# Owen-Liuyuxuan/FSNet

Hardware: AMD Instinct MI355X
Metric: training samples/sec (3-frame triplets) at 192x640, ResNet-18 depth+pose (higher is better)
Workload: dtype bf16; 1 GPU; KITTI Eigen-Zhou-shaped synthetic triplets, ResNet-18 depth+pose, 192x640, bf16, batch 12/GPU, full step (fwd+loss+bwd+clip35+Adam); inputs HBM-resident, no H2D in the timed region; global_batch=12, parallelism=dp1, encoder_pass=two chains (depth and pose encoder on two streams), autotune_steps=0, hipgraph_replays=570

## Files before the change

### fsnet_amd/csrc/bn.hip

```cpp
#include "common.h"
#include "fsnet_hip_internal.h"
#include <algorithm>
#include <cstdlib>

namespace {

__device__ __forceinline__ int pow2_shift(int v) { return (v & (v - 1)) == 0 ? __ffs(v) - 1 : -1; }
__device__ __forceinline__ void split_vec(long i, int CG, int sh, int& cg, long& m) {
  if (sh >= 0) { cg = (int)(i & (CG - 1)); m = i >> sh; }
  else if (i < (1L << 31)) { const unsigned u = (unsigned)i, q = u / (unsigned)CG; cg = (int)(u - q * CG); m = q; }
  else { cg = (int)(i % CG); m = i / CG; }
}
__device__ __forceinline__ void split_row(long m, int H, int W, long& n, int& h, int& w) {
  if (m < (1L << 31)) {
    const unsigned u = (unsigned)m, q = u / (unsigned)W, nn = q / (unsigned)H;
    w = (int)(u - q * W); h = (int)(q - nn * H); n = nn;
  } else {
    w = (int)(m % W); const long q = m / W; h = (int)(q % H); n = q / H;
  }
}


constexpr int MAXC = 2048;

// ... 281 lines not shown
        for (int j = 0; j < V; ++j) {
          v[j] = v[j] * sc[j] + sh[j];
          if (p.relu) v[j] = fmaxf(v[j], 0.f);
        }
        const uint4 u = Unit<T>::pack(v);
        Unit<T>::unpack(u, v);
        if (y && r >= 1 && s >= 1) *reinterpret_cast<uint4*>(y + off) = u;
#pragma unroll
        for (int j = 0; j < V; ++j)
          if (fst || v[j] > best[j]) { best[j] = v[j]; bi[j] = r * 3 + s; }
        fst = false;
      }
    }
    const long mg = ((n * Ho + ho) * Wo + wo) * C + c;
    storev<T>(py + mg, best);
#pragma unroll
    for (int k = 0; k < V / 4; ++k) {
      const uint32_t packed = (uint32_t)bi[4 * k] | ((uint32_t)bi[4 * k + 1] << 8) | ((uint32_t)bi[4 * k + 2] << 16) |
                              ((uint32_t)bi[4 * k + 3] << 24);
      reinterpret_cast<uint32_t*>(p.pool_idx + mg)[k] = packed;
    }
  }
}

template <typename T>
__device__ inline void load_dout(const FsBnBwdArgs& p, const T* dout, long n, int h, int w, int c, float* g) {
  constexpr int V = VecN<T>::N;
  if (!p.fold) {
    loadv<T>(dout + n * p.gN + (long)h * p.gH + (long)w * p.gW + c, g);
    return;
  }
#pragma unroll
  for (int j = 0; j < V; ++j) g[j] = 0.f;
  int hs[2] = {h + 1, 0}, ws[2] = {w + 1, 0};
  int nh = 1, nw = 1;
  if (h == 0) { hs[1] = 0; nh = 2; } else if (h == p.H - 1) { hs[1] = p.H + 1; nh = 2; }
  if (w == 0) { ws[1] = 0; nw = 2; } else if (w == p.W - 1) { ws[1] = p.W + 1; nw = 2; }
  for (int a = 0; a < nh; ++a)
    for (int b = 0; b < nw; ++b) {
      float t[V];
      loadv<T>(dout + n * p.gN + (long)hs[a] * p.gH + (long)ws[b] * p.gW + c, t);
#pragma unroll
      for (int j = 0; j < V; ++j) g[j] += t[j];
    }
}

template <typename T>
__device__ inline void masked_grad(const FsBnBwdArgs& p, const T* dout, const T* yv, long m, int c, float* g) {
  constexpr int V = VecN<T>::N;
  const long hw = (long)p.H * p.W;
  if (!p.fold && p.gW == p.C && p.gH == (long)p.W * p.C && p.gN == hw * p.C &&
      (!p.relu || (p.yW == p.C && p.yH == (long)p.W * p.C && p.yN == hw * p.C))) {
    loadv<T>(dout + m * p.C + c, g);
    if (p.relu) {
      float yy[V];
      loadv<T>(yv + m * p.C + c, yy);
#pragma unroll
      for (int j = 0; j < V; ++j) g[j] = yy[j] > 0.f ? g[j] : 0.f;
    }
    return;
  }
  int w, h; long n;
  split_row(m, p.H, p.W, n, h, w);
  load_dout<T>(p, dout, n, h, w, c, g);
  if (p.relu) {
    float yy[V];
    loadv<T>(yv + n * p.yN + (long)h * p.yH + (long)w * p.yW + c, yy);
#pragma unroll
    for (int j = 0; j < V; ++j) g[j] = yy[j] > 0.f ? g[j] : 0.f;
  }
}


template <typename T>
__device__ inline void pool_grad(const FsBnBwdArgs& p, long m, int c, float* g) {
  constexpr int V = VecN<T>::N;
  const int C = p.C, H = p.H, W = p.W, Ho = H >> 1, Wo = W >> 1;
  const unsigned u = (unsigned)m, q = u / (unsigned)W, nn = q / (unsigned)H;
  const int w = (int)(u - q * W), h = (int)(q - nn * H);
  const int h2 = h >> 1, w2 = w >> 1;
  const int r0 = (h & 1) ? 2 : 1, s0 = (w & 1) ? 2 : 1;
  const bool vh = (h & 1) && h2 + 1 < Ho, vw = (w & 1) && w2 + 1 < Wo;
  const long base = (((long)nn * Ho + h2) * Wo + w2) * C + c;
  const long dh = vh ? (long)Wo * C : 0, dw = vw ? C : 0;
  const long off[4] = {base, base + dw, base + dh, base + dh + dw};
  const int code[4] = {r0 * 3 + s0, r0 * 3, s0, 0};
  const bool ok[4] = {true, vw, vh, vh && vw};
  const T* __restrict__ dy = reinterpret_cast<const T*>(p.pool_dy);
  uint32_t packed[4][V / 4];
  float t[4][V];
#pragma unroll
  for (int k = 0; k < 4; ++k) {
#pragma unroll
    for (int e = 0; e < V / 4; ++e) packed[k][e] = reinterpret_cast<const uint32_t*>(p.pool_idx + off[k])[e];
    loadv<T>(dy + off[k], t[k]);
  }
  if (p.dout) loadv<T>(reinterpret_cast<const T*>(p.dout) + m * C + c, g);
  else {
#pragma unroll
    for (int j = 0; j < V; ++j) g[j] = 0.f;
  }
#pragma unroll
  for (int k = 0; k < 4; ++k)
#pragma unroll
    for (int j = 0; j < V; ++j)
      if (ok[k] && (int)((packed[k][j >> 2] >> (8 * (j & 3))) & 0xff) == code[k]) g[j] += t[k][j];
}
template <typename T>
__device__ inline void pool_mask(const FsBnBwdArgs& p, const T* yv, long m, int c, const float* xr, const float* sc,
                                 const float* sh, float* g) {
  constexpr int V = VecN<T>::N;
  if (!p.relu) return;
  if (yv) {
    float yy[V];
    loadv<T>(yv + m * p.C + c, yy);
#pragma unroll
    for (int j = 0; j < V; ++j) g[j] = yy[j] > 0.f ? g[j] : 0.f;
  } else {
// ... 244 lines not shown
          if (left > 2) req(off + 2 * step, d2, x2, y2);
#pragma unroll
          for (int j = 0; j < V; ++j) { s1[j] += g[j]; s2[j] += g[j] * (xr[j] - mean[j]) * istd[j]; }
        }
        m = m_end;
      }
    }
    for (; m + stride < m_end; m += 2 * stride) {
      float g0[V], g1[V], x0[V], x1[V];
      masked_grad<T>(p, dout, yv, m, c, g0);
      masked_grad<T>(p, dout, yv, m + stride, c, g1);
      loadv<T>(xv + m * C + c, x0);
      loadv<T>(xv + (m + stride) * C + c, x1);
#pragma unroll
      for (int j = 0; j < V; ++j) {
        s1[j] += g0[j] + g1[j];
        s2[j] += g0[j] * (x0[j] - mean[j]) * istd[j] + g1[j] * (x1[j] - mean[j]) * istd[j];
      }
    }
    for (; m < m_end; m += stride) {
      float g0[V], x0[V];
      masked_grad<T>(p, dout, yv, m, c, g0);
      loadv<T>(xv + m * C + c, x0);
#pragma unroll
      for (int j = 0; j < V; ++j) { s1[j] += g0[j]; s2[j] += g0[j] * (x0[j] - mean[j]) * istd[j]; }
    }
  }
#pragma unroll
  for (int j = 0; j < V; ++j) { red[0][j][threadIdx.x] = s1[j]; red[1][j][threadIdx.x] = s2[j]; }
  __syncthreads();
  if (act && pl < 2 * V && pl < PL) {
    for (int kj = pl; kj < 2 * V; kj += PL) {
      int kind = kj / V, j = kj % V;
      float a = 0.f;
      for (int k = 0; k < PL; ++k) a += red[kind][j][k * CGB + cgl];
      double* sl = p.sums + ((long)z * FS_STAT_SLOTS + blockIdx.x % FS_STAT_SLOTS) * 2 * C;
      atomicAdd(sl + kind * C + c + j, (double)a);
    }
  }
}

template <typename T, bool POOL = false>
__global__ __launch_bounds__(256) void bn_bwd_apply_kernel(const FsDual<FsBnBwdArgs, FsNoGeom> d, const int fast) {
  extern __shared__ float bn_smem[];
  const int prob = (int)blockIdx.z >= d.nb0 ? 1 : 0;
  const FsBnBwdArgs& p = d.a[prob];
  const int C = p.C;
  constexpr int V = VecN<T>::N;
  const int CG = C / V, cg_sh = pow2_shift(CG);
  const int SCG = gridDim.y > 1 ? 32 : CG, scg_sh = gridDim.y > 1 ? 5 : cg_sh;
  const int SC = SCG * V, c0 = (int)blockIdx.y * SC;
  float* s_a = bn_smem; float* s_b = bn_smem + SC; float* s_k = bn_smem + 2 * SC;
  float* s_mean = bn_smem + 3 * SC; float* s_istd = bn_smem + 4 * SC;
  const int G = p.groups > 1 ? p.groups : 1;
  const int z = (int)blockIdx.z - (prob ? d.nb0 : 0);
  const int Mg = p.M / G;
  const double* sums = p.sums + (long)z * FS_STAT_SLOTS * 2 * C;
  const double* sums_local = p.sums_local ? p.sums_local + (long)z * FS_STAT_SLOTS * 2 * C : nullptr;
  const T* __restrict__ dout = reinterpret_cast<const T*>(p.dout);
  const T* __restrict__ yv = reinterpret_cast<const T*>(p.y);
  const T* __restrict__ xv = reinterpret_cast<const T*>(p.x);
  const long total = (long)Mg * SCG;
  const long i0 = (long)blockIdx.x * 256 + threadIdx.x;
  float pg[V], px[V];
  if (i0 < total) {
    int cg; long m;
    split_vec(i0, SCG, scg_sh, cg, m);
    m += (long)z * Mg;
    if constexpr (POOL) pool_grad<T>(p, m, c0 + cg * V, pg);
    else masked_grad<T>(p, dout, yv, m, c0 + cg * V, pg);
    loadv<T>(xv + m * C + c0 + cg * V, px);
  }
  for (int cl = threadIdx.x; cl < SC; cl += 256) {
    const int c = c0 + cl;
    double sg = 0.0, sgx = 0.0, lg = 0.0, lgx = 0.0;
#pragma unroll
    for (int k = 0; k < FS_STAT_SLOTS; ++k) {
      sg += sums[(long)k * 2 * C + c]; sgx += sums[(long)k * 2 * C + C + c];
      if (sums_local) { lg += sums_local[(long)k * 2 * C + c]; lgx += sums_local[(long)k * 2 * C + C + c]; }
    }
    float istd = p.save_invstd[z * C + c];
    s_mean[cl] = p.save_mean[z * C + c]; s_istd[cl] = istd;
    s_k[cl] = p.gamma[c] * istd;
    if constexpr (POOL) bn_smem[5 * SC + cl] = (p.beta ? p.beta[c] : 0.f) - s_mean[cl] * s_k[cl];
    s_a[cl] = (float)(sg / p.count);
    s_b[cl] = (float)(sgx / p.count);
    if (blockIdx.x == 0) {
      if (G > 1) {
        if (p.dgamma) atomicAdd(p.dgamma + c, (float)(sums_local ? lgx : sgx));
        if (p.dbeta) atomicAdd(p.dbeta + c, (float)(sums_local ? lg : sg));
      } else {
        if (p.dgamma) p.dgamma[c] += (float)(sums_local ? lgx : sgx);
        if (p.dbeta) p.dbeta[c] += (float)(sums_local ? lg : sg);
      }
    }
  }
  __syncthreads();
  T* __restrict__ dx = reinterpret_cast<T*>(p.dx);
  T* __restrict__ gout = reinterpret_cast<T*>(p.g_out);
  const long stride = (long)gridDim.x * 256;
  if constexpr (!POOL) {
    const long hw = (long)p.H * p.W;
    const bool plain = fast && !p.fold && scg_sh >= 0 && p.gW == C && p.gH == (long)p.W * C && p.gN == hw * C &&
                       (!p.relu || (p.yW == C && p.yH == (long)p.W * C && p.yN == hw * C));
    if (plain) {
      if (i0 >= total) return;
      const int cl = (int)(i0 & (SCG - 1)) * V;
      const long rows = stride >> scg_sh, step = rows * C;
      long off = ((long)z * Mg + (i0 >> scg_sh)) * C + c0 + cl;
      long left = (total - i0 + stride - 1) / stride;
      const bool relu = p.relu != 0;
      float ka[V], kb[V], kk[V], km[V], ki[V];
#pragma unroll
      for (int j = 0; j < V; ++j) { ka[j] = s_a[cl + j]; kb[j] = s_b[cl + j]; kk[j] = s_k[cl + j]; km[j] = s_mean[cl + j]; ki[j] = s_istd[cl + j]; }
      uint4 d1, x1, y1, d2, x2, y2;
      d1 = x1 = y1 = d2 = x2 = y2 = make_uint4(0, 0, 0, 0);
      if (left > 1) {
        d1 = *reinterpret_cast<const uint4*>(dout + off + step); x1 = *reinterpret_cast<const uint4*>(xv + off + step);
        if (relu) y1 = *reinterpret_cast<const uint4*>(yv + off + step);
      }
      if (left > 2) {
        d2 = *reinterpret_cast<const uint4*>(dout + off + 2 * step); x2 = *reinterpret_cast<const uint4*>(xv + off + 2 * step);
        if (relu) y2 = *reinterpret_cast<const uint4*>(yv + off + 2 * step);
      }
      float g[V], xr[V], o[V];
#pragma unroll
      for (int j = 0; j < V; ++j) { g[j] = pg[j]; xr[j] = px[j]; }
      for (;;) {
#pragma unroll
        for (int j = 0; j < V; ++j) {
          float xh = (xr[j] - km[j]) * ki[j];
          o[j] = kk[j] * (g[j] - ka[j] - xh * kb[j]);
        }
        storev<T>(dx + off, o);
        if (gout) storev<T>(gout + off, g);
        if (--left == 0) break;
        off += step;
        Unit<T>::unpack(d1, g); Unit<T>::unpack(x1, xr);
        if (relu) {
          float yy[V];
          Unit<T>::unpack(y1, yy);
#pragma unroll
          for (int j = 0; j < V; ++j) g[j] = yy[j] > 0.f ? g[j] : 0.f;
        }
        d1 = d2; x1 = x2; y1 = y2;
        if (left > 2) {
          d2 = *reinterpret_cast<const uint4*>(dout + off + 2 * step); x2 = *reinterpret_cast<const uint4*>(xv + off + 2 * step);
          if (relu) y2 = *reinterpret_cast<const uint4*>(yv + off + 2 * step);
        }
      }
      return;
    }
  }
  for (long i = i0; i < total; i += stride) {
    int cg; long m;
    split_vec(i, SCG, scg_sh, cg, m);
    m += (long)z * Mg;
    const int cl = cg * V, c = c0 + cl;
    float g[V], xr[V], o[V];
#pragma unroll
    for (int j = 0; j < V; ++j) { g[j] = pg[j]; xr[j] = px[j]; }
    if (i + stride < total) {
      int cg2; long m2;
      split_vec(i + stride, SCG, scg_sh, cg2, m2);
      m2 += (long)z * Mg;
      if constexpr (POOL) pool_grad<T>(p, m2, c0 + cg2 * V, pg);
      else masked_grad<T>(p, dout, yv, m2, c0 + cg2 * V, pg);
      loadv<T>(xv + m2 * C + c0 + cg2 * V, px);
    }
    if constexpr (POOL) pool_mask<T>(p, yv, m, c, xr, s_k + cl, bn_smem + 5 * SC + cl, g);
#pragma unroll
    for (int j = 0; j < V; ++j) {
      float xh = (xr[j] - s_mean[cl + j]) * s_istd[cl + j];
      o[j] = s_k[cl + j] * (g[j] - s_a[cl + j] - xh * s_b[cl + j]);
    }
    storev<T>(dx + m * C + c, o);
    if (gout) storev<T>(gout + m * C + c, g);
  }
}

int bn_slabs(int CG) { return (CG > 32 && (CG & (CG - 1)) == 0) ? CG / 32 : 1; }

bool bn_pool_quads(int CG) { return CG >= 1 && CG <= 32 && (CG & (CG - 1)) == 0; }

int grid_for(long items) {
  long b = (items + 255) / 256;
  const long cap = 512;
  if (b > cap) b = cap;
  if (b < 1) b = 1;
  return (int)b;
}

}

extern "C" int fs_bn_finalize(const FsBnApplyArgs* a, float* scale, float* shift, void* stream) {
  if (!a || !a->gamma || !a->beta || !a->save_mean || !a->save_invstd || !scale || !shift) return FS_EINVAL;
  if (!a->stats && (!a->running_mean || !a->running_var)) return FS_EINVAL;
  if (a->C <= 0 || a->C > MAXC || a->gamma2) return FS_EINVAL;
  const int G = a->groups > 1 ? a->groups : 1;
  if (G > 1 && !a->stats) return FS_EINVAL;
  hipLaunchKernelGGL(bn_finalize_kernel, dim3((a->C + 255) / 256, G), dim3(256), 0, reinterpret_cast<hipStream_t>(stream),
                     *a, scale, shift);
  return fs_launch_status();
}

namespace {
int bn_apply_check(const FsBnApplyArgs* a) {
  if (!a || !a->x || (!a->y && !a->pool_y) || !a->gamma || !a->beta || !a->save_mean || !a->save_invstd) return FS_EINVAL;
  if (a->pool_y) {
    if (!a->pool_idx || !a->stats || a->res || a->gamma2 || a->pad_out || a->H <= 0 || a->W <= 0 || (a->H & 1) || (a->W & 1))
      return FS_EINVAL;
    if (a->M % (a->H * a->W) != 0 || (long)a->M * (a->C / 4) >= 0x7fffffffL) return FS_EINVAL;
    if (a->y && !(a->yW == a->C && a->yH == (long)a->W * a->C && a->yN == (long)a->H * a->W * a->C)) return FS_EINVAL;
  }
  if (!a->stats && (!a->running_mean || !a->running_var)) return FS_EINVAL;
  if (a->C % 8 != 0 || a->C > MAXC || a->M <= 0) return FS_EINVAL;
  if (a->gamma2 && (!a->res || !a->beta2 || !a->save_mean2 || !a->save_invstd2)) return FS_EINVAL;
  if (a->gamma2 && !a->stats2 && (!a->running_mean2 || !a->running_var2)) return FS_EINVAL;
  const int G = a->groups > 1 ? a->groups : 1;
  if (a->M % G != 0 || (G > 1 && !a->stats)) return FS_EINVAL;
  return FS_OK;
}
int bn_bwd_check(const FsBnBwdArgs* a, bool apply) {
  if (!a || (!a->dout && !a->pool_dy) || !a->x || !a->sums || !a->save_mean || !a->save_invstd) return FS_EINVAL;
  if (apply && (!a->dx || !a->gamma)) return FS_EINVAL;
  if (a->C % 8 != 0 || a->C > MAXC || a->M <= 0) return FS_EINVAL;
  const int G = a->groups > 1 ? a->groups : 1;
  if (a->M % G != 0) return FS_EINVAL;
  if (a->pool_dy) {
    if (!a->pool_idx || !a->gamma || a->fold || a->g_out || a->H <= 0 || a->W <= 0 || (a->H & 1) || (a->W & 1)) return FS_EINVAL;
    if (a->relu && !a->y && !a->beta) return FS_EINVAL;
    const long hw = (long)a->H * a->W;
    if (a->M % hw != 0 || (a->M / G) % hw != 0 || (long)a->M >= 0x7fffffffL) return FS_EINVAL;
    if (a->dout && !(a->gW == a->C && a->gH == (long)a->W * a->C && a->gN == hw * a->C)) return FS_EINVAL;
    if (a->y && !(a->yW == a->C && a->yH == (long)a->W * a->C && a->yN == hw * a->C)) return FS_EINVAL;
    return FS_OK;
  }
  if (a->relu && !a->y) return FS_EINVAL;
  return FS_OK;
}
template <typename A>
FsDual<A, FsNoGeom> bn_dual(const A* a, const A* b) {
  FsDual<A, FsNoGeom> d;
  d.a[0] = *a; d.a[1] = b ? *b : *a;
  d.g[0].unused = d.g[1].unused = 0;
  d.nb0 = a->groups > 1 ? a->groups : 1;
  d.nprob = b ? 2 : 1;
  return d;
}
}

extern "C" int fs_bn_apply2(const FsBnApplyArgs* a, const FsBnApplyArgs* b, int dtype, void* stream) {
  int r = bn_apply_check(a);
  if (r != FS_OK) return r;
  if (b) {
    r = bn_apply_check(b);
    if (r != FS_OK) return r;
    if (b->C != a->C || (a->pool_y != nullptr) != (b->pool_y != nullptr) || (a->pool_y && (a->H != b->H || a->W != b->W))) {
      r = fs_bn_apply2(a, nullptr, dtype, stream);
      return r != FS_OK ? r : fs_bn_apply2(b, nullptr, dtype, stream);
    }
  }
  hipStream_t st = reinterpret_cast<hipStream_t>(stream);
  const int vec = dtype == FS_DTYPE_BF16 ? 8 : 4;
  const int G = a->groups > 1 ? a->groups : 1, G1 = b ? (b->groups > 1 ? b->groups : 1) : 0;
  long items = (long)(a->M / G) * (a->C / vec);
  if (b) items = std::max(items, (long)(b->M / G1) * (b->C / vec));
  const FsDual<FsBnApplyArgs, FsNoGeom> d = bn_dual(a, b);
  if (a->pool_y) {
    dim3 pgrid(std::min(2 * grid_for(items / 4), (int)((items / 4 + 255) / 256)), 1, G + G1);
    if (pgrid.x < 1) pgrid.x = 1;
    const unsigned plds = 2u * a->C * sizeof(float);
    if (dtype == FS_DTYPE_BF16) hipLaunchKernelGGL(bn_apply_pool_kernel<bf16>, pgrid, dim3(256), plds, st, d);
    else if (dtype == FS_DTYPE_F32) hipLaunchKernelGGL(bn_apply_pool_kernel<float>, pgrid, dim3(256), plds, st, d);
    else return FS_EINVAL;
    return fs_launch_status();
  }
  const int nslab = bn_slabs(a->C / vec);
  dim3 grid(std::min(grid_for(items / nslab), std::max(32, grid_for(1L << 40) / nslab)), nslab, G + G1);
  const unsigned lds = ((a->gamma2 || (b && b->gamma2)) ? 4u : 2u) * (a->C / nslab) * sizeof(float);
  const int fast = 1;
  if (dtype == FS_DTYPE_BF16) hipLaunchKernelGGL(bn_apply_kernel<bf16>, grid, dim3(256), lds, st, d, fast);
  else if (dtype == FS_DTYPE_F32) hipLaunchKernelGGL(bn_apply_kernel<float>, grid, dim3(256), lds, st, d, fast);
  else return FS_EINVAL;
  return fs_launch_status();
}

extern "C" int fs_bn_apply(const FsBnApplyArgs* a, int dtype, void* stream) { return fs_bn_apply2(a, nullptr, dtype, stream); }

extern "C" int fs_bn_bwd_reduce2(const FsBnBwdArgs* a, const FsBnBwdArgs* b, int dtype, void* stream) {
  int r = bn_bwd_check(a, false);
// ... 13 lines not shown
  if (b) Mg = std::max<long>(Mg, b->M / G1);
  const FsDual<FsBnBwdArgs, FsNoGeom> d = bn_dual(a, b);
  if (a->pool_dy && bn_pool_quads(CG)) {
    long Qg = (a->M / G) / 4;
    if (b) Qg = std::max<long>(Qg, (b->M / G1) / 4);
    dim3 grid((unsigned)std::min<long>((Qg + 256 / CG - 1) / (256 / CG), 1024), 1, G + G1);
    if (dtype == FS_DTYPE_BF16) hipLaunchKernelGGL(bn_bwd_reduce_pool_kernel<bf16>, grid, dim3(256), 0, st, d);
    else if (dtype == FS_DTYPE_F32) hipLaunchKernelGGL(bn_bwd_reduce_pool_kernel<float>, grid, dim3(256), 0, st, d);
    else return FS_EINVAL;
    return fs_launch_status();
  }
#define LAUNCH_REDUCE(CGB, ROWS_PER_BLOCK, MAXB)                                                               \
  {                                                                                                             \
    dim3 grid((unsigned)std::min<long>((Mg + (ROWS_PER_BLOCK) - 1) / (ROWS_PER_BLOCK), MAXB), (CG + CGB - 1) / CGB, G + G1); \
    if (a->pool_dy) {                                                                                           \
      if (dtype == FS_DTYPE_BF16) hipLaunchKernelGGL((bn_bwd_reduce_kernel<bf16, CGB, true>), grid, dim3(256), 0, st, d, 0);  \
      else if (dtype == FS_DTYPE_F32) hipLaunchKernelGGL((bn_bwd_reduce_kernel<float, CGB, true>), grid, dim3(256), 0, st, d, 0); \
      else return FS_EINVAL;                                                                                    \
    } else                                                                                                      \
    if (dtype == FS_DTYPE_BF16) hipLaunchKernelGGL((bn_bwd_reduce_kernel<bf16, CGB>), grid, dim3(256), 0, st, d, rfast);  \
    else if (dtype == FS_DTYPE_F32) hipLaunchKernelGGL((bn_bwd_reduce_kernel<float, CGB>), grid, dim3(256), 0, st, d, rfast); \
    else return FS_EINVAL;                                                                                      \
  }
  const int rfast = 1;
  const long wide_cap = std::max<long>(32, std::min<long>(512, 1024 / ((long)((CG + 31) / 32) * (G + G1))));
  if (CG >= 32) LAUNCH_REDUCE(32, 16, wide_cap)
  else if (CG >= 8) LAUNCH_REDUCE(8, 64, 1024)
  else if (CG >= 4) LAUNCH_REDUCE(4, 128, 1024)
  else LAUNCH_REDUCE(2, 256, 1024)
#undef LAUNCH_REDUCE
  return fs_launch_status();
}

extern "C" int fs_bn_bwd_reduce(const FsBnBwdArgs* a, int dtype, void* stream) { return fs_bn_bwd_reduce2(a, nullptr, dtype, stream); }

extern "C" int fs_bn_bwd_apply2(const FsBnBwdArgs* a, const FsBnBwdArgs* b, int dtype, void* stream) {
  int r = bn_bwd_check(a, true);
  if (r != FS_OK) return r;
  if (b) {
    r = bn_bwd_check(b, true);
    if (r != FS_OK) return r;
    if (b->C != a->C || (a->pool_dy != nullptr) != (b->pool_dy != nullptr) || (a->pool_dy && (a->H != b->H || a->W != b->W))) {
      r = fs_bn_bwd_apply2(a, nullptr, dtype, stream);
      return r != FS_OK ? r : fs_bn_bwd_apply2(b, nullptr, dtype, stream);
    }
  }
  hipStream_t st = reinterpret_cast<hipStream_t>(stream);
  const int vec = dtype == FS_DTYPE_BF16 ? 8 : 4;
  const int G = a->groups > 1 ? a->groups : 1, G1 = b ? (b->groups > 1 ? b->groups : 1) : 0;
  long items = (long)(a->M / G) * (a->C / vec);
  if (b) items = std::max(items, (long)(b->M / G1) * (b->C / vec));
  const int nslab = a->pool_dy ? 1 : bn_slabs(a->C / vec);
  dim3 grid(std::min(grid_for(items / nslab), std::max(32, grid_for(1L << 40) / nslab)), nslab, G + G1);
  const unsigned lds = (a->pool_dy ? 6u : 5u) * (a->C / nslab) * sizeof(float);
  const FsDual<FsBnBwdArgs, FsNoGeom> d = bn_dual(a, b);
  const int fast = 1;
  if (a->pool_dy && bn_pool_quads(a->C / vec)) {
    const int CG = a->C / vec;
    long Qg = (a->M / G) / 4;
    if (b) Qg = std::max<long>(Qg, (b->M / G1) / 4);
    dim3 qgrid((unsigned)std::min<long>((Qg + 256 / CG - 1) / (256 / CG), 2048), 1, G + G1);
    if (dtype == FS_DTYPE_BF16) hipLaunchKernelGGL(bn_bwd_apply_pool_kernel<bf16>, qgrid, dim3(256), lds, st, d);
    else if (dtype == FS_DTYPE_F32) hipLaunchKernelGGL(bn_bwd_apply_pool_kernel<float>, qgrid, dim3(256), lds, st, d);
    else return FS_EINVAL;
    return fs_launch_status();
  }
  if (a->pool_dy) {
    if (dtype == FS_DTYPE_BF16) hipLaunchKernelGGL((bn_bwd_apply_kernel<bf16, true>), grid, dim3(256), lds, st, d, 0);
    else if (dtype == FS_DTYPE_F32) hipLaunchKernelGGL((bn_bwd_apply_kernel<float, true>), grid, dim3(256), lds, st, d, 0);
    else return FS_EINVAL;
    return fs_launch_status();
  }
  if (dtype == FS_DTYPE_BF16) hipLaunchKernelGGL(bn_bwd_apply_kernel<bf16>, grid, dim3(256), lds, st, d, fast);
  else if (dtype == FS_DTYPE_F32) hipLaunchKernelGGL(bn_bwd_apply_kernel<float>, grid, dim3(256), lds, st, d, fast);
  else return FS_EINVAL;
  return fs_launch_status();
}

extern "C" int fs_bn_bwd_apply(const FsBnBwdArgs* a, int dtype, void* stream) { return fs_bn_bwd_apply2(a, nullptr, dtype, stream); }
```

### fsnet_amd/csrc/common.h

```cpp
#pragma once
#include <hip/hip_runtime.h>
#include <stdint.h>

typedef __bf16 bf16;
typedef __attribute__((ext_vector_type(8))) __bf16 bf16x8;
typedef __attribute__((ext_vector_type(4))) __bf16 bf16x4;
typedef __attribute__((ext_vector_type(4))) short s16x4;
typedef __attribute__((ext_vector_type(4))) float f32x4;

#define FS_WAVE 64

#define FS_OK 0
#define FS_EINVAL 1
#define FS_ELAUNCH 2

static inline int fs_launch_status() {
  hipError_t e = hipGetLastError();
  return e == hipSuccess ? FS_OK : FS_ELAUNCH;
}

template <typename T> struct ElemTraits;
template <> struct ElemTraits<float> {
  static constexpr int EG = 4;
  __device__ static inline float to_f(float v) { return v; }
  __device__ static inline float from_f(float v) { return v; }
};
template <> struct ElemTraits<bf16> {
  static constexpr int EG = 8;
  __device__ static inline float to_f(bf16 v) { return (float)v; }
  __device__ static inline bf16 from_f(float v) { return (bf16)v; }
};

__device__ static inline float bf16_bits_to_f(uint32_t b16) { return __uint_as_float(b16 << 16); }
__device__ static inline uint32_t f_to_bf16_bits(float f) {
  uint32_t u = __float_as_uint(f);
  u += 0x7fffu + ((u >> 16) & 1u);
  return u >> 16;
}
typedef __attribute__((ext_vector_type(2))) __bf16 bf16x2_t;
typedef __attribute__((ext_vector_type(2))) float f32x2_t;
__device__ static inline uint32_t pack_bf16x2(float lo, float hi) {
  f32x2_t v = {lo, hi};
  return __builtin_bit_cast(uint32_t, __builtin_convertvector(v, bf16x2_t));
}

template <typename T> __device__ inline void load4(const T* p, float v[4]);
template <> __device__ inline void load4<float>(const float* p, float v[4]) {
  float4 t = *reinterpret_cast<const float4*>(p);
  v[0] = t.x; v[1] = t.y; v[2] = t.z; v[3] = t.w;
}
template <> __device__ inline void load4<bf16>(const bf16* p, float v[4]) {
  uint2 t = *reinterpret_cast<const uint2*>(p);
  v[0] = bf16_bits_to_f(t.x & 0xffffu); v[1] = bf16_bits_to_f(t.x >> 16);
  v[2] = bf16_bits_to_f(t.y & 0xffffu); v[3] = bf16_bits_to_f(t.y >> 16);
}
template <typename T> __device__ inline void store4(T* p, const float v[4]);
template <> __device__ inline void store4<float>(float* p, const float v[4]) {
  *reinterpret_cast<float4*>(p) = make_float4(v[0], v[1], v[2], v[3]);
}
template <> __device__ inline void store4<bf16>(bf16* p, const float v[4]) {
  uint2 t; t.x = pack_bf16x2(v[0], v[1]); t.y = pack_bf16x2(v[2], v[3]);
  *reinterpret_cast<uint2*>(p) = t;
}

__host__ __device__ static inline unsigned fs_div_magic(int d) { return (1u << 20) / (unsigned)d + 1u; }
__device__ static inline int fs_fastdiv(int x, unsigned magic) { return (int)(((unsigned)x * magic) >> 20); }

struct FsDiv { unsigned m; unsigned sh; };
__host__ static inline FsDiv fs_make_div(int d) {
  int l = 0;
  while ((1LL << l) < (long long)d) ++l;
  FsDiv r;
  r.m = (unsigned)(((1ULL << (31 + l)) / (unsigned long long)d) + 1ULL);
  r.sh = (unsigned)(31 + l);
  return r;
}
__device__ static inline int fs_div(int x, FsDiv d) {
  return (int)(((unsigned long long)(unsigned)x * d.m) >> d.sh);
}

template <int CTRL>
__device__ static inline float dpp_mov(float v) {
  return __builtin_bit_cast(float, __builtin_amdgcn_update_dpp(0, __builtin_bit_cast(int, v), CTRL, 0xf, 0xf, true));
}
template <int CTRL>
__device__ static inline double dpp_mov(double v) {
  const long long b = __builtin_bit_cast(long long, v);
  const int lo = __builtin_amdgcn_update_dpp(0, (int)b, CTRL, 0xf, 0xf, true);
  const int hi = __builtin_amdgcn_update_dpp(0, (int)(b >> 32), CTRL, 0xf, 0xf, true);
  return __builtin_bit_cast(double, ((long long)hi << 32) | (unsigned int)lo);
}
__device__ static inline float read_lane(float v, int lane) {
  return __builtin_bit_cast(float, __builtin_amdgcn_readlane(__builtin_bit_cast(int, v), lane));
}
__device__ static inline double read_lane(double v, int lane) {
  const long long b = __builtin_bit_cast(long long, v);
  const int lo = __builtin_amdgcn_readlane((int)b, lane), hi = __builtin_amdgcn_readlane((int)(b >> 32), lane);
  return __builtin_bit_cast(double, ((long long)hi << 32) | (unsigned int)lo);
}
template <typename F>
__device__ static inline F row16_sum(F v) {
  v += dpp_mov<0xB1>(v);
  v += dpp_mov<0x4E>(v);
  v += dpp_mov<0x141>(v);
  v += dpp_mov<0x140>(v);
  return v;
}
__device__ static inline float wave_sum(float v) {
  v = row16_sum(v);
  return (read_lane(v, 0) + read_lane(v, 16)) + (read_lane(v, 32) + read_lane(v, 48));
}
__device__ static inline double wave_sum_d(double v) {
  v = row16_sum(v);
  return (read_lane(v, 0) + read_lane(v, 16)) + (read_lane(v, 32) + read_lane(v, 48));
}
// ... 56 lines not shown
```

### fsnet_amd/csrc/conv1x1.hip

```cpp
#include <cstdlib>
#include "common.h"
#include "fsnet_hip_internal.h"

namespace {

__device__ __forceinline__ uint4 buf_load16(__amdgpu_buffer_rsrc_t rsrc, int voff) {
  return __builtin_bit_cast(uint4, __builtin_amdgcn_raw_buffer_load_b128(rsrc, voff, 0, 0));
}

template <typename T, int CO, int KC>
__global__ __launch_bounds__(256) void conv1x1_kernel(const FsConvArgs p, const FsDiv dW, const FsDiv dH) {
  constexpr int PIX = 128, WP = 4, WC = 1;
  constexpr int WPIX = PIX / WP, WCO = CO / WC;
  constexpr int TP = WPIX / 16, TC = WCO / 16;
  constexpr int UR = KC / 8;
  constexpr int KS = KC / 32;
  constexpr int LCU = (CO * UR + 255) / 256;
  static_assert(sizeof(T) == 2, "bf16 only");
  __shared__ uint4 lds_c[CO * UR < 128 ? 128 : CO * UR];
  constexpr int OROW = CO * 2 + 16;
  __shared__ __attribute__((aligned(16))) unsigned char lds_o[4][WPIX * OROW];

  const int t = threadIdx.x;
  const int lane = t & 63, wave = t >> 6;
// ... 165 lines not shown
  if (p.stats) {
    __syncthreads();
    float* red = reinterpret_cast<float*>(&lds_c[0]);
#pragma unroll
    for (int a = 0; a < TC; ++a)
#pragma unroll
      for (int j = 0; j < 4; ++j) {
        float u = s1[a][j], w = s2[a][j];
        u = row16_sum(u); w = row16_sum(w);
        if (li == 0) {
          int cl = wc * WCO + a * 16 + lg * 4 + j;
          red[(wp * CO + cl) * 2] = u; red[(wp * CO + cl) * 2 + 1] = w;
        }
      }
    __syncthreads();
    if (t < CO) {
      float u = 0.f, w = 0.f;
#pragma unroll
      for (int k = 0; k < WP; ++k) { u += red[(k * CO + t) * 2]; w += red[(k * CO + t) * 2 + 1]; }
      int co = co0 + t;
      if (co < p.Co) {
        const long sg = p.grp_imgs > 0 ? (long)blockIdx.z : (p.stat_group_rows > 0 ? pix0 / p.stat_group_rows : 0);
        double* sl = p.stats + (sg * FS_STAT_SLOTS + px % FS_STAT_SLOTS) * 2 * p.Co;
        atomicAdd(sl + co, (double)u);
        atomicAdd(sl + p.Co + co, (double)w);
      }
    }
  }
}


template <typename T, int CO, int KC>
int launch_1x1(const FsConvArgs& a, hipStream_t st) {
  constexpr int PIX = 128;
  const int npix = (a.M + PIX - 1) / PIX, nco = a.Co_p / CO;
  int blocks = npix * nco;
  if (nco % 8 != 0 && 8 % nco == 0) { const int g = 8 / nco; blocks = 8 * ((npix + g - 1) / g); }
  hipLaunchKernelGGL((conv1x1_kernel<T, CO, KC>), dim3(blocks, 1, a.grp_imgs > 0 ? a.N / a.grp_imgs : 1), dim3(256), 0, st,
                     a, fs_make_div(a.Wd), fs_make_div(a.Hd));
  return fs_launch_status();
}

template <typename T, int CO>
int launch_co(const FsConvArgs& a, hipStream_t st) {
  if (a.Cs <= 64) return launch_1x1<T, CO, 64>(a, st);
  if (a.Cs <= 128) return launch_1x1<T, CO, 128>(a, st);
  return launch_1x1<T, CO, 256>(a, st);
}

}

extern "C" int fs_conv1x1(const FsConvArgs* args, int dtype, void* stream) {
  if (!args || !args->src || !args->wgt || !args->dst) return FS_EINVAL;
  if (dtype != FS_DTYPE_BF16 || args->dshift != 0 || args->ncls > 1 || args->hb_add != 0 || args->hb_mul < 1) return FS_EINVAL;
  if (args->Cs <= 0 || (args->Cs * 2) % 64 != 0 || args->Co % 4 != 0 || args->Co_p % 16 != 0 || args->M <= 0) return FS_EINVAL;
  if (args->src_bytes <= 0 || args->src_bytes > 0x7fffffffLL || args->wgt_bytes <= 0 || args->wgt_bytes > 0x7fffffffLL)
    return FS_EINVAL;
  if (args->stats && args->stat_group_rows > 0 && args->stat_group_rows % 128 != 0) return FS_EINVAL;
  hipStream_t st = reinterpret_cast<hipStream_t>(stream);
  {
    const int r = fs_conv1x1_gemm(*args, st);
    if (r != FS_EINVAL) return r;
  }
  const int cop = args->Co_p;
  if (cop % 64 == 0) return launch_co<bf16, 64>(*args, st);
  if (cop % 32 == 0) return launch_co<bf16, 32>(*args, st);
  return launch_co<bf16, 16>(*args, st);
}
```

### fsnet_amd/csrc/conv3x3_halo.hip

```cpp
#include "common.h"
#include "fsnet_hip_internal.h"
#include "conv_pro.h"
#include <algorithm>
#include <cstdlib>

namespace {

__device__ __forceinline__ int swz64(int row) { return ((row >> 3) & 1) << 1; }

__device__ __forceinline__ uint4 buf_load16(__amdgpu_buffer_rsrc_t rsrc, int voff) {
  return __builtin_bit_cast(uint4, __builtin_amdgcn_raw_buffer_load_b128(rsrc, voff, 0, 0));
}

__device__ __forceinline__ void lds_barrier() {
  asm volatile("s_waitcnt lgkmcnt(0)" ::: "memory");
  __builtin_amdgcn_s_barrier();
  asm volatile("" ::: "memory");
}

struct HaloGeom {
  int TH, TW;
  int tiles_x, tiles_y;
  unsigned mTW, mHW;
  FsDiv dTX, dTY;
// ... 141 lines not shown
    int pi = wp * WPIX + b * 16 + li;
    if (pi >= ntile) pi = 0;
    int ty = fs_fastdiv(pi, g.mTW), tx = pi - ty * g.TW;
    hbase[b] = (STR * ty * HWs + tx) * HS + lg;
  }

  f32x4 acc[TC][TP];
#pragma unroll
  for (int a = 0; a < TC; ++a)
#pragma unroll
    for (int b = 0; b < TP; ++b) acc[a][b] = f32x4{0.f, 0.f, 0.f, 0.f};
  const int s2_row = HWs * HS, s2_par = (g.TW + 1) * HS;

  const int nchunk = (p.Cs * (int)sizeof(T) + 63) / 64;
  load_regs(0);
  for (int cc = 0; cc < nchunk; ++cc) {
    lds_barrier();
    store_lds(cc);
    lds_barrier();
    if (cc + 1 < nchunk) load_regs(cc + 1);
#pragma unroll
    for (int tap = 0; tap < 9; ++tap) {
      const int r = tap / 3, s = tap - r * 3;
      const int hoff = STR == 2 ? r * s2_row + (s & 1) * s2_par + (s >> 1) * HS
                                : (fwd ? (r * HW + s) : ((2 - r) * HW + (2 - s))) * HS;
      uint4 fa[TC], fb[TP];
#pragma unroll
      for (int a = 0; a < TC; ++a) {
        int row = tap * CO + wc * WCO + a * 16 + li;
        fa[a] = lds_w[row * 4 + (lg ^ swz64(row))];
      }
#pragma unroll
      for (int b = 0; b < TP; ++b) fb[b] = lds_h[hbase[b] + hoff];
#pragma unroll
      for (int a = 0; a < TC; ++a)
#pragma unroll
        for (int b = 0; b < TP; ++b) {
          if constexpr (sizeof(T) == 2) {
            acc[a][b] = __builtin_amdgcn_mfma_f32_16x16x32_bf16(
                __builtin_bit_cast(bf16x8, fa[a]), __builtin_bit_cast(bf16x8, fb[b]), acc[a][b], 0, 0, 0);
          } else {
            f32x4 va = __builtin_bit_cast(f32x4, fa[a]);
            f32x4 vb = __builtin_bit_cast(f32x4, fb[b]);
#pragma unroll
            for (int j = 0; j < 4; ++j)
              acc[a][b] = __builtin_amdgcn_mfma_f32_16x16x4f32(va[j], vb[j], acc[a][b], 0, 0, 0);
          }
        }
    }
  }

  const bool has_add = STR == 1 && p.addend != nullptr, has_mask = STR == 1 && p.mask != nullptr;
  const bool has_bnb = STR == 1 && p.bnb_x != nullptr, has_mbn = has_bnb && p.bnb_scale != nullptr;
  float s1[TC][4], s2[TC][4];
#pragma unroll
  for (int a = 0; a < TC; ++a)
#pragma unroll
    for (int j = 0; j < 4; ++j) { s1[a][j] = 0.f; s2[a][j] = 0.f; }
  const int sgoff = p.stat_group_rows > 0 ? fs_div(n, g.dIPG) * p.Co : 0;
  int doff[TP], aoff[TP], moff[TP];
#pragma unroll
  for (int b = 0; b < TP; ++b) {
    int pi = wp * WPIX + b * 16 + li;
    int ty = fs_fastdiv(pi, g.mTW), tx = pi - ty * g.TW;
    int y = y0 + ty, x = x0 + tx;
    bool mok = pi < ntile && y < p.Hd && x < p.Wd;
    doff[b] = mok ? n * (int)p.dN + y * (int)p.dH + x * (int)p.dW : -1;
    aoff[b] = n * (int)p.aN + y * (int)p.aH + x * (int)p.aW;
    moff[b] = n * (int)p.mN + y * (int)p.mH + x * (int)p.mW;
  }
#pragma unroll
  for (int a = 0; a < TC; ++a) {
    const int co = co0 + wc * WCO + a * 16 + lg * 4;
    if (co >= p.Co) continue;
    float4 bv = make_float4(0.f, 0.f, 0.f, 0.f), mu = bv, is = bv, msc = bv, msh = bv;
    if (p.bias) bv = *reinterpret_cast<const float4*>(p.bias + co);
    if (has_bnb) {
      mu = *reinterpret_cast<const float4*>(p.bnb_mean + sgoff + co);
      is = *reinterpret_cast<const float4*>(p.bnb_invstd + sgoff + co);
      if (has_mbn) {
        msc = *reinterpret_cast<const float4*>(p.bnb_scale + sgoff + co);
        msh = *reinterpret_cast<const float4*>(p.bnb_shift + sgoff + co);
      }
    }
#pragma unroll
    for (int b = 0; b < TP; ++b) {
      if (doff[b] < 0) continue;
      float v[4] = {acc[a][b][0] + bv.x, acc[a][b][1] + bv.y, acc[a][b][2] + bv.z, acc[a][b][3] + bv.w};
      if (has_add) {
        float av[4];
        load4<T>(reinterpret_cast<const T*>(p.addend) + aoff[b] + co, av);
        v[0] += av[0]; v[1] += av[1]; v[2] += av[2]; v[3] += av[3];
      }
      if (p.relu) {
#pragma unroll
        for (int j = 0; j < 4; ++j) v[j] = fmaxf(v[j], 0.f);
      }
      if (has_mask) {
        float mv[4];
        load4<T>(reinterpret_cast<const T*>(p.mask) + moff[b] + co, mv);
#pragma unroll
        for (int j = 0; j < 4; ++j) v[j] = mv[j] > 0.f ? v[j] : 0.f;
      }
      if (has_bnb) {
        float cv[4];
        load4<T>(reinterpret_cast<const T*>(p.bnb_x) + doff[b] + co, cv);
        if (has_mbn) {
          v[0] = (cv[0] * msc.x + msh.x) > 0.f ? v[0] : 0.f; v[1] = (cv[1] * msc.y + msh.y) > 0.f ? v[1] : 0.f;
          v[2] = (cv[2] * msc.z + msh.z) > 0.f ? v[2] : 0.f; v[3] = (cv[3] * msc.w + msh.w) > 0.f ? v[3] : 0.f;
        }
        s1[a][0] += v[0]; s1[a][1] += v[1]; s1[a][2] += v[2]; s1[a][3] += v[3];
        s2[a][0] += v[0] * (cv[0] - mu.x) * is.x; s2[a][1] += v[1] * (cv[1] - mu.y) * is.y;
        s2[a][2] += v[2] * (cv[2] - mu.z) * is.z; s2[a][3] += v[3] * (cv[3] - mu.w) * is.w;
      } else if (p.stats) {
#pragma unroll
        for (int j = 0; j < 4; ++j) { s1[a][j] += v[j]; s2[a][j] += v[j] * v[j]; }
      }
      if (p.out_f32) store4<float>(reinterpret_cast<float*>(p.dst) + doff[b] + co, v);
      else store4<T>(reinterpret_cast<T*>(p.dst) + doff[b] + co, v);
    }
  }
  if (p.stats) {
    lds_barrier();
    float* red = reinterpret_cast<float*>(&lds_w[0]);
#pragma unroll
    for (int a = 0; a < TC; ++a)
#pragma unroll
      for (int j = 0; j < 4; ++j) {
        float u = s1[a][j], w = s2[a][j];
        u = row16_sum(u); w = row16_sum(w);
        if (li == 0) {
          int cl = wc * WCO + a * 16 + lg * 4 + j;
          red[(wp * CO + cl) * 2] = u; red[(wp * CO + cl) * 2 + 1] = w;
        }
      }
    lds_barrier();
    if (t < CO) {
      float u = 0.f, w = 0.f;
#pragma unroll
      for (int k = 0; k < WP; ++k) { u += red[(k * CO + t) * 2]; w += red[(k * CO + t) * 2 + 1]; }
      int co = co0 + t;
      if (co < p.Co) {
        const long sg = p.stat_group_rows > 0 ? fs_div(n, g.dIPG) : 0;
        double* sl = p.stats + (sg * FS_STAT_SLOTS + px % FS_STAT_SLOTS) * 2 * p.Co;
        atomicAdd(sl + co, (double)u);
        atomicAdd(sl + p.Co + co, (double)w);
      }
    }
  }
  if constexpr (PRO != 0) { if (bid == 0) pro_block0<PRO>(p, t, 256); }
}

HaloGeom pick_geom(int Hd, int Wd, int PIX, int hmax) {
  HaloGeom best{0, 0, 0, 0, 0u, 0u, FsDiv{0u, 0u}, FsDiv{0u, 0u}, FsDiv{0u, 0u}, FsDiv{0u, 0u}, 0};
  double best_cost = 1e30;
  for (int tw = std::min(4, Wd); tw <= std::min(Wd, 64); ++tw) {
    int th = std::min(PIX / tw, Hd);
    if (th < 1 || (th + 2) * (tw + 2) > hmax) continue;
    int tx = (Wd + tw - 1) / tw, ty = (Hd + th - 1) / th;
    double waste = (double)tx * ty * PIX / ((double)Hd * Wd);
    double halo = (double)(th + 2) * (tw + 2) / ((double)th * tw);
    double cost = waste * (1.0 + 0.15 * halo);
    if (cost < best_cost - 1e-9) { best_cost = cost; best.TH = th; best.TW = tw; best.tiles_x = tx; best.tiles_y = ty; }
  }
  if (best.TW > 0) {
    best.mTW = fs_div_magic(best.TW); best.mHW = fs_div_magic(best.TW + 2);
// ... 83 lines not shown
template <typename T>
int dispatch(const FsConvArgs& a, const FsConvArgs* b, hipStream_t st) {
  const int cop = a.Co_p;
  const int nimg = a.N + (b ? b->N : 0);
  auto blocks_for = [&](int PIX, int CO) {
    HaloGeom g = pick_geom(a.Hd, a.Wd, PIX, PIX == 256 ? 360 : (PIX == 128 ? 208 : 120));
    return g.TH == 0 ? 0L : (long)nimg * g.tiles_x * g.tiles_y * (cop / CO);
  };
  if (cop % 32 == 0) {
    if (blocks_for(128, 32) < 256) return launch_halo<T, 128, 16, 4>(a, b, st);
    return launch_halo<T, 128, 32, 4>(a, b, st);
  }
  if (cop % 16 == 0) {
    if (blocks_for(256, 16) >= 1024) return launch_halo<T, 256, 16, 4>(a, b, st);
    return launch_halo<T, 128, 16, 4>(a, b, st);
  }
  return FS_EINVAL;
}

}

int fs_conv3x3_t32(const FsConvArgs& a, const FsConvArgs* b, int dtype, hipStream_t st);
int fs_conv3x3_p1(const FsConvArgs& a, int dtype, hipStream_t st);

namespace {
int conv3x3_check(const FsConvArgs* args, int dtype) {
  if (!args || !args->src || !args->wgt || !args->dst) return FS_EINVAL;
  const int es = dtype == FS_DTYPE_BF16 ? 2 : 4;
  if (args->Cs <= 0 || (args->Cs * es) % 32 != 0 || ((args->Cs * es) % 64 != 0 && args->Cs * es != 32) || args->dshift != 0)
    return FS_EINVAL;
  const bool s2 = args->hb_mul == 2;
  if (args->hb_mul != 1 && !(s2 && args->sgn > 0 && args->hb_add == -1 && (args->Cs * es) % 64 == 0 && args->pro_mode == 0 &&
                             !args->bnb_x && !args->addend && !args->mask &&
                             args->Hd == (args->Hs - 1) / 2 + 1 && args->Wd == (args->Ws - 1) / 2 + 1))
    return FS_EINVAL;
  if (args->Co % 4 != 0 || args->Co_p % 16 != 0 || args->N <= 0) return FS_EINVAL;
  if (args->src_bytes <= 0 || args->src_bytes > 0x7fffffffLL || args->wgt_bytes <= 0 ||
      args->wgt_bytes > 0x7fffffffLL)
    return FS_EINVAL;
  if (!pro_args_ok(*args)) return FS_EINVAL;
  if (args->pro_mode != 0 && (args->Cs * es) % 64 != 0) return FS_EINVAL;
  {
    auto span_ok = [&](const void* ptr, int64_t sn, int64_t sh, int64_t sw) {
      if (!ptr) return true;
      if (sn < 0 || sh < 0 || sw < 0) return false;
      return (int64_t)(args->N - 1) * sn + (int64_t)(args->Hd - 1) * sh + (int64_t)(args->Wd - 1) * sw + args->Co_p < 0x7fffffffLL;
    };
    if (!span_ok(args->dst, args->dN, args->dH, args->dW) || !span_ok(args->addend, args->aN, args->aH, args->aW) ||
        !span_ok(args->mask, args->mN, args->mH, args->mW))
      return FS_EINVAL;
  }
  if (args->bnb_scale && (!args->bnb_x || !args->bnb_shift || args->mask)) return FS_EINVAL;
  if (args->bnb_x && (!args->stats || !args->bnb_mean || !args->bnb_invstd)) return FS_EINVAL;
  return FS_OK;
}

bool conv3x3_pairable(const FsConvArgs& a, const FsConvArgs& b) {
  auto nn = [](const void* x, const void* y) { return (x == nullptr) == (y == nullptr); };
  return a.Hs == b.Hs && a.Ws == b.Ws && a.Hd == b.Hd && a.Wd == b.Wd && a.Cs == b.Cs && a.Co == b.Co && a.Co_p == b.Co_p &&
         a.nchunks == b.nchunks && a.kg == b.kg && a.hb_mul == b.hb_mul && a.hb_add == b.hb_add && a.sgn == b.sgn &&
         a.relu == b.relu && a.out_f32 == b.out_f32 && a.pro_mode == b.pro_mode && a.pro_relu == b.pro_relu &&
         a.wgt_bytes == b.wgt_bytes && nn(a.bias, b.bias) && nn(a.addend, b.addend) && nn(a.mask, b.mask) &&
         nn(a.stats, b.stats) && nn(a.bnb_x, b.bnb_x) && nn(a.bnb_scale, b.bnb_scale) && nn(a.pro_stats, b.pro_stats);
}

int conv3x3_entry(const FsConvArgs* args, const FsConvArgs* b, int dtype, hipStream_t st) {
  int r = conv3x3_check(args, dtype);
  if (r != FS_OK) return r;
  if (b) {
    r = conv3x3_check(b, dtype);
    if (r != FS_OK) return r;
    if (!conv3x3_pairable(*args, *b)) {
      r = conv3x3_entry(args, nullptr, dtype, st);
      return r != FS_OK ? r : conv3x3_entry(b, nullptr, dtype, st);
    }
  }
  if (args->hb_mul == 2) {
    if (dtype == FS_DTYPE_BF16) return dispatch_s2<bf16>(*args, b, st);
    if (dtype == FS_DTYPE_F32) return dispatch_s2<float>(*args, b, st);
    return FS_EINVAL;
  }
  const int force = args->force_impl;
  if (force < 0 || force > 5 || (b && b->force_impl != force)) return FS_EINVAL;
  if (!b && (force == 0 || force == 5)) {
    r = fs_conv3x3_p1(*args, dtype, st);
    if (r != FS_EINVAL) return r;
  }
  if (force != 1) {
    r = fs_conv3x3_t32(*args, b, dtype, st);
    if (r != FS_EINVAL || (force >= 2 && force <= 4)) return r;
  }
  if (dtype == FS_DTYPE_BF16) return dispatch<bf16>(*args, b, st);
  if (dtype == FS_DTYPE_F32) return dispatch<float>(*args, b, st);
  return FS_EINVAL;
}
}

extern "C" int fs_conv3x3_halo(const FsConvArgs* args, int dtype, void* stream) {
  return conv3x3_entry(args, nullptr, dtype, reinterpret_cast<hipStream_t>(stream));
}

extern "C" int fs_conv3x3_halo2(const FsConvArgs* a0, const FsConvArgs* a1, int dtype, void* stream) {
  return conv3x3_entry(a0, a1, dtype, reinterpret_cast<hipStream_t>(stream));
}

extern "C" int fs_conv3x3_halo_plan(const FsConvArgs* args, int dtype, int32_t* plan) {
  if (!plan) return FS_EINVAL;
  plan[0] = -1; plan[1] = plan[2] = plan[3] = 0;
  fs_conv3x3_plan_slot = plan;
  const int r = conv3x3_entry(args, nullptr, dtype, nullptr);
  fs_conv3x3_plan_slot = nullptr;
  return r;
}

extern "C" int fs_conv3x3_halo2_plan(const FsConvArgs* a0, const FsConvArgs* a1, int dtype, int32_t* plan) {
  if (!plan || !a0) return FS_EINVAL;
// ... 9 lines not shown
```

### fsnet_amd/csrc/conv3x3_p1.hip

```cpp
#include "common.h"
#include "fsnet_hip_internal.h"
#include <algorithm>
#include <cstdlib>

namespace {

__device__ __forceinline__ int p1_swz64(int row) { return ((row >> 3) & 1) << 1; }
__device__ __forceinline__ uint4 p1_load16(__amdgpu_buffer_rsrc_t rsrc, int voff) {
  return __builtin_bit_cast(uint4, __builtin_amdgcn_raw_buffer_load_b128(rsrc, voff, 0, 0));
}
__device__ __forceinline__ void p1_barrier() {
  asm volatile("s_waitcnt lgkmcnt(0)" ::: "memory");
  __builtin_amdgcn_s_barrier();
  asm volatile("" ::: "memory");
}

struct P1Geom {
  int TH, TW, tiles_x, tiles_y, ntiles;
  unsigned mTW, mHW;
  FsDiv dTX, dTY, dIPG;
};

template <typename T, int CO, int UQ>
__global__ __launch_bounds__(256, CO == 16 ? 3 : 2) void conv3x3_p1_kernel(const FsConvArgs p, const P1Geom g) {
// ... 26 lines not shown
      const int tap = rt / CO, row = rt - tap * CO;
      const int off = (tap < 9 && q * 16 < row_bytes) ? row * wrow_bytes + tap * row_bytes + q * 16 : OOB;
      const uint4 w = p1_load16(rs_wgt, off);
      if (rt < 9 * CO) lds_w[rt * 4 + (q ^ p1_swz64(rt))] = w;
    }
  }

  int hrel[LH], hyx[LH];
#pragma unroll
  for (int i = 0; i < LH; ++i) {
    const int idx = t + i * 256, hp = idx / UQ, q = idx % UQ;
    const int hy = fs_fastdiv(min(hp, 4095), g.mHW), hx = hp - hy * HW;
    const bool ok = hp < nhalo && q * 16 < row_bytes;
    hyx[i] = ok ? ((hy << 16) | hx) : -1;
    hrel[i] = (int)(((long)hy * p.sH + (long)hx * p.sW) * es) + q * 16;
  }
  int hbase[TP];
#pragma unroll
  for (int b = 0; b < TP; ++b) {
    int pi = wp * WPIX + b * 16 + li;
    if (pi >= ntile) pi = 0;
    const int ty = fs_fastdiv(pi, g.mTW), tx = pi - ty * g.TW;
    hbase[b] = (ty * HW + tx) * HS + lg;
  }
  int prow[TP];
#pragma unroll
  for (int b = 0; b < TP; ++b) {
    const int pi = wp * WPIX + b * 16 + li;
    const int ty = fs_fastdiv(pi, g.mTW), tx = pi - ty * g.TW;
    prow[b] = pi < ntile ? ((ty << 16) | tx) : -1;
  }

  uint4 rh[LH];
  auto tile_origin = [&](int tile, int& n, int& y0, int& x0) {
    const int tq = fs_div(tile, g.dTX); const int tx_i = tile - tq * g.tiles_x;
    n = fs_div(tq, g.dTY); const int ty_i = tq - n * g.tiles_y;
    y0 = ty_i * g.TH; x0 = tx_i * g.TW;
  };
  auto load_tile = [&](int tile) {
    int n, y0, x0;
    tile_origin(tile, n, y0, x0);
    const int oy = y0 + p.hb_add + (fwd ? 0 : -2), ox = x0 + p.hb_add + (fwd ? 0 : -2);
    const long base = ((long)n * p.sN + (long)oy * p.sH + (long)ox * p.sW) * es;
#pragma unroll
    for (int i = 0; i < LH; ++i) {
      const int hy = hyx[i] >> 16, hx = hyx[i] & 0xffff;
      const bool ok = hyx[i] >= 0 && (unsigned)(oy + hy) < (unsigned)p.Hs && (unsigned)(ox + hx) < (unsigned)p.Ws;
      rh[i] = p1_load16(rs_src, ok ? (int)(base + hrel[i]) : OOB);
    }
  };

  const bool has_add = p.addend != nullptr, has_mask = p.mask != nullptr;
  const bool has_bnb = p.bnb_x != nullptr, has_mbn = has_bnb && p.bnb_scale != nullptr;

  auto store_halo = [&]() {
#pragma unroll
    for (int i = 0; i < LH; ++i) {
      const int idx = t + i * 256, hp = idx / UQ, q = idx % UQ;
      if (hp < HMAX) lds_h[hp * HS + q] = rh[i];
    }
  };
  if constexpr (UQ < 4) {
    for (int idx = t; idx < HMAX * (4 - UQ); idx += 256) lds_h[(idx / (4 - UQ)) * HS + UQ + idx % (4 - UQ)] = make_uint4(0u, 0u, 0u, 0u);
  }
  const int gstep = (int)gridDim.x;
  load_tile(blockIdx.x);
  store_halo();
  if ((int)blockIdx.x + gstep < g.ntiles) load_tile(blockIdx.x + gstep);
  p1_barrier();
  for (int tile = blockIdx.x; tile < g.ntiles; tile += gstep) {
    f32x4 acc[TC][TP];
#pragma unroll
    for (int a = 0; a < TC; ++a)
#pragma unroll
      for (int b = 0; b < TP; ++b) acc[a][b] = f32x4{0.f, 0.f, 0.f, 0.f};
#pragma unroll 1
    for (int r = 0; r < 3; ++r)
#pragma unroll
    for (int s = 0; s < 3; ++s) {
      const int tap = r * 3 + s;
      const int hoff = (fwd ? (r * HW + s) : ((2 - r) * HW + (2 - s))) * HS;
      uint4 fa[TC], fb[TP];
#pragma unroll
      for (int a = 0; a < TC; ++a) {
        const int row = tap * CO + a * 16 + li;
        fa[a] = lds_w[row * 4 + (lg ^ p1_swz64(row))];
      }
#pragma unroll
      for (int b = 0; b < TP; ++b) fb[b] = lds_h[hbase[b] + hoff];
#pragma unroll
      for (int a = 0; a < TC; ++a)
#pragma unroll
        for (int b = 0; b < TP; ++b) {
          if constexpr (sizeof(T) == 2) {
            acc[a][b] = __builtin_amdgcn_mfma_f32_16x16x32_bf16(
                __builtin_bit_cast(bf16x8, fa[a]), __builtin_bit_cast(bf16x8, fb[b]), acc[a][b], 0, 0, 0);
          } else {
            const f32x4 va = __builtin_bit_cast(f32x4, fa[a]), vb = __builtin_bit_cast(f32x4, fb[b]);
#pragma unroll
            for (int j = 0; j < 4; ++j)
              acc[a][b] = __builtin_amdgcn_mfma_f32_16x16x4f32(va[j], vb[j], acc[a][b], 0, 0, 0);
          }
        }
    }

    p1_barrier();
    if (tile + gstep < g.ntiles) {
      store_halo();
      if (tile + 2 * gstep < g.ntiles) load_tile(tile + 2 * gstep);
    }

    int n, y0, x0;
    tile_origin(tile, n, y0, x0);
    const int sgoff = p.stat_group_rows > 0 ? fs_div(n, g.dIPG) * p.Co : 0;
    float s1[TC][4], s2[TC][4];
#pragma unroll
    for (int a = 0; a < TC; ++a)
#pragma unroll
      for (int j = 0; j < 4; ++j) { s1[a][j] = 0.f; s2[a][j] = 0.f; }
    int doff[TP], aoff[TP], moff[TP];
#pragma unroll
    for (int b = 0; b < TP; ++b) {
      const int y = y0 + (prow[b] >> 16), x = x0 + (prow[b] & 0xffff);
      const bool mok = prow[b] >= 0 && y < p.Hd && x < p.Wd;
      doff[b] = mok ? n * (int)p.dN + y * (int)p.dH + x * (int)p.dW : -1;
      aoff[b] = n * (int)p.aN + y * (int)p.aH + x * (int)p.aW;
      moff[b] = n * (int)p.mN + y * (int)p.mH + x * (int)p.mW;
    }
#pragma unroll
    for (int a = 0; a < TC; ++a) {
      const int co = a * 16 + lg * 4;
      if (co >= p.Co) continue;
      float4 bv = make_float4(0.f, 0.f, 0.f, 0.f), mu = bv, is = bv, msc = bv, msh = bv;
      if (p.bias) bv = *reinterpret_cast<const float4*>(p.bias + co);
      if (has_bnb) {
        mu = *reinterpret_cast<const float4*>(p.bnb_mean + sgoff + co);
        is = *reinterpret_cast<const float4*>(p.bnb_invstd + sgoff + co);
        if (has_mbn) {
          msc = *reinterpret_cast<const float4*>(p.bnb_scale + sgoff + co);
          msh = *reinterpret_cast<const float4*>(p.bnb_shift + sgoff + co);
        }
      }
#pragma unroll
      for (int b = 0; b < TP; ++b) {
        if (doff[b] < 0) continue;
        float v[4] = {acc[a][b][0] + bv.x, acc[a][b][1] + bv.y, acc[a][b][2] + bv.z, acc[a][b][3] + bv.w};
        if (has_add) {
          float av[4];
          load4<T>(reinterpret_cast<const T*>(p.addend) + aoff[b] + co, av);
          v[0] += av[0]; v[1] += av[1]; v[2] += av[2]; v[3] += av[3];
        }
        if (p.relu) {
#pragma unroll
          for (int j = 0; j < 4; ++j) v[j] = fmaxf(v[j], 0.f);
        }
        if (has_mask) {
          float mv[4];
          load4<T>(reinterpret_cast<const T*>(p.mask) + moff[b] + co, mv);
#pragma unroll
          for (int j = 0; j < 4; ++j) v[j] = mv[j] > 0.f ? v[j] : 0.f;
        }
        if (has_bnb) {
          float cv[4];
          load4<T>(reinterpret_cast<const T*>(p.bnb_x) + doff[b] + co, cv);
          if (has_mbn) {
            v[0] = (cv[0] * msc.x + msh.x) > 0.f ? v[0] : 0.f; v[1] = (cv[1] * msc.y + msh.y) > 0.f ? v[1] : 0.f;
            v[2] = (cv[2] * msc.z + msh.z) > 0.f ? v[2] : 0.f; v[3] = (cv[3] * msc.w + msh.w) > 0.f ? v[3] : 0.f;
          }
          s1[a][0] += v[0]; s1[a][1] += v[1]; s1[a][2] += v[2]; s1[a][3] += v[3];
          s2[a][0] += v[0] * (cv[0] - mu.x) * is.x; s2[a][1] += v[1] * (cv[1] - mu.y) * is.y;
          s2[a][2] += v[2] * (cv[2] - mu.z) * is.z; s2[a][3] += v[3] * (cv[3] - mu.w) * is.w;
        } else if (p.stats) {
#pragma unroll
          for (int j = 0; j < 4; ++j) { s1[a][j] += v[j]; s2[a][j] += v[j] * v[j]; }
        }
        if (p.out_f32) store4<float>(reinterpret_cast<float*>(p.dst) + doff[b] + co, v);
        else store4<T>(reinterpret_cast<T*>(p.dst) + doff[b] + co, v);
      }
    }
    if (p.stats) {
#pragma unroll
      for (int a = 0; a < TC; ++a)
#pragma unroll
        for (int j = 0; j < 4; ++j) {
          float u = row16_sum(s1[a][j]), w = row16_sum(s2[a][j]);
          if (li == 0) {
            const int cl = a * 16 + lg * 4 + j;
            red[(wp * CO + cl) * 2] = u; red[(wp * CO + cl) * 2 + 1] = w;
          }
        }
      p1_barrier();
      if (t < CO) {
        float u = 0.f, w = 0.f;
#pragma unroll
        for (int k = 0; k < 4; ++k) { u += red[(k * CO + t) * 2]; w += red[(k * CO + t) * 2 + 1]; }
        if (t < p.Co) {
          const long sg = p.stat_group_rows > 0 ? fs_div(n, g.dIPG) : 0;
          double* sl = p.stats + (sg * FS_STAT_SLOTS + tile % FS_STAT_SLOTS) * 2 * p.Co;
          atomicAdd(sl + t, (double)u);
          atomicAdd(sl + p.Co + t, (double)w);
        }
      }
    }
    p1_barrier();
  }
}

P1Geom p1_pick_geom(int Hd, int Wd) {
  P1Geom best{};
  double best_cost = 1e30;
  for (int tw = std::min(4, Wd); tw <= std::min(Wd, 64); ++tw) {
    const int th = std::min(256 / tw, Hd);
    if (th < 1 || (th + 2) * (tw + 2) > 360) continue;
    const int tx = (Wd + tw - 1) / tw, ty = (Hd + th - 1) / th;
    const double waste = (double)tx * ty * 256 / ((double)Hd * Wd);
    const double halo = (double)(th + 2) * (tw + 2) / ((double)th * tw);
    const double cost = waste * (1.0 + 0.15 * halo);
    if (cost < best_cost - 1e-9) { best_cost = cost; best.TH = th; best.TW = tw; best.tiles_x = tx; best.tiles_y = ty; }
  }
  if (best.TW > 0) {
    best.mTW = fs_div_magic(best.TW); best.mHW = fs_div_magic(best.TW + 2);
    best.dTX = fs_make_div(best.tiles_x); best.dTY = fs_make_div(best.tiles_y);
  }
  return best;
// ... 55 lines not shown
```

### fsnet_amd/csrc/conv3x3_s2d.hip

```cpp
#include "t32_common.h"

namespace {

struct S2dGeom {
  int TH, TW;
  int tiles_x, tiles_y;
  unsigned mTW, mHW;
  FsDiv dTX, dTY;
  FsDiv dIPG;
  int pix_major;
};

constexpr int S2D_PIX = 128;
constexpr int S2D_CO = 32;
constexpr int S2D_HMAX = 192;

constexpr int s2d_cls(int pos) { return pos == 0 ? 0 : (pos <= 2 ? 1 : (pos <= 4 ? 2 : 3)); }
constexpr int s2d_off(int pos) { return pos == 1 ? 1 : (pos == 3 ? 2 : (pos == 5 ? 3 : (pos == 6 ? 2 : (pos == 7 ? 1 : 0)))); }

template <typename T, int EP, bool DS>
__global__ __launch_bounds__(256, 3) void conv3x3_s2d_kernel(const FsDual<FsConvArgs, S2dGeom> d) {
  const int prob = (int)blockIdx.x >= d.nb0 ? 1 : 0;
  const FsConvArgs& p = d.a[prob];
  const S2dGeom& g = d.g[prob];
// ... 268 lines not shown
  return blocks;
}

template <typename T, int EP, bool DS>
int s2d_launch(const FsConvArgs& a, const FsConvArgs* b, hipStream_t st) {
  FsDual<FsConvArgs, S2dGeom> d;
  d.a[0] = a; d.a[1] = b ? *b : a;
  d.nprob = b ? 2 : 1;
  int blocks = s2d_problem(a, d.g[0]);
  if (blocks == 0) return FS_EINVAL;
  d.g[1] = d.g[0];
  d.nb0 = blocks;
  if (b) {
    const int b1 = s2d_problem(*b, d.g[1]);
    if (b1 == 0) return FS_EINVAL;
    d.nb0 = fs_xcd_round(blocks);
    blocks = d.nb0 + b1;
  }
  hipLaunchKernelGGL((conv3x3_s2d_kernel<T, EP, DS>), dim3(blocks), dim3(256), 0, st, d);
  return fs_launch_status();
}

inline int s2d_ep_mask(const FsConvArgs& a) {
  return (a.addend ? EP_ADDEND : 0) | (a.mask ? EP_MASK : 0) | (a.bnb_x ? EP_BNB : 0);
}

template <typename T, bool DS>
int s2d_dispatch_ep(const FsConvArgs& a, const FsConvArgs* b, int ep, hipStream_t st) {
  if constexpr (sizeof(T) == 2) {
    switch (ep) {
      case EP_ADDEND: return s2d_launch<T, EP_ADDEND, DS>(a, b, st);
      case EP_ADDEND | EP_MASK | EP_BNB: return s2d_launch<T, EP_ADDEND | EP_MASK | EP_BNB, DS>(a, b, st);
      case EP_MASK | EP_BNB: return s2d_launch<T, EP_MASK | EP_BNB, DS>(a, b, st);
      default: break;
    }
  }
  return s2d_launch<T, -1, DS>(a, b, st);
}

template <typename T>
int s2d_dispatch(const FsConvArgs& a, const FsConvArgs* b, hipStream_t st) {
  const int ep = (b && s2d_ep_mask(*b) != s2d_ep_mask(a)) ? -1 : s2d_ep_mask(a);
  return a.ds_src ? s2d_dispatch_ep<T, true>(a, b, ep, st) : s2d_dispatch_ep<T, false>(a, b, ep, st);
}

bool s2d_takes(const FsConvArgs& a, int dtype) {
  const int es = dtype == FS_DTYPE_BF16 ? 2 : 4;
  if (!a.src || !a.wgt || !a.dst) return false;
  if (a.ncls != 4 || a.hb_mul != 1 || a.hb_add != 0 || a.sgn != 1 || a.dshift != 0) return false;
  if (a.Hs != a.Hd || a.Ws != a.Wd || a.N <= 0) return false;
  if ((a.Cs * es) % 64 != 0 || a.Co_p % S2D_CO != 0 || a.Co % 8 != 0) return false;
  if (a.bias || a.relu || a.out_f32 || a.pro_mode || a.bnb_scale || a.grp_imgs) return false;
  if (a.stats && !a.bnb_x) return false;
  if ((a.ds_src != nullptr) != (a.ds_wgt != nullptr)) return false;
  if (a.ds_src && (a.ds_wgt_row_bytes < (int64_t)a.Cs * es || a.ds_wgt_row_bytes * a.Co_p >= 0x7ffff000LL ||
                   ((uintptr_t)a.ds_src & 15u) || ((uintptr_t)a.ds_wgt & 15u)))
    return false;
  if (a.bnb_x && (!a.stats || !a.bnb_mean || !a.bnb_invstd)) return false;
  if (a.src_bytes <= 0 || a.src_bytes >= 0x7ffff000LL) return false;
  const int64_t wrow = a.wgt_row_bytes ? a.wgt_row_bytes : (int64_t)a.nchunks * a.kg * 16;
  if (wrow < (int64_t)9 * a.Cs * es || (int64_t)a.Co_p * wrow >= 0x7ffff000LL) return false;
  auto al16 = [&](const void* ptr, int64_t sn, int64_t sh, int64_t sw) {
    return ptr == nullptr || (((uintptr_t)ptr & 15u) == 0 && (sn * es) % 16 == 0 && (sh % 2) == 0 && (sw % 2) == 0 &&
                              ((sh / 2) * es) % 16 == 0 && ((sw / 2) * es) % 16 == 0);
  };
  if (!al16(a.dst, a.dN, a.dH, a.dW) || !al16(a.addend, a.aN, a.aH, a.aW) || !al16(a.mask, a.mN, a.mH, a.mW)) return false;
  auto span_ok = [&](const void* ptr, int64_t sn, int64_t sh, int64_t sw) {
    if (!ptr) return true;
    if (sn < 0 || sh < 0 || sw < 0) return false;
    return (int64_t)(a.N - 1) * sn + (int64_t)a.Hd * sh + (int64_t)a.Wd * sw + a.Co < 0x7fffffffLL;
  };
  if (!span_ok(a.dst, a.dN, a.dH, a.dW) || !span_ok(a.addend, a.aN, a.aH, a.aW) || !span_ok(a.mask, a.mN, a.mH, a.mW)) return false;
  if (a.Hd >= 0x7fff || a.Wd >= 0xffff) return false;
  S2dGeom g;
  return s2d_problem(a, g) > 0;
}

bool s2d_pairable(const FsConvArgs& a, const FsConvArgs& b) {
  return a.Co_p == b.Co_p && a.Cs == b.Cs && (a.ds_src != nullptr) == (b.ds_src != nullptr);
}

int s2d_entry(const FsConvArgs* a, const FsConvArgs* b, int dtype, hipStream_t st) {
  if (!a || !s2d_takes(*a, dtype) || (b && !s2d_takes(*b, dtype))) return FS_EINVAL;
  if (b && !s2d_pairable(*a, *b)) {
    const int r = s2d_entry(a, nullptr, dtype, st);
    return r != FS_OK ? r : s2d_entry(b, nullptr, dtype, st);
  }
  if (dtype == FS_DTYPE_BF16) return s2d_dispatch<bf16>(*a, b, st);
  if (dtype == FS_DTYPE_F32) return s2d_dispatch<float>(*a, b, st);
  return FS_EINVAL;
}

}

extern "C" int fs_conv3x3_s2d(const FsConvArgs* args, int dtype, void* stream) {
  return s2d_entry(args, nullptr, dtype, reinterpret_cast<hipStream_t>(stream));
}

extern "C" int fs_conv3x3_s2d2(const FsConvArgs* a0, const FsConvArgs* a1, int dtype, void* stream) {
  return s2d_entry(a0, a1, dtype, reinterpret_cast<hipStream_t>(stream));
}
```

### fsnet_amd/csrc/conv3x3_t32.hip

```cpp
#include "t32_common.h"
#include "conv_pro.h"

namespace {

constexpr int t32_minwaves(int PIX, int CO, int EP, int PRO) {
  return EP < 0 ? 1 : (t32_occupancy(PIX, CO) - (PRO != 0 ? 1 : 0) < 1 ? 1 : t32_occupancy(PIX, CO) - (PRO != 0 ? 1 : 0));
}

template <typename T, int PIX, int CO, int EP, int PRO>
__global__ __launch_bounds__(256, t32_minwaves(PIX, CO, EP, PRO)) void conv3x3_t32_kernel(const FsDual<FsConvArgs, T32Geom> d) {
  const int prob = (int)blockIdx.x >= d.nb0 ? 1 : 0;
  const FsConvArgs& p = d.a[prob];
  const T32Geom& g = d.g[prob];
  const int bid = (int)blockIdx.x - (prob ? d.nb0 : 0);
  constexpr int WPIX = PIX / 4;
  constexpr int TP = WPIX / 32, TC = CO / 32;
  constexpr int HMAX = t32_hmax(PIX);
  constexpr int HS = 5;
  constexpr int LH = (HMAX * 4 + 255) / 256;
  constexpr int WU = 9 * CO * 4;
  constexpr int LW = (WU + 255) / 256;
  constexpr int BUFU = HMAX * HS + WU;
  constexpr int EPS = 9;
  constexpr int OOB = 0x7ffff000;
// ... 103 lines not shown
#pragma unroll
  for (int b = 0; b < TP; ++b) {
    int pi = wave * WPIX + b * 32 + l31;
    if (pi >= ntile) pi = 0;
    const int ty = fs_fastdiv(pi, g.mTW), tx = pi - ty * g.TW;
    hbase[b] = (ty * HW + tx) * HS + hk;
  }
  const int we = hk ^ ((l31 >> 2) & 3);
  const int wa0 = l31 * 4 + we, wa1 = l31 * 4 + (we ^ 2);

  f32x16 acc[TC][TP];
#pragma unroll
  for (int a = 0; a < TC; ++a)
#pragma unroll
    for (int b = 0; b < TP; ++b)
#pragma unroll
      for (int j = 0; j < 16; ++j) acc[a][b][j] = 0.f;

  const int nchunk = (row_bytes + 63) / 64;
  load_regs(0);
  if constexpr (PRO != 0) {
    pro_build_table<PRO>(p, t32_pro_tab, pgrp, t, 256);
  }
  for (int cc = 0; cc < nchunk; ++cc) {
    t32_barrier();
    store_lds(cc);
    t32_barrier();
    if (cc + 1 < nchunk) load_regs(cc + 1);
#pragma unroll
    for (int tap = 0; tap < 9; ++tap) {
      const int r = tap / 3, s = tap - r * 3;
      const int hoff = (fwd ? (r * HW + s) : ((2 - r) * HW + (2 - s))) * HS;
#pragma unroll
      for (int ks = 0; ks < 2; ++ks) {
        uint4 fa[TC], fb[TP];
#pragma unroll
        for (int a = 0; a < TC; ++a) fa[a] = lds_w[(ks ? wa1 : wa0) + (tap * CO + a * 32) * 4];
#pragma unroll
        for (int b = 0; b < TP; ++b) fb[b] = lds[hbase[b] + hoff + 2 * ks];
#pragma unroll
        for (int a = 0; a < TC; ++a)
#pragma unroll
          for (int b = 0; b < TP; ++b) Mma32<T>::run(acc[a][b], fa[a], fb[b]);
      }
    }
  }

  const bool has_bias = T32_FLAG(EP_BIAS, p.bias != nullptr);
  const bool has_add = T32_FLAG(EP_ADDEND, p.addend != nullptr);
  const bool has_relu = T32_FLAG(EP_RELU, p.relu != 0);
  const bool has_mask = T32_FLAG(EP_MASK, p.mask != nullptr);
  const bool has_bnb = T32_FLAG(EP_BNB, p.bnb_x != nullptr);
  const bool has_stats = T32_FLAG(EP_STATS | EP_BNB, p.stats != nullptr);
  const bool has_mbn = T32_FLAG(EP_MASKBN, p.bnb_scale != nullptr);
  const bool f32out = T32_FLAG(EP_F32, p.out_f32 != 0);

  t32_barrier();
  float* ep = reinterpret_cast<float*>(lds + wave * (WPIX * EPS));
  const int l15 = lane & 15, cs = lane >> 4;
  const int sgoff = p.stat_group_rows > 0 ? fs_div(n, g.dIPG) * p.Co : 0;
  constexpr int NI = WPIX / 16;
  int doff[NI];
#pragma unroll
  for (int i = 0; i < NI; ++i) {
    const int pi = wave * WPIX + i * 16 + l15;
    const int ty = fs_fastdiv(pi, g.mTW), tx = pi - ty * g.TW;
    const int y = y0 + ty, x = x0 + tx;
    const bool mok = pi < ntile && y < p.Hd && x < p.Wd;
    doff[i] = mok ? ((y << 16) | x) : -1;
  }
  float* red = reinterpret_cast<float*>(lds + PIX * EPS);

#pragma unroll
  for (int a = 0; a < TC; ++a) {
#pragma unroll
    for (int b = 0; b < TP; ++b)
#pragma unroll
      for (int gq = 0; gq < 4; ++gq) {
        const float4 v = make_float4(acc[a][b][4 * gq], acc[a][b][4 * gq + 1], acc[a][b][4 * gq + 2], acc[a][b][4 * gq + 3]);
        *reinterpret_cast<float4*>(ep + ((b * 32 + l31) * EPS + 2 * gq + hk) * 4) = v;
      }
    t32_wave_sync();
    const int co = co0 + a * 32 + cs * 8;
    const bool cok = co < p.Co;
    const int cof = cok ? co : 0;
    float bv[8], msc[8], msh[8], s1[8], s2[8];
#pragma unroll
    for (int j = 0; j < 8; ++j) { bv[j] = 0.f; msc[j] = 0.f; msh[j] = 0.f; s1[j] = 0.f; s2[j] = 0.f; }
    if (has_bias) load8<float>(p.bias + cof, bv);
    if (has_mbn) { load8<float>(p.bnb_scale + sgoff + cof, msc); load8<float>(p.bnb_shift + sgoff + cof, msh); }
#pragma unroll
    for (int i = 0; i < NI; ++i) {
      const float* rp = ep + ((i * 16 + l15) * EPS + 2 * cs) * 4;
      const float4 v0 = reinterpret_cast<const float4*>(rp)[0], v1 = reinterpret_cast<const float4*>(rp)[1];
      if (doff[i] < 0 || !cok) continue;
      const int y = doff[i] >> 16, x = doff[i] & 0xffff;
      const int dof = n * (int)p.dN + y * (int)p.dH + x * (int)p.dW;
      float v[8] = {v0.x + bv[0], v0.y + bv[1], v0.z + bv[2], v0.w + bv[3], v1.x + bv[4], v1.y + bv[5], v1.z + bv[6], v1.w + bv[7]};
      if (has_add) {
        float av[8];
        load8<T>(reinterpret_cast<const T*>(p.addend) + n * (int)p.aN + y * (int)p.aH + x * (int)p.aW + co, av);
#pragma unroll
        for (int j = 0; j < 8; ++j) v[j] += av[j];
      }
      if (has_relu) {
#pragma unroll
        for (int j = 0; j < 8; ++j) v[j] = fmaxf(v[j], 0.f);
      }
      if (has_mask) {
        float mv[8];
        load8<T>(reinterpret_cast<const T*>(p.mask) + n * (int)p.mN + y * (int)p.mH + x * (int)p.mW + co, mv);
#pragma unroll
        for (int j = 0; j < 8; ++j) v[j] = mv[j] > 0.f ? v[j] : 0.f;
      }
      if (has_bnb) {
        float cv[8];
        load8<T>(reinterpret_cast<const T*>(p.bnb_x) + dof + co, cv);
        if (has_mbn) {
#pragma unroll
          for (int j = 0; j < 8; ++j) v[j] = (cv[j] * msc[j] + msh[j]) > 0.f ? v[j] : 0.f;
        }
#pragma unroll
        for (int j = 0; j < 8; ++j) { s1[j] += v[j]; s2[j] += v[j] * cv[j]; }
      } else if (has_stats) {
#pragma unroll
        for (int j = 0; j < 8; ++j) { s1[j] += v[j]; s2[j] += v[j] * v[j]; }
      }
      if (f32out) store8<float>(reinterpret_cast<float*>(p.dst) + dof + co, v);
      else store8<T>(reinterpret_cast<T*>(p.dst) + dof + co, v);
    }
    if (has_stats) {
      float sv[16];
#pragma unroll
      for (int j = 0; j < 8; ++j) { sv[j] = s1[j]; sv[8 + j] = s2[j]; }
      const float tot = t32_reduce16_row(sv, lane);
      const int j = ((lane >> 1) & 1) * 4 + ((lane >> 2) & 1) * 2 + ((lane >> 3) & 1);
      red[(wave * CO + a * 32 + cs * 8 + j) * 2 + (lane & 1)] = tot;
    }
    t32_wave_sync();
  }
  if (has_stats) {
    t32_barrier();
    if (t < CO) {
      float u = 0.f, w = 0.f;
#pragma unroll
      for (int k = 0; k < 4; ++k) { u += red[(k * CO + t) * 2]; w += red[(k * CO + t) * 2 + 1]; }
      const int co = co0 + t;
      if (co < p.Co) {
        const long sg = p.stat_group_rows > 0 ? fs_div(n, g.dIPG) : 0;
        double* sl = p.stats + (sg * FS_STAT_SLOTS + px % FS_STAT_SLOTS) * 2 * p.Co;
        double wd = (double)w;
        if (has_bnb) wd = (wd - (double)p.bnb_mean[sg * p.Co + co] * (double)u) * (double)p.bnb_invstd[sg * p.Co + co];
        atomicAdd(sl + co, (double)u);
        atomicAdd(sl + p.Co + co, wd);
      }
    }
  }
  if constexpr (PRO != 0) { if (bid == 0) pro_block0<PRO>(p, t, 256); }
}

template <int PIX, int CO>
int t32_problem(const FsConvArgs& a, T32Geom& g) {
  g = t32_pick_geom(a.Hd, a.Wd, PIX, t32_hmax(PIX));
  if (g.TH == 0) return 0;
  g.dIPG = FsDiv{0u, 0u}; g.dPRG = FsDiv{0u, 0u};
  if (a.stat_group_rows > 0) {
    const long hw = (long)a.Hd * a.Wd;
    if (a.stat_group_rows % hw != 0) return 0;
    g.dIPG = fs_make_div((int)(a.stat_group_rows / hw));
  }
  if (a.pro_group_imgs > 0) g.dPRG = fs_make_div(a.pro_group_imgs);
  const int npix = a.N * g.tiles_x * g.tiles_y, nco = a.Co_p / CO;
  int blocks = npix * nco;
  g.pix_major = (nco > 1 && a.src_bytes > 2 * a.wgt_bytes) ? 1 : 0;
  if (g.pix_major) blocks = 8 * ((npix + 7) / 8) * nco;
  else if (nco % 8 != 0 && 8 % nco == 0) { const int q = 8 / nco; blocks = 8 * ((npix + q - 1) / q); }
// ... 16 lines not shown
    blocks = d.nb0 + b1;
  }
  if (fs_conv3x3_plan_slot) {
    fs_conv3x3_plan_slot[0] = 1; fs_conv3x3_plan_slot[1] = blocks; fs_conv3x3_plan_slot[2] = PIX; fs_conv3x3_plan_slot[3] = CO;
    return FS_OK;
  }
  hipLaunchKernelGGL((conv3x3_t32_kernel<T, PIX, CO, EP, PRO>), dim3(blocks), dim3(256), pro_lds_bytes<PRO>(a), st, d);
  return fs_launch_status();
}

template <typename T, int EP, int PRO>
int t32_dispatch_cfg(const FsConvArgs& a, const FsConvArgs* b, int cfg, hipStream_t st) {
  switch (cfg) {
    case 1: return t32_launch<T, 128, 64, EP, PRO>(a, b, st);
    case 2: return t32_launch<T, 128, 32, EP, PRO>(a, b, st);
    default: return t32_launch<T, 256, 32, EP, PRO>(a, b, st);
  }
}

long t32_blocks(const FsConvArgs& a, int nimg, int PIX, int CO) {
  T32Geom g = t32_pick_geom(a.Hd, a.Wd, PIX, t32_hmax(PIX));
  if (g.TH == 0) return 0;
  return (long)nimg * g.tiles_x * g.tiles_y * (a.Co_p / CO);
}
double t32_waste(const FsConvArgs& a, int PIX) {
  T32Geom g = t32_pick_geom(a.Hd, a.Wd, PIX, t32_hmax(PIX));
  if (g.TH == 0) return 1e9;
  return (double)g.tiles_x * g.tiles_y * PIX / ((double)a.Hd * a.Wd);
}

int t32_pick_cfg(const FsConvArgs& a, int nimg) {
  if (a.force_impl >= 2 && a.force_impl <= 4) {
    const int c = a.force_impl - 1;
    return (a.Co_p % 64 != 0 && c == 1) ? 2 : c;
  }
  const bool big = t32_waste(a, 256) <= 1.15 * t32_waste(a, 128);
  if (big && t32_blocks(a, nimg, 256, 32) >= 512) return 3;
  return -1;
}

template <typename T, int PRO>
int t32_dispatch_ep(const FsConvArgs& a, const FsConvArgs* b, int cfg, hipStream_t st) {
  if constexpr (sizeof(T) == 2) {
    switch (t32_ep_mask(a)) {
      case EP_STATS: return t32_dispatch_cfg<T, EP_STATS, PRO>(a, b, cfg, st);
      case EP_BIAS | EP_STATS: return t32_dispatch_cfg<T, EP_BIAS | EP_STATS, PRO>(a, b, cfg, st);
      case EP_BIAS | EP_RELU: return t32_dispatch_cfg<T, EP_BIAS | EP_RELU, PRO>(a, b, cfg, st);
      case 0: return t32_dispatch_cfg<T, 0, PRO>(a, b, cfg, st);
      case EP_ADDEND: return t32_dispatch_cfg<T, EP_ADDEND, PRO>(a, b, cfg, st);
      case EP_MASK: return t32_dispatch_cfg<T, EP_MASK, PRO>(a, b, cfg, st);
      case EP_MASK | EP_BNB: return t32_dispatch_cfg<T, EP_MASK | EP_BNB, PRO>(a, b, cfg, st);
      case EP_ADDEND | EP_MASK | EP_BNB: return t32_dispatch_cfg<T, EP_ADDEND | EP_MASK | EP_BNB, PRO>(a, b, cfg, st);
      case EP_BNB | EP_MASKBN: return t32_dispatch_cfg<T, EP_BNB | EP_MASKBN, PRO>(a, b, cfg, st);
      default: break;
    }
  }
  return t32_dispatch_cfg<T, -1, PRO>(a, b, cfg, st);
}

template <typename T>
int t32_dispatch(const FsConvArgs& a, const FsConvArgs* b, hipStream_t st) {
  const int cfg = t32_pick_cfg(a, a.N + (b ? b->N : 0));
  if (cfg < 0) return FS_EINVAL;
  switch (a.pro_mode) {
    case 0: return t32_dispatch_ep<T, 0>(a, b, cfg, st);
    case 1: return t32_dispatch_ep<T, 1>(a, b, cfg, st);
    default: return FS_EINVAL;
  }
}

}

namespace {
bool t32_takes(const FsConvArgs& a, int dtype) {
  const int es = dtype == FS_DTYPE_BF16 ? 2 : 4;
  if ((a.Cs * es) % 64 != 0 || a.Co_p % 32 != 0 || a.Co % 8 != 0 || a.hb_mul != 1) return false;
  if (a.src_bytes >= 0x7ffff000LL) return false;
  if (a.bnb_scale && (!a.bnb_x || !a.bnb_shift || a.mask)) return false;
  if (a.bnb_x && !a.stats) return false;
  auto al16 = [&](const void* ptr, int64_t sn, int64_t sh, int64_t sw, int esz) {
    return ptr == nullptr || (((uintptr_t)ptr & 15u) == 0 && (sn * esz) % 16 == 0 && (sh * esz) % 16 == 0 && (sw * esz) % 16 == 0);
  };
  const int dsz = a.out_f32 ? 4 : es;
  if (!al16(a.dst, a.dN, a.dH, a.dW, dsz) || !al16(a.addend, a.aN, a.aH, a.aW, es) || !al16(a.mask, a.mN, a.mH, a.mW, es) ||
      !al16(a.bnb_x, a.dN, a.dH, a.dW, es))
    return false;
  const int64_t span = (int64_t)(a.N - 1) * a.dN + (int64_t)(a.Hd - 1) * a.dH + (int64_t)(a.Wd - 1) * a.dW + a.Co;
  if (a.dN < 0 || a.dH < 0 || a.dW < 0 || span >= 0x7fffffffLL) return false;
  return true;
}
}

int fs_conv3x3_t32(const FsConvArgs& a, const FsConvArgs* b, int dtype, hipStream_t st) {
  if (!t32_takes(a, dtype) || (b && !t32_takes(*b, dtype))) return FS_EINVAL;
  if (dtype == FS_DTYPE_BF16) return t32_dispatch<bf16>(a, b, st);
  if (dtype == FS_DTYPE_F32) return t32_dispatch<float>(a, b, st);
  return FS_EINVAL;
}
```

### fsnet_amd/csrc/conv_igemm.hip

```cpp
#include "common.h"
#include "fsnet_hip_internal.h"
#include <algorithm>

namespace {

template <int KG> __device__ __forceinline__ int lds_swz(int row) {
  return KG == 4 ? (((row >> 3) & 1) << 1) : ((row >> 1) & 7);
}

__device__ __forceinline__ uint4 buf_load16(__amdgpu_buffer_rsrc_t rsrc, int voff) {
  return __builtin_bit_cast(uint4, __builtin_amdgcn_raw_buffer_load_b128(rsrc, voff, 0, 0));
}

struct IgGeom { FsDiv dW, dH; };

template <typename T, int PIX, int CO, int WP, int KG>
__global__ __launch_bounds__(256) void conv_igemm_kernel(const FsDual<FsConvArgs, IgGeom> d) {
  const int prob = (int)blockIdx.x >= d.nb0 ? 1 : 0;
  const FsConvArgs& p = d.a[prob];
  const FsDiv dW = d.g[prob].dW, dH = d.g[prob].dH;
  const int bid = (int)blockIdx.x - (prob ? d.nb0 : 0);
  if ((int)blockIdx.z >= (p.grp_imgs > 0 ? p.N / p.grp_imgs : 1)) return;
  using TR = ElemTraits<T>;
  constexpr int WC = 4 / WP;
// ... 267 lines not shown
  const int npix = (a.M + PIX - 1) / PIX, nco = a.Co_p / CO;
  int blocks = npix * nco;
  if (nco % 8 != 0 && 8 % nco == 0) { const int g = 8 / nco; blocks = 8 * ((npix + g - 1) / g); }
  return blocks;
}

template <typename T, int PIX, int CO, int WP, int KG>
int launch_tile(const FsConvArgs& a, const FsConvArgs* b, hipStream_t st) {
  FsDual<FsConvArgs, IgGeom> d;
  d.a[0] = a; d.a[1] = b ? *b : a;
  d.g[0] = IgGeom{fs_make_div(a.Wd), fs_make_div(a.Hd)};
  d.g[1] = b ? IgGeom{fs_make_div(b->Wd), fs_make_div(b->Hd)} : d.g[0];
  d.nprob = b ? 2 : 1;
  int blocks = igemm_blocks<PIX, CO>(a);
  d.nb0 = blocks;
  int nz = a.grp_imgs > 0 ? a.N / a.grp_imgs : 1;
  if (b) {
    d.nb0 = fs_xcd_round(blocks);
    blocks = d.nb0 + igemm_blocks<PIX, CO>(*b);
    nz = std::max(nz, b->grp_imgs > 0 ? b->N / b->grp_imgs : 1);
  }
  hipLaunchKernelGGL((conv_igemm_kernel<T, PIX, CO, WP, KG>), dim3(blocks, a.ncls > 1 ? a.ncls : 1, nz), dim3(256), 0, st, d);
  return fs_launch_status();
}

template <typename T>
int launch_conv(const FsConvArgs& a, const FsConvArgs* b, hipStream_t st) {
  const int cop = a.Co_p;
  const bool k8 = a.kg == 8;
  auto rows = [](const FsConvArgs& q) { return (long)q.M * (q.grp_imgs > 0 ? q.N / q.grp_imgs : 1); };
  const long mtot = rows(a) + (b ? rows(*b) : 0);
  const long m128 = b ? (mtot + 127) / 128 : (long)((a.M + 127) / 128);
  if (cop % 128 == 0 && !k8) {
    long blocks = m128 * (cop / 128);
    if (blocks >= 512) return launch_tile<T, 128, 128, 2, 4>(a, b, st);
    return launch_tile<T, 64, 64, 2, 4>(a, b, st);
  }
  if (cop % 64 == 0) {
    long blocks = m128 * (cop / 64);
    if (blocks >= 512) return k8 ? launch_tile<T, 128, 64, 2, 8>(a, b, st) : launch_tile<T, 128, 64, 2, 4>(a, b, st);
    return k8 ? launch_tile<T, 64, 64, 2, 8>(a, b, st) : launch_tile<T, 64, 64, 2, 4>(a, b, st);
  }
  if (cop % 32 == 0) return k8 ? launch_tile<T, 128, 32, 4, 8>(a, b, st) : launch_tile<T, 128, 32, 4, 4>(a, b, st);
  if (cop % 16 == 0 && !k8) return launch_tile<T, 256, 16, 4, 4>(a, b, st);
  return FS_EINVAL;
}

}

namespace {
int igemm_check(const FsConvArgs* args) {
  if (!args || !args->src || !args->wgt || !args->dst || !args->ktab) return FS_EINVAL;
  if (args->kg != 4 && args->kg != 8) return FS_EINVAL;
  const int units = args->nchunks * (args->kg == 8 ? 2 : 4);
  if (args->nchunks <= 0 || units > 1024) return FS_EINVAL;
  if (args->Co % 4 != 0 || args->Co_p % 16 != 0) return FS_EINVAL;
  if (args->src_bytes <= 0 || args->src_bytes > 0x7fffffffLL || args->wgt_bytes <= 0 ||
      args->wgt_bytes > 0x7fffffffLL)
    return FS_EINVAL;
  if (args->dshift && ((args->sH | args->sW) & 1)) return FS_EINVAL;
  if (args->stats && args->stat_group_rows > 0 && args->stat_group_rows % 256 != 0) return FS_EINVAL;
  if (args->grp_imgs > 0 && (args->N <= 0 || args->N % args->grp_imgs != 0)) return FS_EINVAL;
  return FS_OK;
}
bool igemm_pairable(const FsConvArgs& a, const FsConvArgs& b) {
  return a.Co_p == b.Co_p && a.kg == b.kg && (a.ncls > 1 ? a.ncls : 1) == (b.ncls > 1 ? b.ncls : 1);
}
}

extern "C" int fs_conv_igemm2(const FsConvArgs* args, const FsConvArgs* a1, int dtype, void* stream) {
  int r = igemm_check(args);
  if (r != FS_OK) return r;
  if (a1) {
    r = igemm_check(a1);
    if (r != FS_OK) return r;
    if (!igemm_pairable(*args, *a1)) {
      r = fs_conv_igemm2(args, nullptr, dtype, stream);
      return r != FS_OK ? r : fs_conv_igemm2(a1, nullptr, dtype, stream);
    }
  }
  hipStream_t st = reinterpret_cast<hipStream_t>(stream);
  if (dtype == FS_DTYPE_BF16) return launch_conv<bf16>(*args, a1, st);
  if (dtype == FS_DTYPE_F32) return launch_conv<float>(*args, a1, st);
  return FS_EINVAL;
}

extern "C" int fs_conv_igemm(const FsConvArgs* args, int dtype, void* stream) {
  return fs_conv_igemm2(args, nullptr, dtype, stream);
}
```

### fsnet_amd/csrc/conv_stem.hip

```cpp
#include "common.h"
#include "fsnet_hip_internal.h"
#include <algorithm>

namespace {

constexpr int TY = 8, TX = 16;
constexpr int PH = 2 * TY + 5, PW = 2 * TX + 6;
constexpr int CO = 64, TAPS = 49;

__device__ __forceinline__ uint4 stem_load16(__amdgpu_buffer_rsrc_t rsrc, int voff) {
  return __builtin_bit_cast(uint4, __builtin_amdgcn_raw_buffer_load_b128(rsrc, voff, 0, 0));
}

struct StemFwdGeom { int tiles_x, tiles_y, ntiles, tiles_per_block; FsDiv dTX, dTY, dIPG; };

__global__ __launch_bounds__(256) void conv_stem_kernel(const FsDual<FsConvArgs, StemFwdGeom> d) {
  const int prob = (int)blockIdx.x >= d.nb0 ? 1 : 0;
  const FsConvArgs& p = d.a[prob];
  const int bid = (int)blockIdx.x - (prob ? d.nb0 : 0);
  const int tiles_x = d.g[prob].tiles_x, tiles_y = d.g[prob].tiles_y, ntiles = d.g[prob].ntiles;
  const int tiles_per_block = d.g[prob].tiles_per_block;
  const FsDiv dTX = d.g[prob].dTX, dTY = d.g[prob].dTY, dIPG = d.g[prob].dIPG;
  typedef bf16 T;
  __shared__ uint4 lds_w[CO * TAPS];
// ... 70 lines not shown
    f32x4 acc[4][2];
#pragma unroll
    for (int c = 0; c < 4; ++c)
#pragma unroll
      for (int b = 0; b < 2; ++b) acc[c][b] = f32x4{0.f, 0.f, 0.f, 0.f};
#pragma unroll
    for (int r = 0; r < 7; ++r)
#pragma unroll
      for (int j = 0; j < 2; ++j) {
        const int s = 4 * j + lg;
        uint4 fa[4], fb[2];
#pragma unroll
        for (int c = 0; c < 4; ++c) {
          const uint4 w = lds_w[(c * 16 + li) * TAPS + r * 7 + min(s, 6)];
          fa[c] = s < 7 ? w : make_uint4(0u, 0u, 0u, 0u);
        }
#pragma unroll
        for (int b = 0; b < 2; ++b) fb[b] = lds_x[(2 * (2 * wave + b) + r) * PW + 2 * li + s];
#pragma unroll
        for (int c = 0; c < 4; ++c)
#pragma unroll
          for (int b = 0; b < 2; ++b)
            acc[c][b] = __builtin_amdgcn_mfma_f32_16x16x32_bf16(__builtin_bit_cast(bf16x8, fa[c]),
                                                                __builtin_bit_cast(bf16x8, fb[b]), acc[c][b], 0, 0, 0);
      }

#pragma unroll
    for (int b = 0; b < 2; ++b) {
      const int y = y0 + 2 * wave + b, x = x0 + li;
      if (y < p.Hd && x < p.Wd) {
        T* d = reinterpret_cast<T*>(p.dst) + (long)n * p.dN + (long)y * p.dH + (long)x * p.dW;
#pragma unroll
        for (int c = 0; c < 4; ++c) {
          const int co = c * 16 + lg * 4;
          if (co < p.Co) {
            float v[4] = {acc[c][b][0], acc[c][b][1], acc[c][b][2], acc[c][b][3]};
            store4<T>(d + co, v);
#pragma unroll
            for (int j = 0; j < 4; ++j) { s1[c][j] += v[j]; s2[c][j] += v[j] * v[j]; }
          }
        }
      }
    }
  }
  if (p.stats && cur_group >= 0) flush_stats(cur_group);
}

}

namespace {
int stem_check(const FsConvArgs* a, int dtype) {
  if (!a || !a->src || !a->wgt || !a->dst) return FS_EINVAL;
  if (dtype != FS_DTYPE_BF16 || a->Cs != 8 || a->Co != 64 || a->Co_p != 64) return FS_EINVAL;
  if (a->bias || a->addend || a->mask || a->bnb_x || a->relu || a->out_f32 || a->grp_imgs || a->ncls > 1) return FS_EINVAL;
  if (a->Hd != (a->Hs + 6 - 7) / 2 + 1 || a->Wd != (a->Ws + 6 - 7) / 2 + 1 || a->N <= 0) return FS_EINVAL;
  if (a->nchunks * a->kg * 8 < TAPS * 8) return FS_EINVAL;
  if (a->src_bytes <= 0 || a->src_bytes > 0x7fffffffLL || a->wgt_bytes <= 0 || a->wgt_bytes > 0x7fffffffLL)
    return FS_EINVAL;
  if ((long)a->N * ((a->Wd + TX - 1) / TX) * ((a->Hd + TY - 1) / TY) > 0x7fffffffL) return FS_EINVAL;
  if (a->stat_group_rows > 0 && a->stat_group_rows % ((long)a->Hd * a->Wd) != 0) return FS_EINVAL;
  return FS_OK;
}
int stem_geom(const FsConvArgs& a, long total, StemFwdGeom& g) {
  g.tiles_x = (a.Wd + TX - 1) / TX; g.tiles_y = (a.Hd + TY - 1) / TY;
  g.ntiles = (int)((long)a.N * g.tiles_x * g.tiles_y);
  g.tiles_per_block = (int)std::max<long>(1, (total + 511) / 512);
  g.dTX = fs_make_div(g.tiles_x); g.dTY = fs_make_div(g.tiles_y);
  g.dIPG = a.stat_group_rows > 0 ? fs_make_div((int)(a.stat_group_rows / ((long)a.Hd * a.Wd))) : fs_make_div(1);
  return (g.ntiles + g.tiles_per_block - 1) / g.tiles_per_block;
}
}

extern "C" int fs_conv_stem2(const FsConvArgs* a, const FsConvArgs* a1, int dtype, void* stream) {
  int r = stem_check(a, dtype);
  if (r != FS_OK) return r;
  if (a1 && (r = stem_check(a1, dtype)) != FS_OK) return r;
  FsDual<FsConvArgs, StemFwdGeom> d;
  d.a[0] = *a; d.a[1] = a1 ? *a1 : *a;
  d.nprob = a1 ? 2 : 1;
  auto tiles = [](const FsConvArgs& q) { return (long)q.N * ((q.Wd + TX - 1) / TX) * ((q.Hd + TY - 1) / TY); };
  const long total = tiles(*a) + (a1 ? tiles(*a1) : 0);
  int blocks = stem_geom(*a, total, d.g[0]);
  d.g[1] = d.g[0];
  d.nb0 = blocks;
  if (a1) blocks += stem_geom(*a1, total, d.g[1]);
  hipLaunchKernelGGL(conv_stem_kernel, dim3(blocks), dim3(256), 0, reinterpret_cast<hipStream_t>(stream), d);
  return fs_launch_status();
}

extern "C" int fs_conv_stem(const FsConvArgs* a, int dtype, void* stream) { return fs_conv_stem2(a, nullptr, dtype, stream); }
```

### fsnet_amd/csrc/fsnet_hip_internal.h

```cpp
#pragma once
#include "../../include/fsnet_hip.h"
inline thread_local int32_t* fs_conv3x3_plan_slot = nullptr;

template <typename A, typename G>
struct FsDual {
  A a[2];
  G g[2];
  int nb0;
  int nprob;
};
struct FsNoGeom { int unused; };
inline int fs_xcd_round(long blocks) { return (int)((blocks + 7) / 8 * 8); }

int fs_conv1x1_gemm(const FsConvArgs& a, hipStream_t st);
```

### fsnet_amd/csrc/t32_common.h

```cpp
#pragma once
#include "common.h"
#include "fsnet_hip_internal.h"
#include <algorithm>
#include <cstdlib>

namespace {

typedef __attribute__((ext_vector_type(16))) float f32x16;

__device__ __forceinline__ uint4 t32_load16(__amdgpu_buffer_rsrc_t rsrc, int voff) {
  return __builtin_bit_cast(uint4, __builtin_amdgcn_raw_buffer_load_b128(rsrc, voff, 0, 0));
}

__device__ __forceinline__ void t32_barrier() {
  asm volatile("s_waitcnt lgkmcnt(0)" ::: "memory");
  __builtin_amdgcn_s_barrier();
  asm volatile("" ::: "memory");
}
__device__ __forceinline__ void t32_wave_sync() { asm volatile("s_waitcnt lgkmcnt(0)" ::: "memory"); }

struct T32Geom {
  int TH, TW;
  int tiles_x, tiles_y;
  unsigned mTW, mHW;
// ... 81 lines not shown
struct T32Item { int n, y0, x0, co0, px; };

template <int NR, int NM, int K = 0>
__device__ __forceinline__ void t32_sched_step() {
  if constexpr (K < NR) {
    __builtin_amdgcn_sched_group_barrier(0x100, 1, 0);
    constexpr int m = (NM * (K + 1)) / NR - (NM * K) / NR;
    if constexpr (m > 0) __builtin_amdgcn_sched_group_barrier(0x008, m, 0);
    t32_sched_step<NR, NM, K + 1>();
  }
}

inline T32Geom t32_pick_geom(int Hd, int Wd, int PIX, int hmax) {
  T32Geom best{};
  double best_cost = 1e30;
  for (int tw = std::min(4, Wd); tw <= std::min(Wd, 64); ++tw) {
    const int th = std::min(PIX / tw, Hd);
    if (th < 1 || (th + 2) * (tw + 2) > hmax) continue;
    const int tx = (Wd + tw - 1) / tw, ty = (Hd + th - 1) / th;
    const double waste = (double)tx * ty * PIX / ((double)Hd * Wd);
    const double halo = (double)(th + 2) * (tw + 2) / ((double)th * tw);
    double cost = waste * (1.0 + 0.15 * halo);
    if (tw % 32 != 0 && tw != Wd) cost *= 1.02;
    if (cost < best_cost - 1e-9) { best_cost = cost; best.TH = th; best.TW = tw; best.tiles_x = tx; best.tiles_y = ty; }
  }
  if (best.TW > 0) {
    best.mTW = fs_div_magic(best.TW); best.mHW = fs_div_magic(best.TW + 2);
    best.dTX = fs_make_div(best.tiles_x); best.dTY = fs_make_div(best.tiles_y);
  }
  return best;
}

inline int t32_cu_count() {
  static const int n = [] {
    int dev = 0, cus = 256;
    if (hipGetDevice(&dev) == hipSuccess) {
      hipDeviceProp_t pr;
      if (hipGetDeviceProperties(&pr, dev) == hipSuccess && pr.multiProcessorCount > 0) cus = pr.multiProcessorCount;
    }
    return cus;
  }();
  return n;
}

inline int t32_ep_mask(const FsConvArgs& a) {
  int m = 0;
  if (a.bias) m |= EP_BIAS;
  if (a.addend) m |= EP_ADDEND;
  if (a.relu) m |= EP_RELU;
  if (a.mask) m |= EP_MASK;
  if (a.bnb_x) m |= EP_BNB;
  else if (a.stats) m |= EP_STATS;
  if (a.out_f32) m |= EP_F32;
  if (a.bnb_x && a.bnb_scale) m |= EP_MASKBN;
  return m;
}

}
```

### fsnet_amd/csrc/version.hip

```cpp
#include "common.h"
#include "fsnet_hip_internal.h"
extern "C" int fs_abi_version(void) { return FS_ABI_VERSION; }
extern "C" const char* fs_target_arch(void) { return "gfx950"; }

namespace {
__global__ void timestamp_kernel(unsigned long long* slot) { *slot = wall_clock64(); }
}
extern "C" int fs_debug_timestamp(void* slot, void* stream) {
  if (!slot) return FS_EINVAL;
  hipLaunchKernelGGL(timestamp_kernel, dim3(1), dim3(1), 0, (hipStream_t)stream, (unsigned long long*)slot);
  return fs_launch_status();
}

extern "C" int fs_capture_position(void* stream, unsigned long long* token) {
  if (!token) return FS_EINVAL;
  *token = 0;
  hipStreamCaptureStatus status = hipStreamCaptureStatusNone;
  unsigned long long id = 0;
  hipGraph_t graph = nullptr;
  const hipGraphNode_t* deps = nullptr;
  size_t n = 0;
  hipError_t e = hipStreamGetCaptureInfo_v2((hipStream_t)stream, &status, &id, &graph, &deps, &n);
  if (e != hipSuccess) { (void)hipGetLastError(); return FS_ELAUNCH; }
  if (status != hipStreamCaptureStatusActive) return FS_OK;
  unsigned long long h = 0x9e3779b97f4a7c15ull ^ (unsigned long long)n;
  for (size_t i = 0; i < n; ++i) {
    unsigned long long x = (unsigned long long)(uintptr_t)deps[i];
    x ^= x >> 33; x *= 0xff51afd7ed558ccdull; x ^= x >> 33; x *= 0xc4ceb9fe1a85ec53ull; x ^= x >> 33;
    h += x;
  }
  *token = h ? h : 1;
  return FS_OK;
}
```

### fsnet_amd/engine/nets.py

```python
import os
import weakref

import torch

from ..hip import ops
from ..hip.binding import raw_stream
from ..hip.conv import ConvOp, run_specs
from .runtime import RT, grad_of

STAT_SLOTS = ops.STAT_SLOTS
FOLD_BN = os.environ.get("FSNET_AMD_BN_FOLD", "1").strip().lower() not in ("0", "off", "false", "no")


class StatsPool:

    def __init__(self, device, capacity=1 << 21):
        self.buf = torch.zeros(capacity, dtype=torch.float64, device=device)
        self.off = 0
        self.high = 0
        self.dirty = False
        self.epoch = -1
        ops.register_prezero(self, StatsPool._prezero, device)

    def _prezero(self):
# ... 488 lines not shown
    def accumulate_param_grads(self, op, dc, x, pro=None):
        gw = grad_of(self.m.weight)
        gb = grad_of(self.m.bias) if self.m.bias is not None else None
        if gw is None:
            if gb is not None:
                ops.channel_sum(dc, gb, self.m.bias.numel())
            return
        item = (op, dc, x, gw, gb, self.m.bias.numel() if gb is not None else 0, pro)
        if _TAIL_SINK[0] is not None:
            _TAIL_SINK[0].append(item)
            return
        mode = RT.wgrad_streams if (dc.is_cuda and RT.overlap and (RT.dp is None or RT.dp.wgrad_companions)) else 0
        if mode:
            _defer_param_grads(_current_stream(dc.device), item)
            return
        _run_param_grads(*item, bias_later=_inline_bias_list(dc.device))


def bn_tensors(bn):
    c = bn.__dict__.get("_fs_tensors")
    w = bn.weight
    if c is None or c[0] != w.data_ptr() or c[1] != bn.running_mean.data_ptr():
        d = {"weight": w.data, "bias": bn.bias.data, "running_mean": bn.running_mean,
             "running_var": bn.running_var, "num_batches_tracked": bn.num_batches_tracked}
        c = (w.data_ptr(), bn.running_mean.data_ptr(), d)
        bn.__dict__["_fs_tensors"] = c
    return c[2]


def _dp_stats(stats):
    if RT.dp is not None:
        RT.dp.allreduce_small(stats)
        return RT.dp.world
    return 1


_BWD_POOLS = {}


def bwd_pool_reset(device):
    key = (device, raw_stream(device.index))
    p = _BWD_POOLS.get(key)
    if p is None:
        p = _BWD_POOLS[key] = StatsPool(device)
    if p.epoch != ops.PREZERO_EPOCH[0]:
        p.reset()
    return p


def _bwd_sums(c, st):
    return _BWD_POOLS[(c.device, raw_stream(c.device.index))].take(c.shape[-1], st.groups)


def _bn_bwd(dout, y, c, bn, st, H, W, relu=True, fold=False, g_out=None, sums=None):
    dc = torch.empty_like(c)
    reduced = sums is not None
    if sums is None:
        sums = _bwd_sums(c, st)
    sync = RT.dp is not None and st.count != float("inf")
    ops.bn_backward(dout, y, c, bn.weight.data, st, dc, grad_of(bn.weight), grad_of(bn.bias), H, W, relu=relu,
                    fold=fold, g_out=g_out, sums=sums, sums_zeroed=True, reduced=reduced,
                    allreduce=(RT.dp.allreduce_small if sync else None))
    return dc


def _check_train_bn(bn, what):
    if not bn.training:
        raise NotImplementedError(
            "%s: BatchNorm in eval mode inside a training step is only implemented for the ResNet encoders "
            "(norm_eval / frozen_stages); the reference has no such switch for this module" % what)


def _exchange(pool, tensors, out_of_place=False):
    if RT.dp is None:
        return 1, list(tensors)
    base = pool.buf.untyped_storage().data_ptr() if pool is not None else None
    idx = [i for i, t in enumerate(tensors) if t is not None]
    inside = [i for i in idx if base is not None and tensors[i].untyped_storage().data_ptr() == base]
    res = list(tensors)
    runs, cur = [], []
    for i in sorted(inside, key=lambda i: tensors[i].storage_offset()):
        if cur and tensors[cur[-1]].storage_offset() + tensors[cur[-1]].numel() == tensors[i].storage_offset():
            cur.append(i)
        else:
            if cur:
                runs.append(cur)
            cur = [i]
    if cur:
        runs.append(cur)
    for run in runs:
        lo = tensors[run[0]].storage_offset()
        hi = tensors[run[-1]].storage_offset() + tensors[run[-1]].numel()
        view = pool.buf[lo:hi]
        if out_of_place:
            out = torch.empty_like(view)
            RT.dp.allreduce_small(view, out=out)
            for i in run:
                o = tensors[i].storage_offset() - lo
                res[i] = out[o:o + tensors[i].numel()].view(tensors[i].shape)
        else:
            RT.dp.allreduce_small(view)
    for i in idx:
        if i in inside:
            continue
        if out_of_place:
            res[i] = torch.empty_like(tensors[i])
            RT.dp.allreduce_small(tensors[i], out=res[i])
        else:
            RT.dp.allreduce_small(tensors[i])
    return RT.dp.world, res


class ResNetRunner:

    def __init__(self, module):
# ... 511 lines not shown
                depth = inv if scale is None else inv * scale
                lv["sig"] = (u, depth)
                outs[i] = (lv["logits"], depth, u)
            return outs, ctx
        if sc:
            heads = ops.depth_head_fwd_multi([ctx["lv"][i]["logits"] for i in sc], m.depth_bins, K, m.min_depth,
                                             m.max_depth, P2=P2, base_fx=base_fx)
            for i, (depth, disp) in zip(sc, heads):
                lv = ctx["lv"][i]
                outs[i] = (lv["logits"], depth, disp) + ((lv["unc"],) if "unc" in lv else ())
        return outs, ctx

    def backward(self, ctx, g_depth, g_disp, g_unc=None):
        g_unc = g_unc or {}
        m = self.m
        feats = ctx["feats"]
        dev, dt = feats[-1].device, feats[-1].dtype
        K = int(m.num_output_channels)
        gfeats = [None] * 5
        bwd_pool_reset(dev)
        chain_begins(dev)
        RT.mark("ddec.bwd.start")
        tail = RT.dp is not None and RT.dp.decoder_tail and RT.overlap and dev.type == "cuda" and \
            torch._C._current_graph_task_id() >= 0
        if tail:
            _TAIL_SINK[0] = []
        try:
            return self._backward(ctx, g_depth, g_disp, g_unc, gfeats, dev, dt, K)
        finally:
            items, _TAIL_SINK[0] = _TAIL_SINK[0], None
            if items:
                defer_to_tail(items, self, dev)

    def _backward(self, ctx, g_depth, g_disp, g_unc, gfeats, dev, dt, K):
        m = self.m
        feats = ctx["feats"]

        sc = [i for i in range(5) if i in m.scales and (g_depth.get(i) is not None or g_disp.get(i) is not None)]
        dls = {}
        if sc and getattr(m, "sigmoid_head", False):
            a, bq = 1.0 / float(m.max_depth), 1.0 / float(m.min_depth) - 1.0 / float(m.max_depth)
            for i in sc:
                u, depth = ctx["lv"][i]["sig"]
                du = g_disp[i] if g_disp.get(i) is not None else torch.zeros_like(u)
                if g_depth.get(i) is not None:
                    du = du - g_depth[i] * depth * (bq / (a + bq * u))
                dls[i] = ops.sigmoid_head_bwd(u, du, self.disp[i].ready(dt, dev).Co_p, dt)
        elif sc:
            res = ops.depth_head_bwd_multi([ctx["lv"][i]["logits"] for i in sc], m.depth_bins,
                                           [g_depth.get(i) for i in sc], [g_disp.get(i) for i in sc], K, m.min_depth,
                                           m.max_depth, dt, P2=ctx["P2"], base_fx=ctx["base_fx"])
            dls = dict(zip(sc, res))

        def disp_grad(i):
            lv = ctx["lv"][i]
            y1p = lv["y1p"]
            G = None
            if i in dls:
                cld = self.disp[i]
                opd = cld.ready(dt, dev)
                dl = dls[i]
                cld.accumulate_param_grads(opd, dl, y1p)
                G = opd.dgrad(dl, y1p.shape[1], y1p.shape[2])
            if i in self.unc and g_unc.get(i) is not None:
                clu = self.unc[i]
                opu = clu.ready(dt, dev)
                dlu = ops.sigmoid_head_bwd(lv["unc"], g_unc[i], opu.Co_p, dt)
                clu.accumulate_param_grads(opu, dlu, y1p)
                G = opu.dgrad(dlu, y1p.shape[1], y1p.shape[2], addend=G)
            if G is not None:
                return G, False
            key = (tuple(y1p.shape), y1p.dtype, y1p.device)
            if self._border0 is None or self._border0[0] != key:
                self._border0 = (key, torch.zeros_like(y1p))
            return self._border0[1], True

        Gp, _ = disp_grad(0)
        for i in range(0, 5):
            issue_advanced(dev)
            lv = ctx["lv"][i]
            h, w = lv["h"], lv["w"]
            H2, W2 = 2 * h, 2 * w
            cl1, bn1 = self.up1[i]
            op1 = cl1.ready(dt, dev)
            y1_int = lv["y1p"][:, 1:-1, 1:-1]
            dc1 = _bn_bwd(Gp, y1_int, lv["c1"], bn1, lv["s1"], H2, W2, relu=True, fold=True)
            cl1.accumulate_param_grads(op1, dc1, lv["xcat"])
            dxcat = op1.dgrad(dc1, H2 + 2, W2 + 2)
            cl0, bn0 = self.up0[i]
            op0 = cl0.ready(dt, dev)
            sums0 = _bwd_sums(lv["c0"], lv["s0"])
            d_y0, d_skip = ops.upcat_pad_bwd(dxcat, h, w, op0.Co_p, lv["Cs"], bn=(lv["y0"], lv["c0"], lv["s0"], sums0))
            if i > 0 and lv["Cs"]:
                gfeats[i - 1] = d_skip
            dc0 = _bn_bwd(d_y0, None, lv["c0"], bn0, lv["s0"], h, w, sums=sums0)
            cl0.accumulate_param_grads(op0, dc0, lv["x"])
            if i < 4:
                Gp, fresh = disp_grad(i + 1)
                interior = Gp[:, 1:-1, 1:-1]
                op0.dgrad(dc0, h, w, out=interior, addend=None if fresh else interior)
            else:
                gfeats[4] = op0.dgrad(dc0, h, w)
        RT.mark("ddec.bwd.end")
        flush_deferred(_current_stream())
        return gfeats


class PoseDecoderRunner:
    def __init__(self, module):
        self.m = module
        self.cl = [ConvLayer(module.convs["squeeze"]), ConvLayer(module.convs[("pose", 0)]),
                   ConvLayer(module.convs[("pose", 1)]), ConvLayer(module.convs[("pose", 2)])]

    def forward(self, feat, invert):
        dt, dev = feat.dtype, feat.device
        acts = [feat]
        x = feat
        for j in range(3):
            op = self.cl[j].ready(dt, dev)
            x = op.forward(x, bias=self.cl[j].bias, relu=True)
            acts.append(x)
        op = self.cl[3].ready(dt, dev)
        x3 = op.forward(x, bias=self.cl[3].bias, out_f32=True)
        nf = int(self.m.num_frames_to_predict_for)
        if isinstance(invert, tuple):
            G = len(invert)
            B = x3.shape[0] // G
            outs = [ops.pose_tail_fwd(x3[g * B:(g + 1) * B], nf, invert[g]) for g in range(G)]
            aa, tr, T = (tuple(o[i] for o in outs) for i in range(3))
        else:
            aa, tr, T = ops.pose_tail_fwd(x3, nf, invert)
        return aa, tr, T, {"acts": acts, "x3": x3, "invert": invert, "nf": nf}

    def backward(self, ctx, dT):
        acts, x3 = ctx["acts"], ctx["x3"]
        dt, dev = acts[0].dtype, acts[0].device
        chain_begins(dev)
        RT.mark("pdec.bwd.start")
        if isinstance(ctx["invert"], tuple):
            G = len(ctx["invert"])
            B = x3.shape[0] // G
            d = torch.empty(x3.shape, dtype=dt, device=dev)
            for g in range(G):
                ops.pose_tail_bwd(x3[g * B:(g + 1) * B], dT[g], ctx["nf"], ctx["invert"][g], dt, out=d[g * B:(g + 1) * B])
        else:
            d = ops.pose_tail_bwd(x3, dT, ctx["nf"], ctx["invert"], dt)
        for j in range(3, -1, -1):
            op = self.cl[j].ready(dt, dev)
            xin = acts[j]
            self.cl[j].accumulate_param_grads(op, d, xin)
            d = op.dgrad(d, xin.shape[1], xin.shape[2], mask=(xin if j > 0 else None))
        if RT.lanes:
            flush_deferred(_current_stream())
# ... 2 lines not shown
```

### fsnet_amd/engine/runtime.py

```python
import os

import torch


class _Runtime:
    def __init__(self):
        name = os.environ.get("FSNET_AMD_DTYPE", "bf16").lower()
        self.compute_dtype = {"bf16": torch.bfloat16, "bfloat16": torch.bfloat16, "fp32": torch.float32,
                              "float32": torch.float32}[name]
        self.weights_epoch = 0
        self.dp = None
        self.noise_step = 0
        self.tie_noise = os.environ.get("FSNET_AMD_TIE_NOISE", "1") != "0"
        self.overlap = True
        self.wgrad_streams = 2
        self.wgrad_flush = 8
        self.even_chains = False
        self.wgrad_flush_even = 4
        self.wgrad_balance = 1
        self.wgrad_late = True
        self._nop = {}
        self.stem_flush = False
        self.batch_pose_pairs = True
        self._lanes_env = os.environ.get("FSNET_AMD_LANES", "auto").lower()
        self._lanes = self._lanes_env not in ("0", "auto")
        self._lanes_override = None
        self.stem_flush = self._lanes
        self.pack_overlap = True
        self._side = {}
        self._held = {}
        self._marks = {} if os.environ.get("FSNET_AMD_MARKS", "0") != "0" else None
        self._mark_buf = None

    @property
    def lanes(self):
        return self._lanes

    @lanes.setter
    def lanes(self, v):
        self._lanes_override = None
        if isinstance(v, str) and v.lower() == "auto":
            self._lanes_env, self._lanes = "auto", False
        else:
            self._lanes_env, self._lanes = ("1" if v else "0"), bool(v)
        self.stem_flush = self._lanes

    @property
    def lanes_auto(self):
        return self._lanes_env == "auto"

    @property
    def encoder_pass_ms(self):
        return getattr(self.dp, "encoder_pass_ms", None)

    @encoder_pass_ms.setter
    def encoder_pass_ms(self, v):
        self.dp.encoder_pass_ms = v

    def override_lanes(self, v):
        self._lanes_override = None if v is None else bool(v)
        self.resolve_lanes()

    def resolve_lanes(self):
        if self._lanes_env == "auto":
            if self._lanes_override is not None and self.dp is not None:
                self._lanes = self._lanes_override
            else:
                import torch.distributed as dist
                multi = self.dp is not None or (dist.is_available() and dist.is_initialized() and dist.get_world_size() > 1)
                self._lanes = bool(multi)
            self.stem_flush = self._lanes
        return self._lanes

    def mark(self, name):
        if self._marks is None or not torch.cuda.is_available():
            return
        from ..hip.binding import check, lib, stream_ptr
        if self._mark_buf is None:
            self._mark_buf = torch.zeros(512, dtype=torch.int64, device="cuda")
        idx = self._marks.get(name)
        if idx is None:
# ... 173 lines not shown
```

### fsnet_amd/hip/binding.py

```python
import ctypes as C
import os

_HERE = os.path.dirname(os.path.abspath(__file__))
LIB_PATH = os.path.join(os.path.dirname(_HERE), "lib", "libfsnet_hip.so")

FS_DTYPE_F32 = 0
FS_DTYPE_BF16 = 1


class FsError(RuntimeError):
    pass


class FsConvArgs(C.Structure):
    _fields_ = [
        ("src", C.c_void_p), ("wgt", C.c_void_p), ("dst", C.c_void_p), ("bias", C.c_void_p),
        ("addend", C.c_void_p), ("mask", C.c_void_p), ("stats", C.c_void_p), ("ktab", C.c_void_p),
        ("sN", C.c_int64), ("sH", C.c_int64), ("sW", C.c_int64),
        ("dN", C.c_int64), ("dH", C.c_int64), ("dW", C.c_int64),
        ("aN", C.c_int64), ("aH", C.c_int64), ("aW", C.c_int64),
        ("mN", C.c_int64), ("mH", C.c_int64), ("mW", C.c_int64),
        ("src_bytes", C.c_int64), ("wgt_bytes", C.c_int64),
        ("Hs", C.c_int32), ("Ws", C.c_int32), ("Hd", C.c_int32), ("Wd", C.c_int32),
        ("M", C.c_int32), ("Co", C.c_int32), ("Co_p", C.c_int32), ("nchunks", C.c_int32), ("kg", C.c_int32),
        ("hb_mul", C.c_int32), ("hb_add", C.c_int32), ("sgn", C.c_int32), ("dshift", C.c_int32),
        ("relu", C.c_int32), ("out_f32", C.c_int32), ("N", C.c_int32), ("Cs", C.c_int32),
        ("wgt_row_bytes", C.c_int64),
        ("grp_imgs", C.c_int32), ("ncls", C.c_int32), ("cls_nch", C.c_int32 * 4), ("cls_ktab_off", C.c_int32 * 4), ("cls_wgt_off", C.c_int64 * 4),
        ("bnb_x", C.c_void_p), ("bnb_mean", C.c_void_p), ("bnb_invstd", C.c_void_p),
        ("stat_group_rows", C.c_int32),
        ("pro_a", C.c_void_p), ("pro_b", C.c_void_p), ("pro_c", C.c_void_p), ("pro_m", C.c_void_p), ("pro_src2", C.c_void_p),
        ("pro_mode", C.c_int32), ("pro_relu", C.c_int32), ("pro_group_imgs", C.c_int32), ("force_impl", C.c_int32),
        ("bnb_scale", C.c_void_p), ("bnb_shift", C.c_void_p),
        ("pro_stats", C.c_void_p), ("pro_stats_local", C.c_void_p),
        ("pro_gamma", C.c_void_p), ("pro_beta", C.c_void_p),
        ("pro_mean", C.c_void_p), ("pro_invstd", C.c_void_p),
        ("pro_save_a", C.c_void_p), ("pro_save_b", C.c_void_p),
        ("pro_running_mean", C.c_void_p), ("pro_running_var", C.c_void_p),
        ("pro_nbt", C.c_void_p),
        ("pro_dgamma", C.c_void_p), ("pro_dbeta", C.c_void_p),
        ("pro_dst", C.c_void_p),
        ("pro_count", C.c_double), ("pro_eps", C.c_float), ("pro_momentum", C.c_float),
        ("ds_src", C.c_void_p), ("ds_wgt", C.c_void_p), ("ds_wgt_row_bytes", C.c_int64),
    ]


class FsWgradArgs(C.Structure):
    _fields_ = [
        ("dy", C.c_void_p), ("x", C.c_void_p), ("dw", C.c_void_p), ("ktab", C.c_void_p),
        ("sN", C.c_int64), ("sH", C.c_int64), ("sW", C.c_int64),
        ("Hs", C.c_int32), ("Ws", C.c_int32), ("Hd", C.c_int32), ("Wd", C.c_int32),
        ("M", C.c_int32), ("Cd", C.c_int32),
        ("Co", C.c_int32), ("Ci", C.c_int32), ("R", C.c_int32), ("S", C.c_int32),
        ("stride", C.c_int32), ("pad", C.c_int32), ("ncolgroups", C.c_int32),
        ("workspace", C.c_void_p), ("workspace_elems", C.c_int64), ("x_bytes", C.c_int64), ("use_halo", C.c_int32),
        ("pix_per_split", C.c_int32), ("nsplit", C.c_int32), ("ws_rows", C.c_int32), ("ws_cols", C.c_int32),
        ("pro_a", C.c_void_p), ("pro_b", C.c_void_p), ("pro_relu", C.c_int32), ("pro_group_imgs", C.c_int32),
    ]


class FsPackDesc(C.Structure):
    _fields_ = [
        ("w", C.c_void_p), ("dst_f", C.c_void_p), ("dst_d", C.c_void_p),
        ("k_f", C.c_int64), ("k_d", C.c_int64), ("block_start", C.c_int64),
        ("Co", C.c_int32), ("Ci", C.c_int32), ("R", C.c_int32), ("S", C.c_int32),
        ("rows_f", C.c_int32), ("cs_f", C.c_int32), ("rows_d", C.c_int32), ("cs_d", C.c_int32),
        ("tap_order_d", C.c_int32),
    ]


class FsAugArgs(C.Structure):
    _fields_ = [
        ("src", C.c_void_p), ("minv", C.c_void_p), ("iplan", C.c_void_p), ("fplan", C.c_void_p),
        ("image", C.c_void_p), ("original", C.c_void_p), ("mask", C.c_void_p),
        ("mean", C.c_float * 3), ("std", C.c_float * 3),
        ("B", C.c_int32), ("F", C.c_int32), ("Hs", C.c_int32), ("Ws", C.c_int32), ("H", C.c_int32), ("W", C.c_int32),
    ]


class FsHeadBatch(C.Structure):
    _fields_ = [
        ("logits", C.c_void_p * 4), ("depth", C.c_void_p * 4), ("disp", C.c_void_p * 4),
        ("d_depth", C.c_void_p * 4), ("d_disp", C.c_void_p * 4), ("dlogits", C.c_void_p * 4),
        ("M", C.c_int64 * 4), ("n", C.c_int32), ("nimg", C.c_int32), ("P2", C.c_void_p), ("base_fx", C.c_float),
        ("reserved", C.c_int32),
    ]


class FsResizeArgs(C.Structure):
    _fields_ = [
        ("src", C.c_void_p), ("dims", C.c_void_p), ("image", C.c_void_p),
        ("mean", C.c_float * 3), ("std", C.c_float * 3),
        ("B", C.c_int32), ("F", C.c_int32), ("Hs", C.c_int32), ("Ws", C.c_int32), ("H", C.c_int32), ("W", C.c_int32),
        ("iplan", C.c_void_p), ("fplan", C.c_void_p), ("original", C.c_void_p), ("mask", C.c_void_p),
    ]

# ... 57 lines not shown

class FsPostOptArgs(C.Structure):
    _fields_ = [
        ("image", C.c_void_p), ("depth", C.c_void_p), ("vo", C.c_void_p), ("centres", C.c_void_p),
        ("out", C.c_void_p), ("labels", C.c_void_p), ("nseg", C.c_void_p),
        ("workspace", C.c_void_p), ("workspace_bytes", C.c_int64),
        ("rgb_mean", C.c_double * 3), ("rgb_std", C.c_double * 3),
        ("lab_dist_weight", C.c_float), ("depth_dist_weight", C.c_float), ("image_dist_weight", C.c_float),
        ("lambda0", C.c_double), ("lambda1", C.c_double), ("lambda2", C.c_double),
        ("B", C.c_int32), ("H", C.c_int32), ("W", C.c_int32), ("K", C.c_int32), ("iter_num", C.c_int32),
        ("max_points", C.c_int32),
    ]


class FsFlowArgs(C.Structure):
    _fields_ = [
        ("img0", C.c_void_p), ("img1", C.c_void_p), ("flow", C.c_void_p),
        ("workspace", C.c_void_p), ("workspace_bytes", C.c_int64),
        ("pyr_scale", C.c_double), ("poly_sigma", C.c_double),
        ("B", C.c_int32), ("H", C.c_int32), ("W", C.c_int32), ("levels", C.c_int32), ("winsize", C.c_int32),
        ("iterations", C.c_int32), ("poly_n", C.c_int32), ("flags", C.c_int32),
    ]


class FsMotionMaskArgs(C.Structure):
    _fields_ = [
        ("flow", C.c_void_p), ("P2", C.c_void_p), ("pose", C.c_void_p), ("mask", C.c_void_p),
        ("threshold", C.c_float), ("mode", C.c_int32),
        ("B", C.c_int32), ("H", C.c_int32), ("W", C.c_int32),
    ]


ABI_VERSION = 15
_lib = None


def load_library(path=None):
    global _lib
    if _lib is not None:
        return _lib
    path = path or os.environ.get("FSNET_HIP_LIB", LIB_PATH)
    import torch
    if not os.path.exists(path):
        raise FsError(
            "libfsnet_hip.so not found at %s — the HIP kernel library is required (no CPU fallback). "
            "Build it with `python fsnet_amd/csrc/build.py` or __graft_entry__.build()." % path)
    handle = C.CDLL(path)
    from . import signatures
    signatures.declare(handle)
    got = int(handle.fs_abi_version())
    if got != ABI_VERSION:
        raise FsError("libfsnet_hip.so at %s reports ABI %d, this binding is written against ABI %d (FS_ABI_VERSION "
                      "in include/fsnet_hip.h): rebuild it with `python fsnet_amd/csrc/build.py`" % (path, got, ABI_VERSION))
    _lib = handle
    return _lib


class _LazyLib:
    def __getattr__(self, name):
        return getattr(load_library(), name)


lib = _LazyLib()


def check(status, what=""):
    if status != 0:
        raise FsError("libfsnet_hip call %s failed with status %d" % (what, status))


def raw_stream(device_index=None):
    import torch
    if device_index is None:
        device_index = torch._C._cuda_getDevice()
    return torch._C._cuda_getCurrentRawStream(device_index)


def stream_ptr():
    return C.c_void_p(raw_stream())
```

### fsnet_amd/hip/conv.py

```python
import ctypes as C

import numpy as np
import torch

from .binding import lib, check, stream_ptr, raw_stream, FsConvArgs, FsWgradArgs, FS_DTYPE_BF16, FS_DTYPE_F32


class LaunchProfile:
    active = False
    records = []

    @classmethod
    def begin(cls):
        cls.active, cls.records = True, []

    @classmethod
    def end(cls):
        cls.active = False
        torch.cuda.synchronize()
        out = [(k, f, s.elapsed_time(e) * 1e-3) for (k, f, s, e, _) in cls.records]
        cls.tagged = [(k, f, s.elapsed_time(e) * 1e-3, t) for (k, f, s, e, t) in cls.records]
        cls.records = []
        return out

# ... 384 lines not shown
        eb = dy.element_size()
        tab, offs, nchs = self._class_tables(*_nhwc_strides(dy)[1:])
        o = out[:, 0::2, 0::2]
        a = FsConvArgs()
        a.src, a.dst, a.wgt = dy.data_ptr(), o.data_ptr(), self.w_d.data_ptr()
        a.wgt_row_bytes = self.kd_p * eb
        a.wgt_bytes = (self.rows_d - 1) * self.kd_p * eb + (4 if self.R == 3 else 1) * self.Co_p * eb
        a.sN, a.sH, a.sW = _nhwc_strides(dy)
        a.ktab = tab.data_ptr()
        a.src_bytes = _span_bytes(dy)
        a.dN, a.dH, a.dW = _nhwc_strides(o)
        if addend is not None:
            ad = addend[:, 0::2, 0::2]
            a.addend = ad.data_ptr()
            a.aN, a.aH, a.aW = _nhwc_strides(ad)
        if mask is not None:
            mk = mask[:, 0::2, 0::2]
            a.mask = mk.data_ptr()
            a.mN, a.mH, a.mW = _nhwc_strides(mk)
        a.Hs, a.Ws, a.Hd, a.Wd = Ho, Wo, H // 2, W // 2
        a.M = N * (H // 2) * (W // 2)
        a.Co, a.Co_p, a.nchunks, a.kg = out.shape[3], self.rows_d, max(nchs), self.kg_d
        a.hb_mul, a.hb_add, a.sgn, a.dshift = 1, 0, 1, 0
        a.N, a.Cs = N, self.Co_p
        a.ncls = 4
        for k, ((py, px), taps) in enumerate(self._classes()):
            assert k == 2 * py + px
            a.cls_nch[k], a.cls_ktab_off[k] = nchs[k], min(offs[k], 0 if not taps else offs[k])
            a.cls_wgt_off[k] = taps[0][0] * self.Co_p * eb if taps else 0
        if bn_fuse is not None:
            c, st, sums = bn_fuse
            a.bnb_x = c.data_ptr()
            a.bnb_mean, a.bnb_invstd = st.mean.data_ptr(), st.invstd.data_ptr()
            a.stats = sums.data_ptr()
            a.stat_group_rows = (N // st.groups) * (H // 2) * (W // 2) if st.groups > 1 else 0
        flops = 2.0 * N * Ho * Wo * self.Co * self.R * self.S * self.Ci
        if ds is not None:
            ds_op, dc_ds = ds
            assert self.can_fold_ds_dgrad(ds_op, dy, dc_ds) and out.is_contiguous()
            assert (addend is None or addend.is_contiguous()) and (mask is None or mask.is_contiguous())
            a.ds_src, a.ds_wgt, a.ds_wgt_row_bytes = dc_ds.data_ptr(), ds_op.w_d.data_ptr(), ds_op.kd_p * eb
            flops += 2.0 * N * Ho * Wo * self.Co * self.Ci
            return Spec(["conv3x3_s2d"], a, self.code, "conv3x3_s2d", flops,
                        lambda: "dgrd %s + 1x1/s2 dy[%d,%d,%d,%d]" % (self.describe(), N, Ho, Wo, Cd), out, "conv_dgrad_s2")
        return Spec(["conv3x3_s2d", "conv_igemm"] if self.s2d else ["conv_igemm"], a, self.code,
                    "conv3x3_s2d" if self.s2d else "conv_igemm", flops,
                    lambda: "dgrd %s dy[%d,%d,%d,%d]" % (self.describe(), N, Ho, Wo, Cd), out, "conv_dgrad_s2")

    def dgrad(self, dy, H, W, **kw):
        sp = self.dgrad_spec(dy, H, W, **kw)
        run_specs([sp])
        return sp.out

    def dgrad_spec(self, dy, H, W, out=None, addend=None, mask=None, bn_fuse=None, mask_bn=False, ds=None):
        N, Ho, Wo, Cd = dy.shape
        assert Cd == self.Co_p and dy.dtype == self.dtype and self.need_dgrad
        if out is None:
            out = torch.empty(N, H, W, self.Ci_p, dtype=self.dtype, device=dy.device)
        if bn_fuse is not None:
            c, st, _ = bn_fuse
            assert c.is_contiguous() and out.is_contiguous() and c.shape == out.shape and c.dtype == self.dtype
            assert self.can_fuse_bn_bwd(N, H, W, st.groups)
        if self.s2_classes:
            if H % 2 or W % 2 or H != 2 * Ho or W != 2 * Wo:
                raise NotImplementedError("stride-2 3x3 data gradient expects an even input size (%dx%d)" % (H, W))
            return self._dgrad_s2_classes(dy, H, W, out, addend, mask, bn_fuse, ds)
        if self.s2_classes_1x1 and ds is None and H % 2 == 0 and W % 2 == 0 and H == 2 * Ho and W == 2 * Wo and not mask_bn:
            return self._dgrad_s2_classes(dy, H, W, out, addend, mask, bn_fuse, None)
        assert ds is None
        a = FsConvArgs()
        a.src, a.wgt, a.dst = dy.data_ptr(), self.w_d.data_ptr(), out.data_ptr()
        a.bias, a.stats = None, None
        a.addend = addend.data_ptr() if addend is not None else None
        a.sN, a.sH, a.sW = _nhwc_strides(dy)
        a.ktab = self._table("d", a.sH, a.sW).data_ptr()
        a.src_bytes, a.wgt_bytes = _span_bytes(dy), self.w_d.numel() * self.w_d.element_size()
        a.dN, a.dH, a.dW = _nhwc_strides(out)
        if addend is not None:
            a.aN, a.aH, a.aW = _nhwc_strides(addend)
        if mask is not None:
            a.mask = mask.data_ptr()
            a.mN, a.mH, a.mW = _nhwc_strides(mask)
        a.Hs, a.Ws, a.Hd, a.Wd = Ho, Wo, H, W
        a.M = N * H * W
        a.Co, a.Co_p, a.nchunks, a.kg = out.shape[3], self.rows_d, self.nch_d, self.kg_d
        a.hb_mul, a.hb_add, a.sgn, a.dshift = 1, self.pad, -1, (1 if self.stride == 2 else 0)
        a.relu, a.out_f32 = 0, 0
        a.N, a.Cs = N, self.Co_p
        if bn_fuse is not None:
            c, st, sums = bn_fuse
            a.bnb_x, a.bnb_mean, a.bnb_invstd = c.data_ptr(), st.mean.data_ptr(), st.invstd.data_ptr()
            a.stats = sums.data_ptr()
            a.stat_group_rows = (N // st.groups) * H * W if st.groups > 1 else 0
            if mask_bn:
                assert mask is None and st.scale is not None and self.halo_d
                a.bnb_scale, a.bnb_shift = st.scale.data_ptr(), st.shift.data_ptr()
        else:
            assert not mask_bn
        flops = 2.0 * N * Ho * Wo * self.Co * self.R * self.S * self.Ci
        halo = self.halo_d
        tag = lambda: "dgrd %s dy[%d,%d,%d,%d]" % (self.describe(), N, Ho, Wo, Cd)
        if self._wants_1x1(a):
            return Spec(["conv1x1", "conv_igemm"], a, self.code, "conv1x1", flops, tag, out, "conv_dgrad")
        if halo:
            a.force_impl = FORCE_3X3
            return Spec(["conv3x3_halo"], a, self.code, lambda other: self._kind3x3(a, other), flops, tag, out, "conv_dgrad")
        return Spec(["conv_igemm"], a, self.code, "conv_igemm", flops, tag, out, "conv_dgrad")

    def describe(self):
        return "%dx%d/s%d p%d %d->%d" % (self.R, self.S, self.stride, self.pad, self.Ci, self.Co)

    def wgrad(self, dy, x, dw, pro=None):
        run_specs([self.wgrad_spec(dy, x, dw, pro=pro)])
        return dw

    def wgrad_spec(self, dy, x, dw, pro=None):
        N, Ho, Wo, Cd = dy.shape
        assert dy.is_contiguous() and Cd == self.Co_p and x.shape[3] == self.Ci_p
        assert dw.dtype == torch.float32 and dw.is_contiguous()
        a = FsWgradArgs()
        a.dy, a.x, a.dw, a.ktab = dy.data_ptr(), x.data_ptr(), dw.data_ptr(), self.ktab_w.data_ptr()
        a.sN, a.sH, a.sW = _nhwc_strides(x)
        a.Hs, a.Ws, a.Hd, a.Wd = x.shape[1], x.shape[2], Ho, Wo
        a.M, a.Cd = N * Ho * Wo, Cd
        a.Co, a.Ci, a.R, a.S = self.Co, self.Ci, self.R, self.S
        a.stride, a.pad, a.ncolgroups, a.pix_per_split = self.stride, self.pad, self.ncolgroups, 0
        ws = wgrad_workspace(dy.device)
        a.workspace, a.workspace_elems = ws.data_ptr(), ws.numel()
        a.x_bytes, a.use_halo = _span_bytes(x), 1
        if pro is not None:
            pst, prelu = pro
            a.pro_a, a.pro_b, a.pro_relu = pst.scale.data_ptr(), pst.shift.data_ptr(), int(prelu)
            a.pro_group_imgs = N // pst.groups if pst.groups > 1 else 0
        flops = 2.0 * a.M * self.Co * self.R * self.S * self.Ci
        return Spec(["conv_wgrad"], a, self.code, "conv_wgrad", flops,
                    lambda: "wgrd %s dy[%d,%d,%d,%d]" % (self.describe(), N, Ho, Wo, Cd), dw, "conv_wgrad")
```

### fsnet_amd/hip/ops.py

```python
import ctypes as C
import os

import torch

from .binding import (lib, check, stream_ptr, FsBnApplyArgs, FsBnBwdArgs, FsFlowArgs, FsMotionMaskArgs, FsPhotoArgs,
                      FsPostOptArgs, FsSmoothArgs)
from .conv import dtype_code, _timed, BN_EPS, BN_MOMENTUM, Spec, run_specs

STAT_SLOTS = 8


def _p(t):
    return t.data_ptr() if t is not None else None


def nchw_to_nhwc(a, b, cp, dtype, out=None):
    a = a.contiguous()
    N, Ca, H, W = a.shape
    Cb = 0
    if b is not None:
        b = b.contiguous()
        Cb = b.shape[1]
    if out is None:
        out = torch.empty(N, H, W, cp, dtype=dtype, device=a.device)
# ... 31 lines not shown
    check(lib.fs_bn_finalize(C.byref(a), st.scale.data_ptr(), st.shift.data_ptr(), stream_ptr()), "bn_finalize")
    return st


def bn_apply(x, stats, bn, st, y, H, W, count, **kw):
    run_specs([bn_apply_spec(x, stats, bn, st, y, H, W, count, **kw)])
    return y


def bn_apply_spec(x, stats, bn, st, y, H, W, count, relu=True, pad_out=False, res=None, stats2=None, bn2=None, st2=None,
                  track=True, groups=1, pool=None):
    a = FsBnApplyArgs()
    a.groups = groups
    assert st.groups == groups and (st2 is None or st2.groups == groups)
    Cc = x.shape[-1]
    a.x, a.res, a.y = x.data_ptr(), _p(res), _p(y)
    if pool is not None:
        assert pool[0].is_contiguous() and pool[1].is_contiguous() and pool[0].shape == (x.shape[0], H // 2, W // 2, Cc)
        assert stats is not None and res is None and bn2 is None and not pad_out and H % 2 == 0 and W % 2 == 0
        a.pool_y, a.pool_idx = pool[0].data_ptr(), pool[1].data_ptr()
    else:
        assert y is not None
    a.stats, a.stats2 = _p(stats), _p(stats2)
    a.gamma, a.beta = bn["weight"].data_ptr(), bn["bias"].data_ptr()
    if track or stats is None:
        a.running_mean, a.running_var = bn["running_mean"].data_ptr(), bn["running_var"].data_ptr()
        a.num_batches_tracked = bn["num_batches_tracked"].data_ptr()
    a.save_mean, a.save_invstd = st.mean.data_ptr(), st.invstd.data_ptr()
    st.count = float(count)
    if bn2 is not None:
        a.gamma2, a.beta2 = bn2["weight"].data_ptr(), bn2["bias"].data_ptr()
        if track or stats2 is None:
            a.running_mean2, a.running_var2 = bn2["running_mean"].data_ptr(), bn2["running_var"].data_ptr()
            a.num_batches_tracked2 = bn2["num_batches_tracked"].data_ptr() if track else None
        a.save_mean2, a.save_invstd2 = st2.mean.data_ptr(), st2.invstd.data_ptr()
        st2.count = float(count)
    a.count, a.eps, a.momentum = float(count), BN_EPS, BN_MOMENTUM
    if pad_out:
        assert y.shape[1] == H + 2 and y.shape[2] == W + 2
    if y is not None:
        a.yN, a.yH, a.yW = y.stride(0), y.stride(1), y.stride(2)
    a.M, a.C, a.H, a.W = x.shape[0] * H * W, Cc, H, W
    a.relu, a.pad_out = int(relu), int(pad_out)
    nb = x.numel() * x.element_size() * (1 + (y is not None) + (res is not None))
    if pool is not None:
        nb += pool[0].numel() * pool[0].element_size() + pool[1].numel()
    return Spec(["bn_apply"], a, dtype_code(x.dtype), "bn_apply_pool" if pool is not None else "bn_apply", nb,
                lambda: "[%d,%d,%d,%d]%s%s%s" % (x.shape[0], H, W, Cc, " +res" if res is not None else "",
                                                 " pad" if pad_out else "", " +pool" if pool is not None else ""),
                y, "bn_apply")


def bn_backward(dout, y, x, gamma, st, dx, dgamma, dbeta, H, W, relu=True, fold=False, g_out=None, sums=None,
                allreduce=None, sums_zeroed=False, reduced=False, phase="all", glob=None, pool=None):
    bn_backward_multi([dict(dout=dout, y=y, x=x, gamma=gamma, st=st, dx=dx, dgamma=dgamma, dbeta=dbeta, H=H, W=W, relu=relu,
                            fold=fold, g_out=g_out, sums=sums, sums_zeroed=sums_zeroed, reduced=reduced, glob=glob, pool=pool)],
                      allreduce=allreduce, phase=phase)
    return None if phase == "reduce" else dx


def _bn_bwd_call(dout, y, x, gamma, st, dx, dgamma, dbeta, H, W, relu=True, fold=False, g_out=None, sums=None,
                 sums_zeroed=False, reduced=False, glob=None, pool=None):
    if reduced:
        assert sums is not None and not fold and g_out is None
        relu, y = False, None
    Cc = x.shape[-1]
    a = FsBnBwdArgs()
    if sums is None:
        sums = torch.zeros(st.groups * STAT_SLOTS, 2, Cc, dtype=torch.float64, device=x.device)
    elif not sums_zeroed and not reduced:
        sums.zero_()
    a.dout, a.y, a.x, a.dx, a.g_out = _p(dout), _p(y), x.data_ptr(), _p(dx), _p(g_out)
    if pool is not None:
        assert not reduced and not fold and g_out is None and pool[0].is_contiguous() and pool[1].is_contiguous()
        assert (dout is None or dout.is_contiguous()) and (y is None or y.is_contiguous())
        a.pool_dy, a.pool_idx, a.beta = pool[0].data_ptr(), pool[1].data_ptr(), pool[2].data_ptr()
    else:
        assert dout is not None
    a.sums = sums.data_ptr()
    a.gamma, a.save_mean, a.save_invstd = gamma.data_ptr(), st.mean.data_ptr(), st.invstd.data_ptr()
    a.dgamma, a.dbeta = _p(dgamma), _p(dbeta)
    a.count = st.count
    a.groups = st.groups
    if dout is not None:
        a.gN, a.gH, a.gW = dout.stride(0), dout.stride(1), dout.stride(2)
    if y is not None:
        a.yN, a.yH, a.yW = y.stride(0), y.stride(1), y.stride(2)
    a.M, a.C, a.H, a.W = x.shape[0] * H * W, Cc, H, W
    a.relu, a.fold = int(relu), int(fold)
    shape = (x.shape[0], H, W, Cc)
    return dict(a=a, code=dtype_code(x.dtype), nb=x.numel() * x.element_size(), sums=sums, reduced=reduced, glob=glob,
                has_y=y is not None, has_g=g_out is not None, has_dout=dout is not None,
                shp=lambda: "[%d,%d,%d,%d]%s%s" % (shape + (" fold" if fold else "", " pool" if pool is not None else "")))


def bn_backward_multi(calls, allreduce=None, phase="all", span=None):
    cs = [_bn_bwd_call(**c) for c in calls]
    if phase != "apply":
        run_specs([Spec(["bn_bwd_reduce"], c["a"], c["code"], "bn_bwd_reduce", c["nb"] * (1 + c["has_dout"] + c["has_y"]), c["shp"], None,
                        "bn_bwd_reduce") for c in cs if not c["reduced"]])
    if phase == "reduce":
        return
    pending = [c for c in cs if c["glob"] is None] if allreduce is not None else []
    if len(pending) == 2 and span is not None:
        both = span(pending[0]["sums"], pending[1]["sums"])
        if both is not None:
            out = torch.empty_like(both)
            allreduce(both, out=out)
            n0 = pending[0]["sums"].numel()
            pending[0]["glob"] = out[:n0].view(pending[0]["sums"].shape)
            pending[1]["glob"] = out[n0:].view(pending[1]["sums"].shape)
            pending = []
    for c in pending:
        c["glob"] = torch.empty_like(c["sums"])
        allreduce(c["sums"], out=c["glob"])
    for c in cs:
        if c["glob"] is not None:
            c["a"].sums_local, c["a"].sums = c["sums"].data_ptr(), c["glob"].data_ptr()
    run_specs([Spec(["bn_bwd_apply"], c["a"], c["code"], "bn_bwd_apply", c["nb"] * (2 + c["has_dout"] + c["has_y"] + c["has_g"]), c["shp"],
                    None, "bn_bwd_apply") for c in cs])


def maxpool_fwd(x):
    return maxpool_fwd_multi([x])[0]


def maxpool_fwd_multi(xs):
    outs = []
    for x in xs:
        N, H, W, Cc = x.shape
        Ho, Wo = (H - 1) // 2 + 1, (W - 1) // 2 + 1
# ... 773 lines not shown
```

### fsnet_amd/hip/signatures.py

```python
import ctypes as C

P = C.c_void_p
I = C.c_int
L = C.c_int64
F = C.c_float
D = C.c_double

SIGNATURES = {
    "fs_abi_version": (C.c_int, []),
    "fs_target_arch": (C.c_char_p, []),
    "fs_debug_timestamp": (C.c_int, [P, P]),
    "fs_capture_position": (C.c_int, [P, P]),
    "fs_conv_igemm": (C.c_int, [P, I, P]),
    "fs_conv_igemm2": (C.c_int, [P, P, I, P]),
    "fs_conv3x3_halo2": (C.c_int, [P, P, I, P]),
    "fs_conv3x3_halo2_plan": (C.c_int, [P, P, I, P]),
    "fs_conv3x3_s2d": (C.c_int, [P, I, P]),
    "fs_conv3x3_s2d2": (C.c_int, [P, P, I, P]),
    "fs_conv_stem2": (C.c_int, [P, P, I, P]),
    "fs_conv_wgrad2": (C.c_int, [P, P, I, P]),
    "fs_conv_wgrad2_plan": (C.c_int, [P, P, I, P]),
    "fs_bn_apply2": (C.c_int, [P, P, I, P]),
    "fs_bn_bwd_reduce2": (C.c_int, [P, P, I, P]),
    "fs_bn_bwd_apply2": (C.c_int, [P, P, I, P]),
    "fs_maxpool_fwd2": (C.c_int, [P, P, P, I, P, P, P, I, I, I, I, I, P]),
    "fs_maxpool_bwd2": (C.c_int, [P, P, P, P, I, P, P, P, P, I, I, I, I, I, P]),
    "fs_conv3x3_halo": (C.c_int, [P, I, P]),
    "fs_conv3x3_halo_plan": (C.c_int, [P, I, P]),
    "fs_conv1x1": (C.c_int, [P, I, P]),
    "fs_conv_stem": (C.c_int, [P, I, P]),
    "fs_conv_wgrad": (C.c_int, [P, I, P]),
    "fs_conv_wgrad_plan": (C.c_int, [P, I, P]),
    "fs_pack_weights": (C.c_int, [P, P, I, I, I, I, I, I, L, I, I, P]),
    "fs_sigmoid_head_fwd": (C.c_int, [P, P, L, I, P]),
    "fs_sigmoid_head_bwd": (C.c_int, [P, P, P, L, I, I, P]),
    "fs_distill_fwd": (C.c_int, [P, P, P, L, P, P]),
    "fs_distill_bwd": (C.c_int, [P, P, P, L, P, P, P, P]),
    "fs_resize_linear": (C.c_int, [P, P, I, I, I, I, I, P]),
    "fs_depth_eval": (C.c_int, [P, P, I, I, I, I, I, P, P, P]),
    "fs_depth_eval_masked": (C.c_int, [P, P, P, I, I, I, I, I, F, F, I, P, P, P]),
    "fs_lidar_mei_depth": (C.c_int, [P, P, L, P, P, I, I, I, P, P, P, L, P]),
    "fs_lidar_mei_depth_workspace_bytes": (C.c_int64, [I, I, I]),
    "fs_lidar_pinhole_depth": (C.c_int, [P, P, L, P, I, I, I, P, P, L, P]),
    "fs_lidar_pinhole_depth_workspace_bytes": (C.c_int64, [I, I, I]),
    "fs_postopt": (C.c_int, [P, P]),
    "fs_postopt_workspace_bytes": (C.c_int64, [I, I, I, I]),
    "fs_optflow_farneback": (C.c_int, [P, P]),
    "fs_optflow_workspace_bytes": (C.c_int64, [P]),
    "fs_optflow_level_image": (C.c_int, [P, I, P, P]),
    "fs_motion_mask": (C.c_int, [P, P]),
    "fs_augment_masks": (C.c_int, [P, P, P, P, P, I, I, I, I, I, P]),
    "fs_copy_multi": (C.c_int, [P, P, P, I, P]),
    "fs_zero_multi": (C.c_int, [P, P, I, P]),
    "fs_pack_tile_blocks": (C.c_int64, [C.c_int, C.c_int, C.c_int, C.c_int]),
    "fs_pack_weights_multi": (C.c_int, [P, I, L, I, P]),
    "fs_nchw_to_nhwc": (C.c_int, [P, P, P, I, I, I, I, I, I, I, P]),
    "fs_bn_apply": (C.c_int, [P, I, P]),
    "fs_bn_finalize": (C.c_int, [P, P, P, P]),
    "fs_bn_bwd_reduce": (C.c_int, [P, I, P]),
    "fs_bn_bwd_apply": (C.c_int, [P, I, P]),
    "fs_maxpool_fwd": (C.c_int, [P, P, P, I, I, I, I, I, P]),
    "fs_maxpool_bwd": (C.c_int, [P, P, P, P, I, I, I, I, I, P]),
# ... 39 lines not shown
```

### include/fsnet_hip.h

```cpp
#ifndef FSNET_HIP_H
#define FSNET_HIP_H
#include <stdint.h>

#ifdef __cplusplus
extern "C" {
#endif

#define FS_OK 0
#define FS_EINVAL 1
#define FS_ELAUNCH 2

#define FS_DTYPE_F32 0
#define FS_DTYPE_BF16 1

#define FS_STAT_SLOTS 8

#define FS_ABI_VERSION 15
int fs_abi_version(void);
const char* fs_target_arch(void);
int fs_debug_timestamp(void* slot, void* stream);
int fs_capture_position(void* stream, unsigned long long* token);

typedef struct FsConvArgs {
  const void* src;
  const void* wgt;
  void* dst;
  const float* bias;
  const void* addend;
  const void* mask;
  double* stats;
  const int* ktab;
  int64_t sN, sH, sW;
  int64_t dN, dH, dW;
  int64_t aN, aH, aW;
  int64_t mN, mH, mW;
  int64_t src_bytes;
  int64_t wgt_bytes;
  int32_t Hs, Ws;
  int32_t Hd, Wd;
  int32_t M;
  int32_t Co;
  int32_t Co_p;
  int32_t nchunks;
  int32_t kg;
  int32_t hb_mul, hb_add, sgn, dshift;
  int32_t relu;
  int32_t out_f32;
  int32_t N;
  int32_t Cs;
  int64_t wgt_row_bytes;
  int32_t grp_imgs;
  int32_t ncls;
  int32_t cls_nch[4];
  int32_t cls_ktab_off[4];
  int64_t cls_wgt_off[4];
  const void* bnb_x;
  const float* bnb_mean; const float* bnb_invstd;
  int32_t stat_group_rows;
  const float* pro_a; const float* pro_b; const float* pro_c; const float* pro_m;
  const void* pro_src2;
  int32_t pro_mode, pro_relu, pro_group_imgs;
  int32_t force_impl;
  const float* bnb_scale; const float* bnb_shift;
  const double* pro_stats; const double* pro_stats_local;
  const float* pro_gamma; const float* pro_beta;
  float* pro_mean; float* pro_invstd;
  float* pro_save_a; float* pro_save_b;
  float* pro_running_mean; float* pro_running_var;
  int64_t* pro_nbt;
  float* pro_dgamma; float* pro_dbeta;
  void* pro_dst;
  double pro_count;
  float pro_eps, pro_momentum;
  const void* ds_src; const void* ds_wgt;
  int64_t ds_wgt_row_bytes;
} FsConvArgs;
int fs_conv_igemm(const FsConvArgs* args, int dtype, void* stream);

int fs_conv_igemm2(const FsConvArgs* a0, const FsConvArgs* a1, int dtype, void* stream);
int fs_conv1x1(const FsConvArgs* args, int dtype, void* stream);

int fs_conv3x3_halo(const FsConvArgs* args, int dtype, void* stream);
int fs_conv3x3_halo_plan(const FsConvArgs* args, int dtype, int32_t* plan);
int fs_conv3x3_halo2(const FsConvArgs* a0, const FsConvArgs* a1, int dtype, void* stream);
int fs_conv3x3_halo2_plan(const FsConvArgs* a0, const FsConvArgs* a1, int dtype, int32_t* plan);

int fs_conv3x3_s2d(const FsConvArgs* args, int dtype, void* stream);
int fs_conv3x3_s2d2(const FsConvArgs* a0, const FsConvArgs* a1, int dtype, void* stream);

int fs_conv_stem(const FsConvArgs* args, int dtype, void* stream);
int fs_conv_stem2(const FsConvArgs* a0, const FsConvArgs* a1, int dtype, void* stream);

typedef struct FsWgradArgs {
  const void* dy;
  const void* x;
  float* dw;
  const int* ktab;
  int64_t sN, sH, sW;
  int32_t Hs, Ws;
  int32_t Hd, Wd;
  int32_t M;
  int32_t Cd;
  int32_t Co, Ci, R, S;
  int32_t stride, pad;
  int32_t ncolgroups;
  float* workspace;
  int64_t workspace_elems;
  int64_t x_bytes;
  int32_t use_halo;
  int32_t pix_per_split, nsplit, ws_rows, ws_cols;
  const float* pro_a; const float* pro_b;
  int32_t pro_relu, pro_group_imgs;
} FsWgradArgs;
int fs_conv_wgrad(const FsWgradArgs* args, int dtype, void* stream);
int fs_conv_wgrad_plan(const FsWgradArgs* args, int dtype, int32_t* plan);
int fs_conv_wgrad2(const FsWgradArgs* a0, const FsWgradArgs* a1, int dtype, void* stream);
int fs_conv_wgrad2_plan(const FsWgradArgs* a0, const FsWgradArgs* a1, int dtype, int32_t* plan);

int fs_pack_weights(const float* w_oihw, void* dst, int Co, int Ci, int R, int S, int rows_p,
                    int cs_p, int64_t ktot_p, int transpose, int dtype, void* stream);

typedef struct FsPackDesc {
  const float* w;
  void* dst_f;
  void* dst_d;
  int64_t k_f, k_d;
  int64_t block_start;
  int32_t Co, Ci, R, S;
// ... 275 lines not shown
```

Baseline: 2292 samples/s.

## Fold depth-decoder BN backward sums into padded 3x3 dgrad epilogue

Extends the 3x3 dgrad kernels (halo, p1, t32) with an external-BN epilogue. It reads the BN input through its own strides and a padding window, rebuilds the ReLU mask from gamma, beta, mean and invstd, and accumulates the BN backward sums while the gradient is still in registers. The BN backward apply kernel can then rebuild the ReLU mask from x and beta instead of reading the stored output y. The intent is to drop a separate reduction pass and the y read for decoder BN layers behind padding or reflection convs, at the cost of extra epilogue work, more register pressure and a larger FsConvArgs ABI. It is enabled by default through ddec_bn1_fold.

```diff
diff --git a/fsnet_amd/csrc/bn.hip b/fsnet_amd/csrc/bn.hip
--- a/fsnet_amd/csrc/bn.hip
+++ b/fsnet_amd/csrc/bn.hip
@@ -357,7 +357,7 @@
   if (!p.fold && p.gW == p.C && p.gH == (long)p.W * p.C && p.gN == hw * p.C &&
       (!p.relu || (p.yW == p.C && p.yH == (long)p.W * p.C && p.yN == hw * p.C))) {
     loadv<T>(dout + m * p.C + c, g);
-    if (p.relu) {
+    if (p.relu && yv) {
       float yy[V];
       loadv<T>(yv + m * p.C + c, yy);
 #pragma unroll
@@ -368,7 +368,7 @@
   int w, h; long n;
   split_row(m, p.H, p.W, n, h, w);
   load_dout<T>(p, dout, n, h, w, c, g);
-  if (p.relu) {
+  if (p.relu && yv) {
     float yy[V];
     loadv<T>(yv + n * p.yN + (long)h * p.yH + (long)w * p.yW + c, yy);
 #pragma unroll
@@ -719,6 +719,7 @@
   const int SC = SCG * V, c0 = (int)blockIdx.y * SC;
   float* s_a = bn_smem; float* s_b = bn_smem + SC; float* s_k = bn_smem + 2 * SC;
   float* s_mean = bn_smem + 3 * SC; float* s_istd = bn_smem + 4 * SC;
+  const bool xmask = !POOL && p.relu && !p.y && p.beta;
   const int G = p.groups > 1 ? p.groups : 1;
   const int z = (int)blockIdx.z - (prob ? d.nb0 : 0);
   const int Mg = p.M / G;
@@ -749,7 +750,7 @@
     float istd = p.save_invstd[z * C + c];
     s_mean[cl] = p.save_mean[z * C + c]; s_istd[cl] = istd;
     s_k[cl] = p.gamma[c] * istd;
-    if constexpr (POOL) bn_smem[5 * SC + cl] = (p.beta ? p.beta[c] : 0.f) - s_mean[cl] * s_k[cl];
+    if (POOL || xmask) bn_smem[5 * SC + cl] = (p.beta ? p.beta[c] : 0.f) - s_mean[cl] * s_k[cl];
     s_a[cl] = (float)(sg / p.count);
     s_b[cl] = (float)(sgx / p.count);
     if (blockIdx.x == 0) {
@@ -768,7 +769,7 @@
   const long stride = (long)gridDim.x * 256;
   if constexpr (!POOL) {
     const long hw = (long)p.H * p.W;
-    const bool plain = fast && !p.fold && scg_sh >= 0 && p.gW == C && p.gH == (long)p.W * C && p.gN == hw * C &&
+    const bool plain = fast && !p.fold && !xmask && scg_sh >= 0 && p.gW == C && p.gH == (long)p.W * C && p.gN == hw * C &&
                        (!p.relu || (p.yW == C && p.yH == (long)p.W * C && p.yN == hw * C));
     if (plain) {
       if (i0 >= total) return;
@@ -836,6 +837,7 @@
       loadv<T>(xv + m2 * C + c0 + cg2 * V, px);
     }
     if constexpr (POOL) pool_mask<T>(p, yv, m, c, xr, s_k + cl, bn_smem + 5 * SC + cl, g);
+    else if (xmask) pool_mask<T>(p, nullptr, m, c, xr, s_k + cl, bn_smem + 5 * SC + cl, g);
 #pragma unroll
     for (int j = 0; j < V; ++j) {
       float xh = (xr[j] - s_mean[cl + j]) * s_istd[cl + j];
@@ -903,7 +905,7 @@
     if (a->y && !(a->yW == a->C && a->yH == (long)a->W * a->C && a->yN == hw * a->C)) return FS_EINVAL;
     return FS_OK;
   }
-  if (a->relu && !a->y) return FS_EINVAL;
+  if (a->relu && !a->y && !(apply && a->beta)) return FS_EINVAL;
   return FS_OK;
 }
 template <typename A>
@@ -1023,7 +1025,8 @@
   if (b) items = std::max(items, (long)(b->M / G1) * (b->C / vec));
   const int nslab = a->pool_dy ? 1 : bn_slabs(a->C / vec);
   dim3 grid(std::min(grid_for(items / nslab), std::max(32, grid_for(1L << 40) / nslab)), nslab, G + G1);
-  const unsigned lds = (a->pool_dy ? 6u : 5u) * (a->C / nslab) * sizeof(float);
+  auto xmask = [](const FsBnBwdArgs* q) { return q && q->relu && !q->y && q->beta; };
+  const unsigned lds = ((a->pool_dy || xmask(a) || xmask(b)) ? 6u : 5u) * (a->C / nslab) * sizeof(float);
   const FsDual<FsBnBwdArgs, FsNoGeom> d = bn_dual(a, b);
   const int fast = 1;
   if (a->pool_dy && bn_pool_quads(a->C / vec)) {
diff --git a/fsnet_amd/csrc/common.h b/fsnet_amd/csrc/common.h
--- a/fsnet_amd/csrc/common.h
+++ b/fsnet_amd/csrc/common.h
@@ -61,6 +61,13 @@
 template <> __device__ inline void store4<bf16>(bf16* p, const float v[4]) {
   uint2 t; t.x = pack_bf16x2(v[0], v[1]); t.y = pack_bf16x2(v[2], v[3]);
   *reinterpret_cast<uint2*>(p) = t;
+}
+template <typename T> __device__ inline void round4(const float v[4], float q[4]);
+template <> __device__ inline void round4<float>(const float v[4], float q[4]) { q[0] = v[0]; q[1] = v[1]; q[2] = v[2]; q[3] = v[3]; }
+template <> __device__ inline void round4<bf16>(const float v[4], float q[4]) {
+  const uint32_t a = pack_bf16x2(v[0], v[1]), b = pack_bf16x2(v[2], v[3]);
+  q[0] = bf16_bits_to_f(a & 0xffffu); q[1] = bf16_bits_to_f(a >> 16);
+  q[2] = bf16_bits_to_f(b & 0xffffu); q[3] = bf16_bits_to_f(b >> 16);
 }
 
 __host__ __device__ static inline unsigned fs_div_magic(int d) { return (1u << 20) / (unsigned)d + 1u; }
diff --git a/fsnet_amd/csrc/conv1x1.hip b/fsnet_amd/csrc/conv1x1.hip
--- a/fsnet_amd/csrc/conv1x1.hip
+++ b/fsnet_amd/csrc/conv1x1.hip
@@ -241,6 +241,7 @@
 
 extern "C" int fs_conv1x1(const FsConvArgs* args, int dtype, void* stream) {
   if (!args || !args->src || !args->wgt || !args->dst) return FS_EINVAL;
+  if (fs_bnb_ext(*args)) return FS_EINVAL;
   if (dtype != FS_DTYPE_BF16 || args->dshift != 0 || args->ncls > 1 || args->hb_add != 0 || args->hb_mul < 1) return FS_EINVAL;
   if (args->Cs <= 0 || (args->Cs * 2) % 64 != 0 || args->Co % 4 != 0 || args->Co_p % 16 != 0 || args->M <= 0) return FS_EINVAL;
   if (args->src_bytes <= 0 || args->src_bytes > 0x7fffffffLL || args->wgt_bytes <= 0 || args->wgt_bytes > 0x7fffffffLL)
diff --git a/fsnet_amd/csrc/conv3x3_halo.hip b/fsnet_amd/csrc/conv3x3_halo.hip
--- a/fsnet_amd/csrc/conv3x3_halo.hip
+++ b/fsnet_amd/csrc/conv3x3_halo.hip
@@ -217,13 +217,14 @@
 
   const bool has_add = STR == 1 && p.addend != nullptr, has_mask = STR == 1 && p.mask != nullptr;
   const bool has_bnb = STR == 1 && p.bnb_x != nullptr, has_mbn = has_bnb && p.bnb_scale != nullptr;
+  const bool bnb_ext = has_bnb && p.bxN != 0;
   float s1[TC][4], s2[TC][4];
 #pragma unroll
   for (int a = 0; a < TC; ++a)
 #pragma unroll
     for (int j = 0; j < 4; ++j) { s1[a][j] = 0.f; s2[a][j] = 0.f; }
   const int sgoff = p.stat_group_rows > 0 ? fs_div(n, g.dIPG) * p.Co : 0;
-  int doff[TP], aoff[TP], moff[TP];
+  int doff[TP], aoff[TP], moff[TP], boff[TP];
 #pragma unroll
   for (int b = 0; b < TP; ++b) {
     int pi = wp * WPIX + b * 16 + li;
@@ -233,6 +234,7 @@
     doff[b] = mok ? n * (int)p.dN + y * (int)p.dH + x * (int)p.dW : -1;
     aoff[b] = n * (int)p.aN + y * (int)p.aH + x * (int)p.aW;
     moff[b] = n * (int)p.mN + y * (int)p.mH + x * (int)p.mW;
+    boff[b] = !bnb_ext ? doff[b] : (mok ? fs_bnb_src(p, n, y, x) : -1);
   }
 #pragma unroll
   for (int a = 0; a < TC; ++a) {
@@ -247,6 +249,11 @@
         msc = *reinterpret_cast<const float4*>(p.bnb_scale + sgoff + co);
         msh = *reinterpret_cast<const float4*>(p.bnb_shift + sgoff + co);
       }
+      if (bnb_ext) {
+        const float4 ga = *reinterpret_cast<const float4*>(p.bnb_gamma + co), be = *reinterpret_cast<const float4*>(p.bnb_beta + co);
+        msc.x = ga.x * is.x; msc.y = ga.y * is.y; msc.z = ga.z * is.z; msc.w = ga.w * is.w;
+        msh.x = be.x - mu.x * msc.x; msh.y = be.y - mu.y * msc.y; msh.z = be.z - mu.z * msc.z; msh.w = be.w - mu.w * msc.w;
+      }
     }
 #pragma unroll
     for (int b = 0; b < TP; ++b) {
@@ -268,15 +275,28 @@
         for (int j = 0; j < 4; ++j) v[j] = mv[j] > 0.f ? v[j] : 0.f;
       }
       if (has_bnb) {
-        float cv[4];
-        load4<T>(reinterpret_cast<const T*>(p.bnb_x) + doff[b] + co, cv);
-        if (has_mbn) {
-          v[0] = (cv[0] * msc.x + msh.x) > 0.f ? v[0] : 0.f; v[1] = (cv[1] * msc.y + msh.y) > 0.f ? v[1] : 0.f;
-          v[2] = (cv[2] * msc.z + msh.z) > 0.f ? v[2] : 0.f; v[3] = (cv[3] * msc.w + msh.w) > 0.f ? v[3] : 0.f;
+        if (bnb_ext) {
+          if (boff[b] >= 0) {
+            float cv[4], q[4];
+            load4<T>(reinterpret_cast<const T*>(p.bnb_x) + boff[b] + co, cv);
+            round4<T>(v, q);
+            q[0] = (cv[0] * msc.x + msh.x) > 0.f ? q[0] : 0.f; q[1] = (cv[1] * msc.y + msh.y) > 0.f ? q[1] : 0.f;
+            q[2] = (cv[2] * msc.z + msh.z) > 0.f ? q[2] : 0.f; q[3] = (cv[3] * msc.w + msh.w) > 0.f ? q[3] : 0.f;
+            s1[a][0] += q[0]; s1[a][1] += q[1]; s1[a][2] += q[2]; s1[a][3] += q[3];
+            s2[a][0] += q[0] * (cv[0] - mu.x) * is.x; s2[a][1] += q[1] * (cv[1] - mu.y) * is.y;
+            s2[a][2] += q[2] * (cv[2] - mu.z) * is.z; s2[a][3] += q[3] * (cv[3] - mu.w) * is.w;
+          }
+        } else {
+          float cv[4];
+          load4<T>(reinterpret_cast<const T*>(p.bnb_x) + doff[b] + co, cv);
+          if (has_mbn) {
+            v[0] = (cv[0] * msc.x + msh.x) > 0.f ? v[0] : 0.f; v[1] = (cv[1] * msc.y + msh.y) > 0.f ? v[1] : 0.f;
+            v[2] = (cv[2] * msc.z + msh.z) > 0.f ? v[2] : 0.f; v[3] = (cv[3] * msc.w + msh.w) > 0.f ? v[3] : 0.f;
+          }
+          s1[a][0] += v[0]; s1[a][1] += v[1]; s1[a][2] += v[2]; s1[a][3] += v[3];
+          s2[a][0] += v[0] * (cv[0] - mu.x) * is.x; s2[a][1] += v[1] * (cv[1] - mu.y) * is.y;
+          s2[a][2] += v[2] * (cv[2] - mu.z) * is.z; s2[a][3] += v[3] * (cv[3] - mu.w) * is.w;
         }
-        s1[a][0] += v[0]; s1[a][1] += v[1]; s1[a][2] += v[2]; s1[a][3] += v[3];
-        s2[a][0] += v[0] * (cv[0] - mu.x) * is.x; s2[a][1] += v[1] * (cv[1] - mu.y) * is.y;
-        s2[a][2] += v[2] * (cv[2] - mu.z) * is.z; s2[a][3] += v[3] * (cv[3] - mu.w) * is.w;
       } else if (p.stats) {
 #pragma unroll
         for (int j = 0; j < 4; ++j) { s1[a][j] += v[j]; s2[a][j] += v[j] * v[j]; }
@@ -466,6 +486,7 @@
   }
   if (args->bnb_scale && (!args->bnb_x || !args->bnb_shift || args->mask)) return FS_EINVAL;
   if (args->bnb_x && (!args->stats || !args->bnb_mean || !args->bnb_invstd)) return FS_EINVAL;
+  if (!fs_bnb_ext_ok(*args)) return FS_EINVAL;
   return FS_OK;
 }
 
@@ -475,7 +496,8 @@
          a.nchunks == b.nchunks && a.kg == b.kg && a.hb_mul == b.hb_mul && a.hb_add == b.hb_add && a.sgn == b.sgn &&
          a.relu == b.relu && a.out_f32 == b.out_f32 && a.pro_mode == b.pro_mode && a.pro_relu == b.pro_relu &&
          a.wgt_bytes == b.wgt_bytes && nn(a.bias, b.bias) && nn(a.addend, b.addend) && nn(a.mask, b.mask) &&
-         nn(a.stats, b.stats) && nn(a.bnb_x, b.bnb_x) && nn(a.bnb_scale, b.bnb_scale) && nn(a.pro_stats, b.pro_stats);
+         nn(a.stats, b.stats) && nn(a.bnb_x, b.bnb_x) && nn(a.bnb_scale, b.bnb_scale) && nn(a.pro_stats, b.pro_stats) &&
+         (a.bxN != 0) == (b.bxN != 0);
 }
 
 int conv3x3_entry(const FsConvArgs* args, const FsConvArgs* b, int dtype, hipStream_t st) {
diff --git a/fsnet_amd/csrc/conv3x3_p1.hip b/fsnet_amd/csrc/conv3x3_p1.hip
--- a/fsnet_amd/csrc/conv3x3_p1.hip
+++ b/fsnet_amd/csrc/conv3x3_p1.hip
@@ -102,6 +102,7 @@
 
   const bool has_add = p.addend != nullptr, has_mask = p.mask != nullptr;
   const bool has_bnb = p.bnb_x != nullptr, has_mbn = has_bnb && p.bnb_scale != nullptr;
+  const bool bnb_ext = has_bnb && p.bxN != 0;
 
   auto store_halo = [&]() {
 #pragma unroll
@@ -168,7 +169,7 @@
     for (int a = 0; a < TC; ++a)
 #pragma unroll
       for (int j = 0; j < 4; ++j) { s1[a][j] = 0.f; s2[a][j] = 0.f; }
-    int doff[TP], aoff[TP], moff[TP];
+    int doff[TP], aoff[TP], moff[TP], boff[TP];
 #pragma unroll
     for (int b = 0; b < TP; ++b) {
       const int y = y0 + (prow[b] >> 16), x = x0 + (prow[b] & 0xffff);
@@ -176,6 +177,7 @@
       doff[b] = mok ? n * (int)p.dN + y * (int)p.dH + x * (int)p.dW : -1;
       aoff[b] = n * (int)p.aN + y * (int)p.aH + x * (int)p.aW;
       moff[b] = n * (int)p.mN + y * (int)p.mH + x * (int)p.mW;
+      boff[b] = !bnb_ext ? doff[b] : (mok ? fs_bnb_src(p, n, y, x) : -1);
     }
 #pragma unroll
     for (int a = 0; a < TC; ++a) {
@@ -190,6 +192,11 @@
           msc = *reinterpret_cast<const float4*>(p.bnb_scale + sgoff + co);
           msh = *reinterpret_cast<const float4*>(p.bnb_shift + sgoff + co);
         }
+        if (bnb_ext) {
+          const float4 ga = *reinterpret_cast<const float4*>(p.bnb_gamma + co), be = *reinterpret_cast<const float4*>(p.bnb_beta + co);
+          msc.x = ga.x * is.x; msc.y = ga.y * is.y; msc.z = ga.z * is.z; msc.w = ga.w * is.w;
+          msh.x = be.x - mu.x * msc.x; msh.y = be.y - mu.y * msc.y; msh.z = be.z - mu.z * msc.z; msh.w = be.w - mu.w * msc.w;
+        }
       }
 #pragma unroll
       for (int b = 0; b < TP; ++b) {
@@ -211,15 +218,28 @@
           for (int j = 0; j < 4; ++j) v[j] = mv[j] > 0.f ? v[j] : 0.f;
         }
         if (has_bnb) {
-          float cv[4];
-          load4<T>(reinterpret_cast<const T*>(p.bnb_x) + doff[b] + co, cv);
-          if (has_mbn) {
-            v[0] = (cv[0] * msc.x + msh.x) > 0.f ? v[0] : 0.f; v[1] = (cv[1] * msc.y + msh.y) > 0.f ? v[1] : 0.f;
-            v[2] = (cv[2] * msc.z + msh.z) > 0.f ? v[2] : 0.f; v[3] = (cv[3] * msc.w + msh.w) > 0.f ? v[3] : 0.f;
+          if (bnb_ext) {
+            if (boff[b] >= 0) {
+              float cv[4], q[4];
+              load4<T>(reinterpret_cast<const T*>(p.bnb_x) + boff[b] + co, cv);
+              round4<T>(v, q);
+              q[0] = (cv[0] * msc.x + msh.x) > 0.f ? q[0] : 0.f; q[1] = (cv[1] * msc.y + msh.y) > 0.f ? q[1] : 0.f;
+              q[2] = (cv[2] * msc.z + msh.z) > 0.f ? q[2] : 0.f; q[3] = (cv[3] * msc.w + msh.w) > 0.f ? q[3] : 0.f;
+              s1[a][0] += q[0]; s1[a][1] += q[1]; s1[a][2] += q[2]; s1[a][3] += q[3];
+              s2[a][0] += q[0] * (cv[0] - mu.x) * is.x; s2[a][1] += q[1] * (cv[1] - mu.y) * is.y;
+              s2[a][2] += q[2] * (cv[2] - mu.z) * is.z; s2[a][3] += q[3] * (cv[3] - mu.w) * is.w;
+            }
+          } else {
+            float cv[4];
+            load4<T>(reinterpret_cast<const T*>(p.bnb_x) + doff[b] + co, cv);
+            if (has_mbn) {
+              v[0] = (cv[0] * msc.x + msh.x) > 0.f ? v[0] : 0.f; v[1] = (cv[1] * msc.y + msh.y) > 0.f ? v[1] : 0.f;
+              v[2] = (cv[2] * msc.z + msh.z) > 0.f ? v[2] : 0.f; v[3] = (cv[3] * msc.w + msh.w) > 0.f ? v[3] : 0.f;
+            }
+            s1[a][0] += v[0]; s1[a][1] += v[1]; s1[a][2] += v[2]; s1[a][3] += v[3];
+            s2[a][0] += v[0] * (cv[0] - mu.x) * is.x; s2[a][1] += v[1] * (cv[1] - mu.y) * is.y;
+            s2[a][2] += v[2] * (cv[2] - mu.z) * is.z; s2[a][3] += v[3] * (cv[3] - mu.w) * is.w;
           }
-          s1[a][0] += v[0]; s1[a][1] += v[1]; s1[a][2] += v[2]; s1[a][3] += v[3];
-          s2[a][0] += v[0] * (cv[0] - mu.x) * is.x; s2[a][1] += v[1] * (cv[1] - mu.y) * is.y;
-          s2[a][2] += v[2] * (cv[2] - mu.z) * is.z; s2[a][3] += v[3] * (cv[3] - mu.w) * is.w;
         } else if (p.stats) {
 #pragma unroll
           for (int j = 0; j < 4; ++j) { s1[a][j] += v[j]; s2[a][j] += v[j] * v[j]; }
diff --git a/fsnet_amd/csrc/conv3x3_s2d.hip b/fsnet_amd/csrc/conv3x3_s2d.hip
--- a/fsnet_amd/csrc/conv3x3_s2d.hip
+++ b/fsnet_amd/csrc/conv3x3_s2d.hip
@@ -344,6 +344,7 @@
   if ((a.Cs * es) % 64 != 0 || a.Co_p % S2D_CO != 0 || a.Co % 8 != 0) return false;
   if (a.bias || a.relu || a.out_f32 || a.pro_mode || a.bnb_scale || a.grp_imgs) return false;
   if (a.stats && !a.bnb_x) return false;
+  if (fs_bnb_ext(a)) return false;
   if ((a.ds_src != nullptr) != (a.ds_wgt != nullptr)) return false;
   if (a.ds_src && (a.ds_wgt_row_bytes < (int64_t)a.Cs * es || a.ds_wgt_row_bytes * a.Co_p >= 0x7ffff000LL ||
                    ((uintptr_t)a.ds_src & 15u) || ((uintptr_t)a.ds_wgt & 15u)))
diff --git a/fsnet_amd/csrc/conv3x3_t32.hip b/fsnet_amd/csrc/conv3x3_t32.hip
--- a/fsnet_amd/csrc/conv3x3_t32.hip
+++ b/fsnet_amd/csrc/conv3x3_t32.hip
@@ -179,7 +179,8 @@
   const bool has_mask = T32_FLAG(EP_MASK, p.mask != nullptr);
   const bool has_bnb = T32_FLAG(EP_BNB, p.bnb_x != nullptr);
   const bool has_stats = T32_FLAG(EP_STATS | EP_BNB, p.stats != nullptr);
-  const bool has_mbn = T32_FLAG(EP_MASKBN, p.bnb_scale != nullptr);
+  const bool has_mbn = T32_FLAG(EP_MASKBN, p.bnb_scale != nullptr || p.bxN != 0);
+  const bool bnb_ext = has_bnb && p.bxN != 0;
   const bool f32out = T32_FLAG(EP_F32, p.out_f32 != 0);
 
   t32_barrier();
@@ -215,7 +216,14 @@
 #pragma unroll
     for (int j = 0; j < 8; ++j) { bv[j] = 0.f; msc[j] = 0.f; msh[j] = 0.f; s1[j] = 0.f; s2[j] = 0.f; }
     if (has_bias) load8<float>(p.bias + cof, bv);
-    if (has_mbn) { load8<float>(p.bnb_scale + sgoff + cof, msc); load8<float>(p.bnb_shift + sgoff + cof, msh); }
+    if (has_mbn && !bnb_ext) { load8<float>(p.bnb_scale + sgoff + cof, msc); load8<float>(p.bnb_shift + sgoff + cof, msh); }
+    if (bnb_ext) {
+      float mu[8], is[8], be[8];
+      load8<float>(p.bnb_gamma + cof, msc); load8<float>(p.bnb_beta + cof, be);
+      load8<float>(p.bnb_mean + sgoff + cof, mu); load8<float>(p.bnb_invstd + sgoff + cof, is);
+#pragma unroll
+      for (int j = 0; j < 8; ++j) { msc[j] = msc[j] * is[j]; msh[j] = be[j] - mu[j] * msc[j]; }
+    }
 #pragma unroll
     for (int i = 0; i < NI; ++i) {
       const float* rp = ep + ((i * 16 + l15) * EPS + 2 * cs) * 4;
@@ -241,14 +249,28 @@
         for (int j = 0; j < 8; ++j) v[j] = mv[j] > 0.f ? v[j] : 0.f;
       }
       if (has_bnb) {
-        float cv[8];
-        load8<T>(reinterpret_cast<const T*>(p.bnb_x) + dof + co, cv);
-        if (has_mbn) {
-#pragma unroll
-          for (int j = 0; j < 8; ++j) v[j] = (cv[j] * msc[j] + msh[j]) > 0.f ? v[j] : 0.f;
+        if (bnb_ext) {
+          const int bof = fs_bnb_src(p, n, y, x);
+          if (bof >= 0) {
+            float cv[8], q[8];
+            load8<T>(reinterpret_cast<const T*>(p.bnb_x) + bof + co, cv);
+            round4<T>(v, q); round4<T>(v + 4, q + 4);
+#pragma unroll
+            for (int j = 0; j < 8; ++j) {
+              q[j] = (cv[j] * msc[j] + msh[j]) > 0.f ? q[j] : 0.f;
+              s1[j] += q[j]; s2[j] += q[j] * cv[j];
+            }
+          }
+        } else {
+          float cv[8];
+          load8<T>(reinterpret_cast<const T*>(p.bnb_x) + dof + co, cv);
+          if (has_mbn) {
+#pragma unroll
+            for (int j = 0; j < 8; ++j) v[j] = (cv[j] * msc[j] + msh[j]) > 0.f ? v[j] : 0.f;
+          }
+#pragma unroll
+          for (int j = 0; j < 8; ++j) { s1[j] += v[j]; s2[j] += v[j] * cv[j]; }
         }
-#pragma unroll
-        for (int j = 0; j < 8; ++j) { s1[j] += v[j]; s2[j] += v[j] * cv[j]; }
       } else if (has_stats) {
 #pragma unroll
         for (int j = 0; j < 8; ++j) { s1[j] += v[j]; s2[j] += v[j] * v[j]; }
@@ -371,6 +393,7 @@
       case EP_MASK | EP_BNB: return t32_dispatch_cfg<T, EP_MASK | EP_BNB, PRO>(a, b, cfg, st);
       case EP_ADDEND | EP_MASK | EP_BNB: return t32_dispatch_cfg<T, EP_ADDEND | EP_MASK | EP_BNB, PRO>(a, b, cfg, st);
       case EP_BNB | EP_MASKBN: return t32_dispatch_cfg<T, EP_BNB | EP_MASKBN, PRO>(a, b, cfg, st);
+      case EP_ADDEND | EP_BNB | EP_MASKBN: return t32_dispatch_cfg<T, EP_ADDEND | EP_BNB | EP_MASKBN, PRO>(a, b, cfg, st);
       default: break;
     }
   }
@@ -402,7 +425,7 @@
   };
   const int dsz = a.out_f32 ? 4 : es;
   if (!al16(a.dst, a.dN, a.dH, a.dW, dsz) || !al16(a.addend, a.aN, a.aH, a.aW, es) || !al16(a.mask, a.mN, a.mH, a.mW, es) ||
-      !al16(a.bnb_x, a.dN, a.dH, a.dW, es))
+      !al16(a.bnb_x, a.bxN ? a.bxN : a.dN, a.bxN ? a.bxH : a.dH, a.bxN ? a.bxW : a.dW, es))
     return false;
   const int64_t span = (int64_t)(a.N - 1) * a.dN + (int64_t)(a.Hd - 1) * a.dH + (int64_t)(a.Wd - 1) * a.dW + a.Co;
   if (a.dN < 0 || a.dH < 0 || a.dW < 0 || span >= 0x7fffffffLL) return false;
diff --git a/fsnet_amd/csrc/conv_igemm.hip b/fsnet_amd/csrc/conv_igemm.hip
--- a/fsnet_amd/csrc/conv_igemm.hip
+++ b/fsnet_amd/csrc/conv_igemm.hip
@@ -343,6 +343,7 @@
 int igemm_check(const FsConvArgs* args) {
   if (!args || !args->src || !args->wgt || !args->dst || !args->ktab) return FS_EINVAL;
   if (args->kg != 4 && args->kg != 8) return FS_EINVAL;
+  if (fs_bnb_ext(*args)) return FS_EINVAL;
   const int units = args->nchunks * (args->kg == 8 ? 2 : 4);
   if (args->nchunks <= 0 || units > 1024) return FS_EINVAL;
   if (args->Co % 4 != 0 || args->Co_p % 16 != 0) return FS_EINVAL;
diff --git a/fsnet_amd/csrc/conv_stem.hip b/fsnet_amd/csrc/conv_stem.hip
--- a/fsnet_amd/csrc/conv_stem.hip
+++ b/fsnet_amd/csrc/conv_stem.hip
@@ -146,6 +146,7 @@
 int stem_check(const FsConvArgs* a, int dtype) {
   if (!a || !a->src || !a->wgt || !a->dst) return FS_EINVAL;
   if (dtype != FS_DTYPE_BF16 || a->Cs != 8 || a->Co != 64 || a->Co_p != 64) return FS_EINVAL;
+  if (fs_bnb_ext(*a)) return FS_EINVAL;
   if (a->bias || a->addend || a->mask || a->bnb_x || a->relu || a->out_f32 || a->grp_imgs || a->ncls > 1) return FS_EINVAL;
   if (a->Hd != (a->Hs + 6 - 7) / 2 + 1 || a->Wd != (a->Ws + 6 - 7) / 2 + 1 || a->N <= 0) return FS_EINVAL;
   if (a->nchunks * a->kg * 8 < TAPS * 8) return FS_EINVAL;
diff --git a/fsnet_amd/csrc/fsnet_hip_internal.h b/fsnet_amd/csrc/fsnet_hip_internal.h
--- a/fsnet_amd/csrc/fsnet_hip_internal.h
+++ b/fsnet_amd/csrc/fsnet_hip_internal.h
@@ -13,3 +13,27 @@
 inline int fs_xcd_round(long blocks) { return (int)((blocks + 7) / 8 * 8); }
 
 int fs_conv1x1_gemm(const FsConvArgs& a, hipStream_t st);
+
+constexpr int FS_BNB_EXT_MAX_C = 256;
+inline bool fs_bnb_ext(const FsConvArgs& a) {
+  return a.bxN != 0 || a.bxH != 0 || a.bxW != 0 || a.bnb_win != 0 || a.bnb_pad != 0 || a.bnb_gamma != nullptr || a.bnb_beta != nullptr;
+}
+inline bool fs_bnb_ext_ok(const FsConvArgs& a) {
+  if (!fs_bnb_ext(a)) return true;
+  if (a.bxN <= 0 || a.bxH <= 0 || a.bxW <= 0 || a.bnb_win < 0 || a.bnb_win > 2 || a.bnb_pad < 0 || a.bnb_pad > 1) return false;
+  if (!a.bnb_x || !a.stats || !a.bnb_mean || !a.bnb_invstd || !a.bnb_gamma || !a.bnb_beta) return false;
+  if (a.bnb_scale || a.bnb_shift || a.mask || a.relu || a.out_f32 || a.ncls > 1 || a.hb_mul != 1) return false;
+  if (a.Co > FS_BNB_EXT_MAX_C) return false;
+  const int64_t h = (int64_t)a.Hd - 2 * a.bnb_pad, w = (int64_t)a.Wd - 2 * a.bnb_pad;
+  if (h < 1 || w < 1 || a.N < 1) return false;
+  return (int64_t)(a.N - 1) * a.bxN + (h - 1) * a.bxH + (w - 1) * a.bxW + a.Co_p < 0x7fffffffLL;
+}
+#ifdef __HIPCC__
+__device__ __forceinline__ int fs_bnb_src(const FsConvArgs& p, int n, int y, int x) {
+  const int pad = p.bnb_pad;
+  const bool ring = y < pad || x < pad || y >= p.Hd - pad || x >= p.Wd - pad;
+  if ((p.bnb_win == 1 && ring) || (p.bnb_win == 2 && !ring)) return -1;
+  const int cy = min(max(y - pad, 0), p.Hd - 1 - 2 * pad), cx = min(max(x - pad, 0), p.Wd - 1 - 2 * pad);
+  return n * (int)p.bxN + cy * (int)p.bxH + cx * (int)p.bxW;
+}
+#endif
diff --git a/fsnet_amd/csrc/t32_common.h b/fsnet_amd/csrc/t32_common.h
--- a/fsnet_amd/csrc/t32_common.h
+++ b/fsnet_amd/csrc/t32_common.h
@@ -157,7 +157,7 @@
   if (a.bnb_x) m |= EP_BNB;
   else if (a.stats) m |= EP_STATS;
   if (a.out_f32) m |= EP_F32;
-  if (a.bnb_x && a.bnb_scale) m |= EP_MASKBN;
+  if (a.bnb_x && (a.bnb_scale || a.bxN)) m |= EP_MASKBN;
   return m;
 }
 
diff --git a/fsnet_amd/csrc/version.hip b/fsnet_amd/csrc/version.hip
--- a/fsnet_amd/csrc/version.hip
+++ b/fsnet_amd/csrc/version.hip
@@ -1,6 +1,7 @@
 #include "common.h"
 #include "fsnet_hip_internal.h"
 extern "C" int fs_abi_version(void) { return FS_ABI_VERSION; }
+extern "C" int fs_conv_args_bytes(void) { return (int)sizeof(FsConvArgs); }
 extern "C" const char* fs_target_arch(void) { return "gfx950"; }
 
 namespace {
diff --git a/fsnet_amd/engine/nets.py b/fsnet_amd/engine/nets.py
--- a/fsnet_amd/engine/nets.py
+++ b/fsnet_amd/engine/nets.py
@@ -564,7 +564,7 @@
     return _BWD_POOLS[(c.device, raw_stream(c.device.index))].take(c.shape[-1], st.groups)
 
 
-def _bn_bwd(dout, y, c, bn, st, H, W, relu=True, fold=False, g_out=None, sums=None):
+def _bn_bwd(dout, y, c, bn, st, H, W, relu=True, fold=False, g_out=None, sums=None, mask_x=False):
     dc = torch.empty_like(c)
     reduced = sums is not None
     if sums is None:
@@ -572,7 +572,8 @@
     sync = RT.dp is not None and st.count != float("inf")
     ops.bn_backward(dout, y, c, bn.weight.data, st, dc, grad_of(bn.weight), grad_of(bn.bias), H, W, relu=relu,
                     fold=fold, g_out=g_out, sums=sums, sums_zeroed=True, reduced=reduced,
-                    allreduce=(RT.dp.allreduce_small if sync else None))
+                    allreduce=(RT.dp.allreduce_small if sync else None),
+                    mask_x=(bn.bias.data if (reduced and mask_x) else None))
     return dc
 
 
@@ -1190,22 +1191,49 @@
                                            m.max_depth, dt, P2=ctx["P2"], base_fx=ctx["base_fx"])
             dls = dict(zip(sc, res))
 
-        def disp_grad(i):
+        def heads_of(i):
+            has_u = i in self.unc and g_unc.get(i) is not None
+            return ([self.disp[i]] if i in dls else []) + ([self.unc[i]] if has_u else [])
+
+        def bn1_sums(i):
+            lv = ctx["lv"][i]
+            y1p, s1 = lv["y1p"], lv["s1"]
+            N, Hp, Wp, _ = y1p.shape
+            heads = heads_of(i)
+            if not RT.ddec_bn1_fold or s1.groups != 1 or (i == 0 and not heads):
+                return None
+            if heads and not heads[-1].ready(dt, dev).can_fold_pad_sums(N, Hp - 2, Wp - 2, Hp, Wp, "all" if i == 0 else "ring",
+                                                                     s1.groups, addend=len(heads) > 1):
+                return None
+            if i > 0 and not self.up0[i - 1][0].ready(dt, dev).can_fold_pad_sums(N, Hp - 2, Wp - 2, Hp - 2, Wp - 2, "interior",
+                                                                              s1.groups, addend=bool(heads)):
+                return None
+            return _bwd_sums(lv["c1"], s1)
+
+        def disp_grad(i, sums1=None):
             lv = ctx["lv"][i]
             y1p = lv["y1p"]
             G = None
+            last = heads_of(i)[-1:] if sums1 is not None else []
+            bn1 = self.up1[i][1]
+
+            def ps(cl):
+                if not last or cl is not last[0]:
+                    return None
+                return (lv["c1"], lv["s1"], sums1, bn1.weight.data, bn1.bias.data, "all" if i == 0 else "ring")
+
             if i in dls:
                 cld = self.disp[i]
                 opd = cld.ready(dt, dev)
                 dl = dls[i]
                 cld.accumulate_param_grads(opd, dl, y1p)
-                G = opd.dgrad(dl, y1p.shape[1], y1p.shape[2])
+                G = opd.dgrad(dl, y1p.shape[1], y1p.shape[2], pad_sums=ps(cld))
             if i in self.unc and g_unc.get(i) is not None:
                 clu = self.unc[i]
                 opu = clu.ready(dt, dev)
                 dlu = ops.sigmoid_head_bwd(lv["unc"], g_unc[i], opu.Co_p, dt)
                 clu.accumulate_param_grads(opu, dlu, y1p)
-                G = opu.dgrad(dlu, y1p.shape[1], y1p.shape[2], addend=G)
+                G = opu.dgrad(dlu, y1p.shape[1], y1p.shape[2], addend=G, pad_sums=ps(clu))
             if G is not None:
                 return G, False
             key = (tuple(y1p.shape), y1p.dtype, y1p.device)
@@ -1213,7 +1241,8 @@
                 self._border0 = (key, torch.zeros_like(y1p))
             return self._border0[1], True
 
-        Gp, _ = disp_grad(0)
+        sums1 = bn1_sums(0)
+        Gp, _ = disp_grad(0, sums1)
         for i in range(0, 5):
             issue_advanced(dev)
             lv = ctx["lv"][i]
@@ -1222,7 +1251,7 @@
             cl1, bn1 = self.up1[i]
             op1 = cl1.ready(dt, dev)
             y1_int = lv["y1p"][:, 1:-1, 1:-1]
-            dc1 = _bn_bwd(Gp, y1_int, lv["c1"], bn1, lv["s1"], H2, W2, relu=True, fold=True)
+            dc1 = _bn_bwd(Gp, y1_int, lv["c1"], bn1, lv["s1"], H2, W2, relu=True, fold=True, sums=sums1, mask_x=True)
             cl1.accumulate_param_grads(op1, dc1, lv["xcat"])
             dxcat = op1.dgrad(dc1, H2 + 2, W2 + 2)
             cl0, bn0 = self.up0[i]
@@ -1234,9 +1263,14 @@
             dc0 = _bn_bwd(d_y0, None, lv["c0"], bn0, lv["s0"], h, w, sums=sums0)
             cl0.accumulate_param_grads(op0, dc0, lv["x"])
             if i < 4:
-                Gp, fresh = disp_grad(i + 1)
+                sums1 = bn1_sums(i + 1)
+                Gp, fresh = disp_grad(i + 1, sums1)
                 interior = Gp[:, 1:-1, 1:-1]
-                op0.dgrad(dc0, h, w, out=interior, addend=None if fresh else interior)
+                nlv = ctx["lv"][i + 1]
+                nbn1 = self.up1[i + 1][1]
+                op0.dgrad(dc0, h, w, out=interior, addend=None if fresh else interior,
+                          pad_sums=None if sums1 is None else (nlv["c1"], nlv["s1"], sums1, nbn1.weight.data, nbn1.bias.data,
+                                                               "interior"))
             else:
                 gfeats[4] = op0.dgrad(dc0, h, w)
         RT.mark("ddec.bwd.end")
diff --git a/fsnet_amd/engine/runtime.py b/fsnet_amd/engine/runtime.py
--- a/fsnet_amd/engine/runtime.py
+++ b/fsnet_amd/engine/runtime.py
@@ -27,6 +27,7 @@
         self._lanes_override = None
         self.stem_flush = self._lanes
         self.pack_overlap = True
+        self.ddec_bn1_fold = True
         self._side = {}
         self._held = {}
         self._marks = {} if os.environ.get("FSNET_AMD_MARKS", "0") != "0" else None
diff --git a/fsnet_amd/hip/binding.py b/fsnet_amd/hip/binding.py
--- a/fsnet_amd/hip/binding.py
+++ b/fsnet_amd/hip/binding.py
@@ -42,6 +42,9 @@
         ("pro_dst", C.c_void_p),
         ("pro_count", C.c_double), ("pro_eps", C.c_float), ("pro_momentum", C.c_float),
         ("ds_src", C.c_void_p), ("ds_wgt", C.c_void_p), ("ds_wgt_row_bytes", C.c_int64),
+        ("bxN", C.c_int64), ("bxH", C.c_int64), ("bxW", C.c_int64),
+        ("bnb_win", C.c_int32), ("bnb_pad", C.c_int32),
+        ("bnb_gamma", C.c_void_p), ("bnb_beta", C.c_void_p),
     ]
 
 
@@ -205,6 +208,9 @@
     if got != ABI_VERSION:
         raise FsError("libfsnet_hip.so at %s reports ABI %d, this binding is written against ABI %d (FS_ABI_VERSION "
                       "in include/fsnet_hip.h): rebuild it with `python fsnet_amd/csrc/build.py`" % (path, got, ABI_VERSION))
+    if not hasattr(handle, "fs_conv_args_bytes") or int(handle.fs_conv_args_bytes()) != C.sizeof(FsConvArgs):
+        raise FsError("libfsnet_hip.so at %s was built with another FsConvArgs than this binding mirrors (%d bytes here): "
+                      "rebuild it with `python fsnet_amd/csrc/build.py`" % (path, C.sizeof(FsConvArgs)))
     _lib = handle
     return _lib
 
diff --git a/fsnet_amd/hip/conv.py b/fsnet_amd/hip/conv.py
--- a/fsnet_amd/hip/conv.py
+++ b/fsnet_amd/hip/conv.py
@@ -460,11 +460,56 @@
         run_specs([sp])
         return sp.out
 
-    def dgrad_spec(self, dy, H, W, out=None, addend=None, mask=None, bn_fuse=None, mask_bn=False, ds=None):
+    PAD_WINDOWS = {"all": (0, 1), "interior": (1, 0), "ring": (2, 1)}
+    PAD_SUMS_MAX_C = 256
+
+    def can_fold_pad_sums(self, N, Hy, Wy, H, W, window, groups=1, addend=False):
+        if not (self.halo_d and self.Ci_p == self.Ci and groups == 1 and window in self.PAD_WINDOWS):
+            return False
+        return self.pad_sums_plan(N, Hy, Wy, H, W, window, addend) is not None
+
+    def pad_sums_plan(self, N, Hy, Wy, H, W, window, addend=False):
+        key = ("ps", N, Hy, Wy, H, W, window, bool(addend), FORCE_3X3)
+        if key in self._tabs:
+            return self._tabs[key]
+        eb = 2 if self.dtype == torch.bfloat16 else 4
+        win, pad = self.PAD_WINDOWS[window]
+        Cd, Cx = self.Co_p, self.Ci_p
+        a = FsConvArgs()
+        a.src, a.wgt, a.dst = 16, 16, 16
+        a.sN, a.sH, a.sW = Hy * Wy * Cd, Wy * Cd, Cd
+        Hp, Wp = (H + 2, W + 2) if window == "interior" else (H, W)
+        a.dN, a.dH, a.dW = Hp * Wp * Cx, Wp * Cx, Cx
+        if addend:
+            a.addend, a.aN, a.aH, a.aW = 16, a.dN, a.dH, a.dW
+        a.src_bytes, a.wgt_bytes = N * Hy * Wy * Cd * eb, self.w_d.numel() * eb
+        a.Hs, a.Ws, a.Hd, a.Wd, a.M = Hy, Wy, H, W, N * H * W
+        a.Co, a.Co_p, a.nchunks, a.kg = Cx, self.rows_d, self.nch_d, self.kg_d
+        a.hb_mul, a.hb_add, a.sgn = 1, self.pad, -1
+        a.N, a.Cs = N, Cd
+        Hc, Wc = H - 2 * pad, W - 2 * pad
+        a.bnb_x = a.bnb_mean = a.bnb_invstd = a.bnb_gamma = a.bnb_beta = a.stats = 16
+        a.bxN, a.bxH, a.bxW = Hc * Wc * Cx, Wc * Cx, Cx
+        a.bnb_win, a.bnb_pad = win, pad
+        a.force_impl = FORCE_3X3
+        plan = (C.c_int32 * 4)()
+        res = None
+        if Hc >= 1 and Wc >= 1 and lib.fs_conv3x3_halo_plan(C.byref(a), self.code, plan) == 0:
+            res = {"kernel": {0: "halo", 1: "t32", 2: "p1"}[int(plan[0])], "blocks": int(plan[1]), "pix": int(plan[2]), "co": int(plan[3])}
+        self._tabs[key] = res
+        return res
+
+    def dgrad_spec(self, dy, H, W, out=None, addend=None, mask=None, bn_fuse=None, mask_bn=False, ds=None, pad_sums=None):
         N, Ho, Wo, Cd = dy.shape
         assert Cd == self.Co_p and dy.dtype == self.dtype and self.need_dgrad
         if out is None:
             out = torch.empty(N, H, W, self.Ci_p, dtype=self.dtype, device=dy.device)
+        if pad_sums is not None:
+            c, st, _, _, _, window = pad_sums
+            win, pad = self.PAD_WINDOWS[window]
+            assert bn_fuse is None and mask is None and not mask_bn and ds is None and self.halo_d and self.stride == 1
+            assert c.is_contiguous() and c.dtype == self.dtype and c.shape == (N, H - 2 * pad, W - 2 * pad, self.Ci_p)
+            assert tuple(out.shape) == (N, H, W, self.Ci_p) and st.groups == 1 and self.Ci_p == self.Ci
         if bn_fuse is not None:
             c, st, _ = bn_fuse
             assert c.is_contiguous() and out.is_contiguous() and c.shape == out.shape and c.dtype == self.dtype
@@ -505,6 +550,13 @@
                 a.bnb_scale, a.bnb_shift = st.scale.data_ptr(), st.shift.data_ptr()
         else:
             assert not mask_bn
+        if pad_sums is not None:
+            c, st, sums, gamma, beta, window = pad_sums
+            a.bnb_x, a.bnb_mean, a.bnb_invstd = c.data_ptr(), st.mean.data_ptr(), st.invstd.data_ptr()
+            a.bnb_gamma, a.bnb_beta = gamma.data_ptr(), beta.data_ptr()
+            a.stats = sums.data_ptr()
+            a.bxN, a.bxH, a.bxW = _nhwc_strides(c)
+            a.bnb_win, a.bnb_pad = self.PAD_WINDOWS[window]
         flops = 2.0 * N * Ho * Wo * self.Co * self.R * self.S * self.Ci
         halo = self.halo_d
         tag = lambda: "dgrd %s dy[%d,%d,%d,%d]" % (self.describe(), N, Ho, Wo, Cd)
diff --git a/fsnet_amd/hip/ops.py b/fsnet_amd/hip/ops.py
--- a/fsnet_amd/hip/ops.py
+++ b/fsnet_amd/hip/ops.py
@@ -107,16 +107,20 @@
 
 
 def bn_backward(dout, y, x, gamma, st, dx, dgamma, dbeta, H, W, relu=True, fold=False, g_out=None, sums=None,
-                allreduce=None, sums_zeroed=False, reduced=False, phase="all", glob=None, pool=None):
+                allreduce=None, sums_zeroed=False, reduced=False, phase="all", glob=None, pool=None, mask_x=None):
     bn_backward_multi([dict(dout=dout, y=y, x=x, gamma=gamma, st=st, dx=dx, dgamma=dgamma, dbeta=dbeta, H=H, W=W, relu=relu,
-                            fold=fold, g_out=g_out, sums=sums, sums_zeroed=sums_zeroed, reduced=reduced, glob=glob, pool=pool)],
+                            fold=fold, g_out=g_out, sums=sums, sums_zeroed=sums_zeroed, reduced=reduced, glob=glob, pool=pool,
+                            mask_x=mask_x)],
                       allreduce=allreduce, phase=phase)
     return None if phase == "reduce" else dx
 
 
 def _bn_bwd_call(dout, y, x, gamma, st, dx, dgamma, dbeta, H, W, relu=True, fold=False, g_out=None, sums=None,
-                 sums_zeroed=False, reduced=False, glob=None, pool=None):
-    if reduced:
+                 sums_zeroed=False, reduced=False, glob=None, pool=None, mask_x=None):
+    if reduced and mask_x is not None:
+        assert sums is not None and g_out is None and pool is None
+        relu, y = True, None
+    elif reduced:
         assert sums is not None and not fold and g_out is None
         relu, y = False, None
     Cc = x.shape[-1]
@@ -132,6 +136,8 @@
         a.pool_dy, a.pool_idx, a.beta = pool[0].data_ptr(), pool[1].data_ptr(), pool[2].data_ptr()
     else:
         assert dout is not None
+    if reduced and mask_x is not None:
+        a.beta = mask_x.data_ptr()
     a.sums = sums.data_ptr()
     a.gamma, a.save_mean, a.save_invstd = gamma.data_ptr(), st.mean.data_ptr(), st.invstd.data_ptr()
     a.dgamma, a.dbeta = _p(dgamma), _p(dbeta)
diff --git a/fsnet_amd/hip/signatures.py b/fsnet_amd/hip/signatures.py
--- a/fsnet_amd/hip/signatures.py
+++ b/fsnet_amd/hip/signatures.py
@@ -8,6 +8,7 @@
 
 SIGNATURES = {
     "fs_abi_version": (C.c_int, []),
+    "fs_conv_args_bytes": (C.c_int, []),
     "fs_target_arch": (C.c_char_p, []),
     "fs_debug_timestamp": (C.c_int, [P, P]),
     "fs_capture_position": (C.c_int, [P, P]),
diff --git a/include/fsnet_hip.h b/include/fsnet_hip.h
--- a/include/fsnet_hip.h
+++ b/include/fsnet_hip.h
@@ -17,6 +17,7 @@
 
 #define FS_ABI_VERSION 15
 int fs_abi_version(void);
+int fs_conv_args_bytes(void);
 const char* fs_target_arch(void);
 int fs_debug_timestamp(void* slot, void* stream);
 int fs_capture_position(void* stream, unsigned long long* token);
@@ -74,6 +75,9 @@
   float pro_eps, pro_momentum;
   const void* ds_src; const void* ds_wgt;
   int64_t ds_wgt_row_bytes;
+  int64_t bxN, bxH, bxW;
+  int32_t bnb_win, bnb_pad;
+  const float* bnb_gamma; const float* bnb_beta;
 } FsConvArgs;
 int fs_conv_igemm(const FsConvArgs* args, int dtype, void* stream);
 
```

Result: no change. 2291 samples/s (-0.0%).
